# f1tenth/f1tenth_planning

Hardware: AMD Instinct MI355X
Metric: candidate-trajectory-steps/sec per GPU; p50 plan() latency @4096 egos (higher is better)
Workload: dtype f32 filter + f64 decision

## Files before the change

f1tenth_planning_amd/csrc/f1p_device.h:

```cpp
#pragma once
#include <hip/hip_runtime.h>
#include <stdint.h>

#include "../../include/f1p.h"

#define F1P_WAVE 64
#define F1P_PI 3.14159265358979323846
#define F1P_LA_NONE INT32_MIN
#ifndef F1P_NEAREST_PRUNE
#define F1P_NEAREST_PRUNE 1
#endif

namespace f1p {

__device__ __forceinline__ double shfl_d(double v, int src) {
    int lo = __double2loint(v), hi = __double2hiint(v);
    lo = __shfl(lo, src, F1P_WAVE);
    hi = __shfl(hi, src, F1P_WAVE);
    return __hiloint2double(hi, lo);
}
__device__ __forceinline__ double shfl_xor_d(double v, int mask) {
    int lo = __double2loint(v), hi = __double2hiint(v);
    lo = __shfl_xor(lo, mask, F1P_WAVE);
    hi = __shfl_xor(hi, mask, F1P_WAVE);
// ... 177 lines not shown
    best_d = __builtin_huge_val();
    best_i = 0x7fffffff;
    double bt = 0.0;
    const int lane = tid & 63, wave = tid >> 6, nw = nthreads >> 6;
    const int nseg = n - 1;
    const int nchunk = (nseg + 63) >> 6;
    const int stride = (n + 63) >> 6;
    int j = lane * stride;
    if (j > n - 1) j = n - 1;
    double b0x = 0.0, b0X = 0.0, b0y = 0.0, b0Y = 0.0, sx_ = 0.0, sy_ = 0.0;
    if (pre) { b0x = pre[0]; b0X = pre[1]; b0y = pre[2]; b0Y = pre[3]; sx_ = pre[4]; sy_ = pre[5]; }
    else {
        if (lane < nchunk) { b0x = box[4 * lane]; b0X = box[4 * lane + 1]; b0y = box[4 * lane + 2]; b0Y = box[4 * lane + 3]; }
        sx_ = wx[j]; sy_ = wy[j];
    }
    const double ex = px - sx_, ey = py - sy_;
    const double ub2_own = ex * ex + ey * ey;
    const float ub2_up = (float)ub2_own * (1.0f + 2.4e-7f);
    const double ub2 = (double)f32_from_order_key(wave_min_key(f32_order_key(ub2_up == ub2_up ? ub2_up : __builtin_nanf(""))));
    const double thr = ub2 * (1.0 + 1e-6) + 1e-9;
    int turn = 0;
    for (int cb = 0; cb < nchunk; cb += 64) {
        const int c = cb + lane;
        bool keep = false;
        if (c < nchunk) {
            double xmin = b0x, xmax = b0X, ymin = b0y, ymax = b0Y;
            if (cb > 0) { xmin = box[4 * c]; xmax = box[4 * c + 1]; ymin = box[4 * c + 2]; ymax = box[4 * c + 3]; }
            const double dx = __builtin_fmax(__builtin_fmax(xmin - px, px - xmax), 0.0);
            const double dy = __builtin_fmax(__builtin_fmax(ymin - py, py - ymax), 0.0);
            keep = !(dx * dx + dy * dy > thr);
        }
        unsigned long long m = __ballot(keep);
        while (m) {
            const int b = __ffsll((long long)m) - 1;
            m &= m - 1;
            if (turn == wave) {
                const int i = ((cb + b) << 6) + lane;
                if (i < nseg) {
                    const SegProj s = seg_project(px, py, wx[i], wy[i], wx[i + 1], wy[i + 1]);
                    if (argmin_better(s.d, i, best_d, best_i)) { best_d = s.d; best_i = i; bt = s.t; }
                }
            }
            if (++turn == nw) turn = 0;
        }
    }
    if (best_t) *best_t = bt;
}

struct SegHit { bool hit; double t, x, y; };

__device__ __forceinline__ SegHit seg_hit(double px, double py, double radius, double sx, double sy, double ex, double ey,
                                          bool is_start_seg, double start_t) {
    SegHit h;
    h.hit = false; h.t = 0.0; h.x = 0.0; h.y = 0.0;
    ex = ex + 1e-6;
    ey = ey + 1e-6;
    const double vx = ex - sx, vy = ey - sy;
    const double a = dot2(vx, vy, vx, vy);
    const double b = 2.0 * dot2(vx, vy, sx - px, sy - py);
    const double c = dot2(sx, sy, sx, sy) + dot2(px, py, px, py) - 2.0 * dot2(sx, sy, px, py) - radius * radius;
    double disc = b * b - 4 * a * c;
    if (disc < 0) return h;
    disc = __builtin_sqrt(disc);
    const double t1 = (-b - disc) / (2.0 * a);
    const double t2 = (-b + disc) / (2.0 * a);
    const bool ok1 = (t1 >= 0.0) & (t1 <= 1.0) & (!is_start_seg | (t1 >= start_t));
    const bool ok2 = (t2 >= 0.0) & (t2 <= 1.0) & (!is_start_seg | (t2 >= start_t));
    if (ok1) { h.hit = true; h.t = t1; }
    else if (ok2) { h.hit = true; h.t = t2; }
    if (h.hit) { h.x = sx + h.t * vx; h.y = sy + h.t * vy; }
    return h;
}

struct Intersect { bool found; int i; double t, x, y; };

__device__ __forceinline__ Intersect wave_intersect(double px, double py, double radius, const double* wx, const double* wy,
                                                    int n, double tstart, bool wrap) {
    const int lane = threadIdx.x & 63;
    const int start_i = (int)tstart;
    const double start_t = tstart - __builtin_trunc(tstart);
    Intersect r;
    r.found = false; r.i = 0; r.t = 0.0; r.x = 0.0; r.y = 0.0;
    for (int base = start_i; base < n - 1; base += 64) {
        const int i = base + lane;
        SegHit h;
        h.hit = false; h.t = 0; h.x = 0; h.y = 0;
        if (i < n - 1) h = seg_hit(px, py, radius, wx[i], wy[i], wx[i + 1], wy[i + 1], i == start_i, start_t);
        const unsigned long long m = __ballot(h.hit);
        if (m) {
            const int first = __ffsll((long long)m) - 1;
            r.found = true; r.i = base + first;
            r.t = shfl_d(h.t, first); r.x = shfl_d(h.x, first); r.y = shfl_d(h.y, first);
            return r;
        }
    }
    if (wrap) {
        for (int base = -1; base < start_i; base += 64) {
            const int i = base + lane;
            SegHit h;
            h.hit = false; h.t = 0; h.x = 0; h.y = 0;
            if (i < start_i) {
                const int i0 = i < 0 ? i + n : i;
                int i1 = i + 1; if (i1 >= n) i1 -= n;
                h = seg_hit(px, py, radius, wx[i0], wy[i0], wx[i1], wy[i1], false, 0.0);
            }
            const unsigned long long m = __ballot(h.hit);
            if (m) {
                const int first = __ffsll((long long)m) - 1;
                r.found = true; r.i = base + first;
                r.t = shfl_d(h.t, first); r.x = shfl_d(h.x, first); r.y = shfl_d(h.y, first);
                return r;
            }
        }
    }
    return r;
}

__device__ __forceinline__ void get_actuation(double pose_theta, double lx, double ly, double lspeed, double px, double py,
                                              double lookahead, double wheelbase, double& speed, double& steer) {
    const double sn = pose_theta == 0.0 ? -pose_theta : sin(-pose_theta);
    const double cs = pose_theta == 0.0 ? 1.0 : cos(-pose_theta);
    const double wy = dot2(sn, cs, lx - px, ly - py);
    speed = lspeed;
    if (fabs(wy) < 1e-6) { steer = 0.0; return; }
    const double radius = 1 / (2.0 * wy / (lookahead * lookahead));
    steer = atan(wheelbase / radius);
}

struct Track { double steer, speed; int la_idx, status; };

__device__ __forceinline__ Track wave_pursuit(double px, double py, double theta, double lookahead, double wheelbase,
                                              double max_reacquire, const double* wx, const double* wy, const double* wv,
                                              double v_const, int n, int near_i, double near_t, double near_d) {
    Track o;
    o.steer = 0.0; o.speed = 0.0; o.la_idx = F1P_LA_NONE; o.status = F1P_ST_NO_LOOKAHEAD;
    double cx, cy, cv;
    if (near_d < lookahead) {
        const Intersect it = wave_intersect(px, py, lookahead, wx, wy, n, (double)near_i + near_t, true);
        if (!it.found) return o;
        o.la_idx = it.i;
        const int r = it.i < 0 ? it.i + n : it.i;
        cx = wx[r]; cy = wy[r]; cv = wv ? wv[near_i] : v_const;
        o.status = F1P_ST_INTERSECT;
    } else if (near_d < max_reacquire) {
        cx = wx[near_i]; cy = wy[near_i]; cv = wv ? wv[near_i] : v_const;
        o.status = F1P_ST_REACQUIRE;
    } else {
        return o;
    }
    get_actuation(theta, cx, cy, cv, px, py, lookahead, wheelbase, o.speed, o.steer);
    return o;
}

struct GridDev {
    const uint32_t* bits;
    int32_t w, h, wwords;
    double inv_res, ox, oy;
};

__device__ __forceinline__ bool cell_of(const GridDev& g, double x, double y, int& gx, int& gy) {
    const double fx = __builtin_floor((x - g.ox) * g.inv_res);
    const double fy = __builtin_floor((y - g.oy) * g.inv_res);
    const bool inside = (fx >= 0.0) & (fy >= 0.0) & (fx < (double)g.w) & (fy < (double)g.h);
    gx = inside ? (int)fx : -1;
    gy = inside ? (int)fy : -1;
    return inside;
}

struct KmpcStep { double x, y, v, yaw; };

template <bool FAST>
__device__ __forceinline__ void kmpc_step(KmpcStep& s, double a, double delta, const f1p_kmpc_cfg& c) {
    if (delta >= c.max_steer) delta = c.max_steer;
    else if (delta <= -c.max_steer) delta = -c.max_steer;
    double sn, cs, tn;
    if (FAST) {
        double sd, cd;
        sincos_core(s.yaw, &sn, &cs);
        sincos_core(delta, &sd, &cd);
        tn = sd / cd;
    } else {
        sincos(s.yaw, &sn, &cs);
        tn = tan(delta);
    }
    const double x = s.x + s.v * cs * c.dt;
    const double y = s.y + s.v * sn * c.dt;
    const double yaw = s.yaw + (s.v / c.wheelbase) * tn * c.dt;
    double v = s.v + a * c.dt;
    if (v > c.max_speed) v = c.max_speed;
    else if (v < c.min_speed) v = c.min_speed;
    s.x = x; s.y = y; s.yaw = yaw; s.v = v;
}


struct DynState { double x, y, delta, v, yaw, yr, beta; };
struct DynConst { double K, gl_r, gl_f, h, F, R, M, N, lf2cf, lr2cr, l_r, l_f; };

__device__ __forceinline__ DynConst dyn_const(const f1p_stmpc_cfg& c) {
    const double* p = c.params;
    const double mass = p[0], l_f = p[1], l_r = p[2], h_cog = p[3], c_f = p[4], c_r = p[5], iz = p[6], mu = p[7];
    const double g = 9.81;
    DynConst k;
    k.K = (mu * mass) / ((l_f + l_r) * iz);
    k.gl_r = g * l_r; k.gl_f = g * l_f; k.h = h_cog;
    k.F = l_f * c_f; k.R = l_r * c_r;
    k.M = (mu * c_f) / (l_f + l_r);
    k.N = (mu * c_r) / (l_f + l_r);
    k.lf2cf = l_f * l_f * c_f; k.lr2cr = l_r * l_r * c_r;
    k.l_r = l_r; k.l_f = l_f;
    return k;
}

template <bool FAST>
__device__ __forceinline__ void dyn_step(DynState& s, double a, double delta_v, const f1p_stmpc_cfg& c, const DynConst& k) {
    if (delta_v >= c.max_steer_v) delta_v = c.max_steer_v;
    else if (delta_v <= -c.max_steer_v) delta_v = -c.max_steer_v;
    if (a >= c.max_accel) a = c.max_accel;
    else if (a <= -c.max_accel) a = -c.max_accel;
    const double T = k.gl_r - (a * k.h);
    const double V = k.gl_f + (a * k.h);
    const double A1 = k.K * k.F * T;
    const double A2 = k.K * (k.R * V - k.F * T);
    const double A3 = k.K * (k.lf2cf * T + k.lr2cr * V);
    const double A4 = k.M * T;
    const double A5 = k.N * V + k.M * T;
    const double A6 = k.N * V * k.l_r - k.M * T * k.l_f;
    double sn, cs, tn;
    if (FAST) {
        double sd, cd;
        sincos_fast(s.yaw + s.beta, &sn, &cs);
        sincos_core(s.delta, &sd, &cd);
        tn = sd / cd;
    } else {
        sincos(s.yaw + s.beta, &sn, &cs);
        tn = tan(s.delta);
    }
    const double x_new = s.x + s.v * cs * c.dt;
    const double y_new = s.y + s.v * sn * c.dt;
    double delta_new = s.delta + delta_v * c.dt;
    double v_new = s.v + a * c.dt;
    const double yaw_new = s.yaw + s.v / c.wheelbase * tn * c.dt;
    const double yr_new = s.yr + (A1 * s.delta + A2 * s.beta - A3 * (s.yr / s.v)) * c.dt;
    const double beta_new = s.beta + (A4 * (s.delta / s.v) - A5 * (s.beta / s.v) + A6 * (s.yr / (s.v * s.v)) - s.yr) * c.dt;
    if (v_new > c.max_speed) v_new = c.max_speed;
    else if (v_new < c.min_speed) v_new = c.min_speed;
    if (delta_new >= c.max_steer) delta_new = c.max_steer;
    else if (delta_new <= -c.max_steer) delta_new = -c.max_steer;
    s.x = x_new; s.y = y_new; s.delta = delta_new; s.v = v_new; s.yaw = yaw_new; s.yr = yr_new; s.beta = beta_new;
}

}
```

f1tenth_planning_amd/csrc/f1p_internal.h:

```cpp
#pragma once
#include <vector>
#include <hip/hip_runtime.h>
#include <stdint.h>

#include <string>

#include "../../include/f1p.h"
#include "f1p_device.h"

#define F1P_KMPC_CFG_SLOTS 8

struct WarmBuf {
    void* d = nullptr;
    size_t bytes = 0;
    int key[3] = {0, 0, 0};
    bool is(int a, int b, int c = 0) const { return d && key[0] == a && key[1] == b && key[2] == c; }
    template <typename T> T* as() const { return (T*)d; }
};

struct f1p_ctx {
    int device = -1;
    hipStream_t stream = nullptr;
    hipEvent_t ev0 = nullptr, ev1 = nullptr;
    hipStream_t copy_stream = nullptr;
    hipEvent_t ev_chunk[8] = {};
    std::string err;
    hipDeviceProp_t prop;

    int n_wp = 0;
    bool has_psi = false;
    double *d_wx = nullptr, *d_wy = nullptr, *d_wv = nullptr, *d_wpsi = nullptr, *d_wkappa = nullptr;
    bool has_kappa = false;
    double* d_wbox = nullptr;

    int trk_K = 0;
    int trk_rows = 0, trk_chunks = 0;
    bool trk_has_psi = false, trk_has_kappa = false;
    double *d_tx = nullptr, *d_ty = nullptr, *d_tv = nullptr, *d_tpsi = nullptr, *d_tkappa = nullptr, *d_tbox = nullptr;
    int32_t* d_ttab = nullptr;

    bool has_grid = false;
    uint32_t* d_bits = nullptr;
    uint32_t* d_bits0 = nullptr;
    double inflate_radius = 0.0;
    double user_inflate = 0.0;
    double disc_radius = 0.0;
    uint32_t* d_bits_clear = nullptr;
    double clear_dist = 0.0;
    int lattice_clear_r = 2;
    int n_disc = 0;
    double disc_off[4] = {0, 0, 0, 0};
    int gw = 0, gh = 0, gwwords = 0;
    double res = 0, inv_res = 0, ox = 0, oy = 0;

    char* d_arena = nullptr;
    size_t arena_bytes = 0, arena_used = 0;
    char* h_bounce = nullptr;

    bool kmpc_mixed = true;
    float* d_dbg_cost32 = nullptr;
    int32_t* d_dbg_nref = nullptr;

    bool stmpc_mixed = true;
    float* d_dbg_st_cost32 = nullptr;
    int32_t* d_dbg_st_nref = nullptr;
    char* d_st_scratch = nullptr;
    size_t st_scratch_bytes = 0;
    bool st_q_dirty = true;

    f1p_kmpc_cfg* d_kmpc_cfg = nullptr;
    f1p_kmpc_cfg* h_kmpc_cfg = nullptr;
    f1p_kmpc_cfg* d_kmpc_cfg_cur = nullptr;
    int kmpc_cfg_used = 0;
    WarmBuf kmpc_warm;
    bool kmpc_warm_valid = false;
    char* d_kmpc_scratch = nullptr;
    int kmpc_cap_E = 0, kmpc_cap_R = 0;
    int kmpc_yaw_fixup = 1;
    int kmpc_groups = 0;
    WarmBuf kmpc_qp_warm;
    bool kmpc_qp_warm_valid = false;
    int kmpc_qp_pack = 0;
    WarmBuf stmpc_qp_warm;
    std::vector<int32_t> stmpc_qp_len;
    WarmBuf stmpc_warm;
    std::vector<int32_t> stmpc_warm_tag;

    char* d_bb_scratch = nullptr;
    size_t bb_scratch_bytes = 0;

    int lattice_mixed = 1;
    int pursuit_form = 0;
    char* d_mix_scratch = nullptr;
    size_t mix_scratch_bytes = 0;
    int mix_last_E = 0;
    size_t mix_ego_n_off = 0;
    char* d_rec_scratch = nullptr;
    size_t rec_scratch_bytes = 0;
    float dbg_margin_rel = 0.f, dbg_margin_abs = 0.f; bool dbg_margins = false;
    int audit_every = 0, audit_egos = 0;
    bool auditing = false;
    unsigned long long audit_plans = 0;
    unsigned long long* d_audit = nullptr;
    char* d_audit_buf = nullptr;
    size_t audit_buf_bytes = 0;
    int lattice_chunks = 0;
    hipStream_t pipe_stream[2] = {};
    hipEvent_t ev_pipe[4] = {};
    char* d_order = nullptr;
    size_t order_bytes = 0;
    int order_E = 0;
    bool order_valid = false;
    int lattice_order = 1;
    bool step_chain = false;
    bool mix_q_dirty_prev = false;
    bool mix_q_dirty = false;
    bool lattice_profile = false, lattice_profile_valid = false;
    hipEvent_t ev_prof[5] = {};
    float* d_dbg_lat_bound = nullptr;
    float* d_dbg_lat_cost32 = nullptr;
    int32_t* d_dbg_lat_state = nullptr;
    int32_t* d_dbg_lat_pass = nullptr;

    bool lattice_closed_loop = false;
    double* d_cl_theta[2] = {nullptr, nullptr};
    size_t cl_bytes = 0;
    int cl_cur = 0;
    bool cl_valid = false;
    int cl_E = 0, cl_S = 0;

    bool traj_dst_host = false;
    char* h_step = nullptr; size_t step_host_bytes = 0;
    char* h_step_dev = nullptr;
    char* d_step = nullptr; size_t step_dev_bytes = 0;
    struct HostBlock { char* base; size_t bytes; char* dev; };
    std::vector<HostBlock> host_blocks;
    int step_traj_E = 0, step_traj_S = 0;

    char* d_split_scratch = nullptr;
    int split_cap_E = 0;
    int lattice_split = 0;

    void* rccl_lib = nullptr;
    void* comm = nullptr;
    int comm_rank = 0, comm_nranks = 0;
    uint64_t* d_comm_key = nullptr;
    int32_t* d_comm_idx = nullptr;
    int comm_cap = 0;
    int comm_exchange = 0;
    uint64_t* d_comm_rec = nullptr;
    int comm_rec_cap = 0, comm_rec_ranks = 0;
};

namespace f1p {

int set_error(f1p_ctx* ctx, int code, const std::string& msg);
int check_hip(f1p_ctx* ctx, hipError_t e, const char* what);

#define F1P_HIP(ctx, call)                                   \
    do {                                                     \
        hipError_t _e = (call);                              \
        if (_e != hipSuccess) return f1p::check_hip((ctx), _e, #call); \
    } while (0)

int arena_reset(f1p_ctx* ctx, size_t need_bytes);
void* arena_take(f1p_ctx* ctx, size_t bytes);

GridDev grid_dev(const f1p_ctx* ctx);

int warm_ensure(f1p_ctx* ctx, WarmBuf* w, size_t bytes, int a, int b, int c, bool zero, bool* fresh);
int warm_upload(f1p_ctx* ctx, WarmBuf* w, const void* host, size_t bytes);
int warm_download(f1p_ctx* ctx, const WarmBuf* w, void* host, size_t bytes);

int launch_nearest(f1p_ctx* ctx, const double* d_pts, int E, double* d_proj, double* d_dist, double* d_t, int32_t* d_idx);
int launch_intersect(f1p_ctx* ctx, const double* d_pts, const double* d_start_t, int E, double radius, int wrap,
                     double* d_p, int32_t* d_i, double* d_t, int32_t* d_found);
int launch_pure_pursuit(f1p_ctx* ctx, const double* d_poses, int E, double lookahead, double wheelbase,
                        double max_reacquire, double* d_steer, double* d_speed, int32_t* d_near, int32_t* d_la,
                        int32_t* d_status);
int launch_pack_grid(f1p_ctx* ctx, const uint8_t* d_img, int w, int h, int occupied_below);
int launch_grid_edt(f1p_ctx* ctx, int cap, uint32_t thr2, float* d_dist_img, uint32_t* d_d2, uint32_t* d_bits_out, const uint32_t* src = nullptr);
int ensure_clear_map(f1p_ctx* ctx, double dist_cells);

enum LatticeMode { LATTICE_FULL = 0, LATTICE_EVAL = 1, LATTICE_EMIT = 2 };
int launch_lattice(f1p_ctx* ctx, int mode, const double* d_poses, const double* d_goals, const double* d_prev_theta,
                   int E, const f1p_lattice_cfg* cfg, const int32_t* d_emit_idx, const double* d_emit_cost,
                   double* d_steer, double* d_speed, int32_t* d_best_idx, double* d_best_cost, int32_t* d_status,
                   int32_t* d_near_idx, double* d_best_traj, double* d_all_cost, double* d_all_traj, float* d_best_traj32 = nullptr,
                   double* d_theta_out = nullptr,
                   double* d_pose_copy = nullptr,
                   const int32_t* d_track_id = nullptr);
int launch_clothoid_sample(f1p_ctx* ctx, const double* d_params, int n, int S, double* d_rows);
int launch_clothoid_g1(f1p_ctx* ctx, const double* d_goals, int n, double* d_k0, double* d_dk, double* d_len, int32_t* d_ok);

int launch_kmpc_shoot(f1p_ctx* ctx, const double* d_x0, const double* d_ref, const float* d_controls, int E,
                      const f1p_kmpc_cfg* cfg, double* d_steer, double* d_speed, int32_t* d_best_idx,
                      double* d_best_cost, double* d_best_seq);
int launch_kmpc_plan_gen(f1p_ctx* ctx, const double* d_x0, const double* d_ref, int E, const f1p_kmpc_cfg* cfg,
                         const f1p_kmpc_sampler* smp, const float* d_warm_in, float* d_warm_out, double* d_steer, double* d_speed,
                         int32_t* d_best_idx, double* d_best_cost, double* d_best_seq,
                         const int32_t* d_ids = nullptr, int wstride = 0, uint32_t ego_off = 0u);
int launch_kmpc_gen_controls(f1p_ctx* ctx, float* d_controls, int E, const f1p_kmpc_cfg* cfg, const f1p_kmpc_sampler* smp, const float* d_warm);
int kmpc_plan_groups(const f1p_ctx* ctx, int E, int R);
int launch_kmpc_qp(f1p_ctx* ctx, const double* d_x0, const double* d_ref, const double* d_pa, const double* d_pd, int pstride, int E,
                   const f1p_kmpc_cfg* cfg, int max_iter, double tol, double* d_steer, double* d_speed, int32_t* d_status, double* d_u,
                   double* d_xk, double* d_obj, double* d_duals, int32_t* d_iters, double* d_warm_out);
int kmpc_qp_pack(const f1p_ctx* ctx, int T);
int launch_stmpc_qp(f1p_ctx* ctx, const double* d_x0, const double* d_ref, const double* d_pa, const double* d_pd, int pstride, int E,
                    const f1p_stmpc_cfg* cfg, int max_iter, double tol, double* d_steer, double* d_speed, int32_t* d_status, double* d_u,
                    double* d_x, double* d_obj, double* d_duals, int32_t* d_iters, double* d_warm_out);
size_t stmpc_qp_lds_bytes(int T);
int launch_stmpc_qp_warm_in(f1p_ctx* ctx, const double* d_warm, const int32_t* d_idx, const int32_t* d_use, int nb, int Tb, int W, double* d_out);
int launch_stmpc_qp_warm_out(f1p_ctx* ctx, const double* d_in, const int32_t* d_idx, int nb, int Tb, int W, double* d_warm);
int launch_stmpc_qp_kref(f1p_ctx* ctx, const double* d_ref7, int nb, int T, double* d_ref4);
int launch_kmpc_predict(f1p_ctx* ctx, const double* d_x0, const double* d_oa, const double* d_od, int E,
                        const f1p_kmpc_cfg* cfg, double* d_path);
int launch_kmpc_ref(f1p_ctx* ctx, const double* d_states, int E, int horizon, double dt, double dl, double* d_ref);
int launch_kmpc_sample(f1p_ctx* ctx, float* d_controls, int E, const f1p_kmpc_cfg* cfg, uint64_t seed, double sigma_a,
                       double sigma_d);
int launch_stanley(f1p_ctx* ctx, const double* d_states, int E, double wheelbase, double k_path, double* d_steer,
                   double* d_speed, int32_t* d_near);
int launch_lqr(f1p_ctx* ctx, const double* d_states, double* d_err, int E, double wheelbase, double ts, const double* q,
               double r, int max_iter, double eps, double* d_steer, double* d_speed, int32_t* d_near);
int launch_stmpc_predict(f1p_ctx* ctx, const double* d_x0, const double* d_oa, const double* d_od, int E, const f1p_stmpc_cfg* cfg, double* d_path);
int launch_stmpc_shoot(f1p_ctx* ctx, const double* d_x0, const double* d_ref, const float* d_controls, int E, const f1p_stmpc_cfg* cfg,
                       double* d_steer, double* d_speed, int32_t* d_best_idx, double* d_best_cost, double* d_best_seq);
int launch_stmpc_ref(f1p_ctx* ctx, const double* d_states, int E, int horizon, double dt, double dl, double* d_ref);
int launch_stmpc_plan_gen(f1p_ctx* ctx, const double* d_x0, const double* d_ref, int E, const f1p_stmpc_cfg* cfg, const f1p_stmpc_sampler* smp,
                          float* d_warm, int wstride, const int32_t* d_ids, double* d_steer, double* d_speed, int32_t* d_best_idx,
                          double* d_best_cost, double* d_best_seq);
int launch_stmpc_gen_controls(f1p_ctx* ctx, float* d_controls, int E, const f1p_stmpc_cfg* cfg, const f1p_stmpc_sampler* smp, float* d_warm, int wstride);
int launch_stmpc_warm_zero(f1p_ctx* ctx, float* d_warm, const int32_t* d_rows, int n, int wstride);
struct TrackSetDev {
    const double *x, *y, *v, *psi, *kappa, *box;
    const int4* tab;
    int K;
};
TrackSetDev track_set_dev(const f1p_ctx* ctx);
int launch_nearest_tracks(f1p_ctx* ctx, const double* d_pts, const int32_t* d_tid, int E, double* d_proj, double* d_dist, double* d_t,
                          int32_t* d_idx);
int launch_pure_pursuit_tracks(f1p_ctx* ctx, const double* d_poses, const int32_t* d_tid, int E, double lookahead, double wheelbase,
                               double max_reacquire, double* d_steer, double* d_speed, int32_t* d_near, int32_t* d_la, int32_t* d_status);
int launch_stanley_tracks(f1p_ctx* ctx, const double* d_states, const int32_t* d_tid, int E, double wheelbase, double k_path,
                          double* d_steer, double* d_speed, int32_t* d_near);
int launch_lqr_tracks(f1p_ctx* ctx, const double* d_states, const int32_t* d_tid, double* d_err, int E, double wheelbase, double ts,
                      const double* q, double r, int max_iter, double eps, double* d_steer, double* d_speed, int32_t* d_near);
int launch_kmpc_ref_tracks(f1p_ctx* ctx, const double* d_states, const int32_t* d_tid, int E, int horizon, double dt, double dl, double* d_ref);
int launch_stmpc_ref_tracks(f1p_ctx* ctx, const double* d_states, const int32_t* d_tid, int E, int horizon, double dt, double dl, double* d_ref);
int launch_argmin_key(f1p_ctx* ctx, const double* d_cost, uint64_t* d_key, int E);
int launch_argmin_mask(f1p_ctx* ctx, const uint64_t* d_own, const uint64_t* d_min, const int32_t* d_idx, int32_t* d_masked,
                       double* d_cost_out, int E);
int launch_argmin_pack(f1p_ctx* ctx, const double* d_cost, const int32_t* d_idx, uint64_t* d_rec, int E);
int launch_argmin_reduce(f1p_ctx* ctx, const uint64_t* d_recs, int N, int E, int32_t* d_idx_out, double* d_cost_out);

}
```

f1tenth_planning_amd/csrc/f1p_lattice.hip:

```cpp
#include "f1p_host.h"

using namespace f1p;

#ifndef F1P_TRAJ_ZEROCOPY
#define F1P_TRAJ_ZEROCOPY 1
#endif
#ifndef F1P_IO_ZEROCOPY
#define F1P_IO_ZEROCOPY 1
#endif
#define F1P_PLAN_CHUNK_MIN_EGOS 2048
#ifndef F1P_ZEROCOPY_MIN_EGOS
#define F1P_ZEROCOPY_MIN_EGOS 32
#endif
#define F1P_PLAN_CHUNKS_MAX 8

static int ensure_copy_stream(f1p_ctx* ctx) {
    if (ctx->copy_stream) return F1P_OK;
    F1P_HIP(ctx, hipStreamCreateWithFlags(&ctx->copy_stream, hipStreamNonBlocking));
    for (auto& ev : ctx->ev_chunk) F1P_HIP(ctx, hipEventCreateWithFlags(&ev, hipEventDisableTiming));
    return F1P_OK;
}

static int validate_lattice(f1p_ctx* ctx, const f1p_lattice_cfg* cfg, int E, bool device_goals, bool need_outputs_ok, bool tracks = false) {
    if (!cfg) return set_error(ctx, F1P_EINVAL, "cfg is NULL");
// ... 238 lines not shown
    const int K = (pinned && E >= 8192) ? (E / 4096 < F1P_PLAN_CHUNKS_MAX ? E / 4096 : F1P_PLAN_CHUNKS_MAX) : 1;
    if (K > 1 && (rc = ensure_copy_stream(ctx))) return rc;
    if (K == 1) {
        if ((rc = plan(0, e))) return rc;
        cl_commit(ctx, cl, E, (int)S);
        return s.finish();
    }
    for (int k = 0; k < K; ++k) {
        const size_t e0 = e * k / K, e1 = e * (k + 1) / K, n = e1 - e0;
        if ((rc = plan(e0, n))) return rc;
        F1P_HIP(ctx, hipEventRecord(ctx->ev_chunk[k], ctx->stream));
        F1P_HIP(ctx, hipStreamWaitEvent(ctx->copy_stream, ctx->ev_chunk[k], 0));
        F1P_HIP(ctx, hipMemcpyAsync(best_traj + e0 * S * 4, d_bt + e0 * S * 4, n * S * 4 * sizeof(TRAJ), hipMemcpyDeviceToHost, ctx->copy_stream));
    }
    cl_commit(ctx, cl, E, (int)S);
    rc = s.gather(best_traj);
    F1P_HIP(ctx, hipStreamSynchronize(ctx->copy_stream));
    return rc;
}

int f1p_lattice_plan_batch(f1p_ctx* ctx, const double* poses, const double* goals, const double* prev_theta,
                           int32_t E, const f1p_lattice_cfg* cfg, double* steer, double* speed, int32_t* best_idx,
                           double* best_cost, int32_t* status, int32_t* near_idx, double* best_traj,
                           double* all_cost, double* all_traj) {
    F1P_ENTER(ctx);
    return lattice_plan_batch_impl<double>(ctx, poses, goals, prev_theta, E, cfg, steer, speed, best_idx, best_cost, status, near_idx, best_traj, all_cost, all_traj);
}

int f1p_lattice_plan_batch_f32(f1p_ctx* ctx, const double* poses, const double* goals, const double* prev_theta,
                               int32_t E, const f1p_lattice_cfg* cfg, double* steer, double* speed, int32_t* best_idx,
                               double* best_cost, int32_t* status, int32_t* near_idx, float* best_traj32) {
    F1P_ENTER(ctx);
    return lattice_plan_batch_impl<float>(ctx, poses, goals, prev_theta, E, cfg, steer, speed, best_idx, best_cost, status, near_idx, best_traj32, nullptr, nullptr);
}

int f1p_lattice_plan_tracks_batch(f1p_ctx* ctx, const double* poses, const double* goals, const double* prev_theta, const int32_t* track_id,
                                  int32_t E, const f1p_lattice_cfg* cfg, double* steer, double* speed, int32_t* best_idx,
                                  double* best_cost, int32_t* status, int32_t* near_idx, double* best_traj,
                                  double* all_cost, double* all_traj) {
    F1P_ENTER(ctx);
    return lattice_plan_batch_impl<double>(ctx, poses, goals, prev_theta, E, cfg, steer, speed, best_idx, best_cost, status, near_idx, best_traj, all_cost, all_traj,
                                           track_id, true);
}

int f1p_lattice_plan_tracks_batch_f32(f1p_ctx* ctx, const double* poses, const double* goals, const double* prev_theta, const int32_t* track_id,
                                      int32_t E, const f1p_lattice_cfg* cfg, double* steer, double* speed, int32_t* best_idx,
                                      double* best_cost, int32_t* status, int32_t* near_idx, float* best_traj32) {
    F1P_ENTER(ctx);
    return lattice_plan_batch_impl<float>(ctx, poses, goals, prev_theta, E, cfg, steer, speed, best_idx, best_cost, status, near_idx, best_traj32, nullptr, nullptr,
                                          track_id, true);
}

static int ensure_step(f1p_ctx* ctx, int E, int S, bool keep_traj) {
    const size_t hb = al256(32 * (size_t)E) + 2 * al256(8 * (size_t)E) + al256(4 * (size_t)E);
    if (hb > ctx->step_host_bytes) {
        F1P_HIP(ctx, hipStreamSynchronize(ctx->stream));
        if (ctx->h_step) (void)hipHostFree(ctx->h_step);
        ctx->h_step = nullptr; ctx->step_host_bytes = 0; ctx->h_step_dev = nullptr;
        F1P_HIP(ctx, hipHostMalloc((void**)&ctx->h_step, hb, hipHostMallocDefault));
        ctx->step_host_bytes = hb;
        void* dev = nullptr;
        ctx->h_step_dev = (hipHostGetDevicePointer(&dev, ctx->h_step, 0) == hipSuccess) ? (char*)dev : nullptr;
        if (!ctx->h_step_dev) (void)hipGetLastError();
    }
    const size_t db = al256(32 * (size_t)E) + 2 * al256(4 * (size_t)E) + (keep_traj ? al256(32 * (size_t)E * S) : 0);
    if (db > ctx->step_dev_bytes) {
        F1P_HIP(ctx, hipStreamSynchronize(ctx->stream));
        if (ctx->d_step) (void)hipFree(ctx->d_step);
        ctx->d_step = nullptr; ctx->step_dev_bytes = 0; ctx->step_traj_E = 0;
        F1P_HIP(ctx, hipMalloc((void**)&ctx->d_step, db));
        ctx->step_dev_bytes = db;
    }
    return F1P_OK;
}

static int lattice_step_impl(f1p_ctx* ctx, const double* poses, int32_t E, const f1p_lattice_cfg* cfg, double* steer, double* speed,
                             int32_t* status, int32_t keep_traj, const int32_t* track_id, bool tracks) {
    int rc = validate_lattice(ctx, cfg, E, true, E == 0 || (poses && steer && speed), tracks);
    if (rc) return rc;
    if (cfg->cand_count > 0) return set_error(ctx, F1P_EINVAL, "f1p_lattice_step_batch plans whole egos: cfg.cand_count must be 0");
    if (tracks && E > 0 && !track_id) return set_error(ctx, F1P_EINVAL, "track_id is NULL");
    if (E == 0) return F1P_OK;
    const int S = cfg->n_stations;
    const size_t e = (size_t)E;
    if ((rc = ensure_step(ctx, E, S, keep_traj != 0))) return rc;
    char* hb = ctx->h_step;
    double* h_poses = (double*)hb; double* h_steer = (double*)(hb + al256(32 * e)); double* h_speed = (double*)((char*)h_steer + al256(8 * e));
    int32_t* h_status = (int32_t*)((char*)h_speed + al256(8 * e));
    char* db = ctx->d_step;
    double* d_pose_copy = (double*)db; int32_t* d_idx = (int32_t*)(db + al256(32 * e)); int32_t* d_near = (int32_t*)((char*)d_idx + al256(4 * e));
    double* d_traj = keep_traj ? (double*)((char*)d_near + al256(4 * e)) : nullptr;
    const double* k_poses = (const double*)pinned_device_ptr(ctx, poses, 32 * e);
    if (!k_poses) { memcpy(h_poses, poses, 32 * e); k_poses = (const double*)pinned_device_ptr(ctx, h_poses, 32 * e); }
    double* k_steer = (double*)pinned_device_ptr(ctx, steer, 8 * e); double* k_speed = (double*)pinned_device_ptr(ctx, speed, 8 * e);
    int32_t* k_status = status ? (int32_t*)pinned_device_ptr(ctx, status, 4 * e) : nullptr;
    const bool own_steer = !k_steer, own_speed = !k_speed, own_status = status && !k_status;
    if (own_steer) k_steer = (double*)pinned_device_ptr(ctx, h_steer, 8 * e);
    if (own_speed) k_speed = (double*)pinned_device_ptr(ctx, h_speed, 8 * e);
    if (own_status) k_status = (int32_t*)pinned_device_ptr(ctx, h_status, 4 * e);
    if (!k_poses || !k_steer || !k_speed || (status && !k_status)) return set_error(ctx, F1P_ESTATE, "page-locked step block is not device-visible");
    const int32_t* k_tid = tracks ? (const int32_t*)pinned_device_ptr(ctx, track_id, 4 * e) : nullptr;
    if (tracks && !k_tid) {
        if ((rc = arena_reset(ctx, al256(4 * e)))) return rc;
        int32_t* d = (int32_t*)arena_take(ctx, 4 * e);
        F1P_HIP(ctx, hipMemcpyAsync(d, track_id, 4 * e, hipMemcpyHostToDevice, ctx->stream));
        k_tid = d;
    }
    const bool was_armed = ctx->lattice_closed_loop;
    if (!was_armed && !ctx->step_chain) ctx->cl_valid = false;
    ctx->lattice_closed_loop = true;
    ClosedLoop cl;
    rc = cl_begin(ctx, nullptr, E, S, true, &cl);
    if (rc == F1P_OK)
        rc = launch_lattice(ctx, LATTICE_FULL, k_poses, nullptr, cl.prev, E, cfg, nullptr, nullptr, k_steer, k_speed, d_idx, nullptr, k_status, d_near,
                            d_traj, nullptr, nullptr, nullptr, cl.out, d_pose_copy, k_tid);
    ctx->lattice_closed_loop = was_armed;
    if (rc) return rc;
    cl_commit(ctx, cl, E, S);
    ctx->step_chain = !was_armed;
    ctx->step_traj_E = keep_traj ? E : 0; ctx->step_traj_S = S;
    F1P_HIP(ctx, hipStreamSynchronize(ctx->stream));
    if (own_steer) memcpy(steer, h_steer, 8 * e);
    if (own_speed) memcpy(speed, h_speed, 8 * e);
    if (own_status) memcpy(status, h_status, 4 * e);
    return F1P_OK;
}

int f1p_lattice_step_batch(f1p_ctx* ctx, const double* poses, int32_t E, const f1p_lattice_cfg* cfg, double* steer, double* speed,
                           int32_t* status, int32_t keep_traj) {
    F1P_ENTER(ctx);
    return lattice_step_impl(ctx, poses, E, cfg, steer, speed, status, keep_traj, nullptr, false);
}

int f1p_lattice_step_tracks_batch(f1p_ctx* ctx, const double* poses, const int32_t* track_id, int32_t E, const f1p_lattice_cfg* cfg, double* steer,
                                  double* speed, int32_t* status, int32_t keep_traj) {
    F1P_ENTER(ctx);
    return lattice_step_impl(ctx, poses, E, cfg, steer, speed, status, keep_traj, track_id, true);
}

int f1p_lattice_fetch_traj(f1p_ctx* ctx, double* best_traj, int32_t E, int32_t S) {
    F1P_ENTER(ctx);
    if (!best_traj) return set_error(ctx, F1P_EINVAL, "best_traj is NULL");
    if (ctx->step_traj_E <= 0 || !ctx->d_step) return set_error(ctx, F1P_ESTATE, "no trajectories kept: call f1p_lattice_step_batch with keep_traj = 1 first");
    if (E != ctx->step_traj_E || S != ctx->step_traj_S) return set_error(ctx, F1P_EINVAL, "E / S differ from the last f1p_lattice_step_batch");
    const size_t e = (size_t)E;
    const char* d_traj = ctx->d_step + al256(32 * e) + 2 * al256(4 * e);
    F1P_HIP(ctx, hipMemcpyAsync(best_traj, d_traj, 32 * e * S, hipMemcpyDeviceToHost, ctx->stream));
    F1P_HIP(ctx, hipStreamSynchronize(ctx->stream));
    return F1P_OK;
}

int f1p_lattice_set_mode(f1p_ctx* ctx, int32_t mixed, float* d_cost32, int32_t* d_state) {
    if (!ctx) return F1P_EINVAL;
    if (mixed < 0 || mixed > 3) return set_error(ctx, F1P_EINVAL, "mixed must be 0 (all fp64), 1 (f32 filter, the default), 2 (f32 filter at any batch size) or 3 (as 2, one ego per wave in the per-ego kernels)");
    ctx->lattice_mixed = mixed;
    ctx->d_dbg_lat_cost32 = d_cost32;
    ctx->d_dbg_lat_state = d_state;
    return F1P_OK;
}

int f1p_lattice_set_split(f1p_ctx* ctx, int32_t groups) {
    if (!ctx) return F1P_EINVAL;
    if (groups < 0 || groups > 16) return set_error(ctx, F1P_EINVAL, "groups must be in [0, 16]");
    ctx->lattice_split = groups;
    return F1P_OK;
}

int f1p_lattice_set_clearance(f1p_ctx* ctx, int32_t stations_each_side) {
    if (!ctx) return F1P_EINVAL;
    if (stations_each_side < 0 || stations_each_side > 2) return set_error(ctx, F1P_EINVAL, "stations_each_side must be 0, 1 or 2");
    ctx->lattice_clear_r = stations_each_side;
    return F1P_OK;
}

int f1p_lattice_debug_queue(f1p_ctx* ctx, int32_t* entries_per_ego, int32_t E) {
    F1P_ENTER(ctx);
    if (!entries_per_ego || E < 1) return set_error(ctx, F1P_EINVAL, "entries_per_ego is NULL or E < 1");
    if (!ctx->d_mix_scratch || ctx->mix_last_E != E) return set_error(ctx, F1P_ESTATE, "no mixed-schedule plan of this batch size has run");
    F1P_HIP(ctx, hipStreamSynchronize(ctx->stream));
    F1P_HIP(ctx, hipMemcpy(entries_per_ego, ctx->d_mix_scratch + ctx->mix_ego_n_off, sizeof(int32_t) * (size_t)E, hipMemcpyDeviceToHost));
    return F1P_OK;
}

int f1p_lattice_debug_bound(f1p_ctx* ctx, float* d_bound) {
    if (!ctx) return F1P_EINVAL;
    ctx->d_dbg_lat_bound = d_bound;
    return F1P_OK;
}

int f1p_lattice_set_order(f1p_ctx* ctx, int32_t heavy_first) {
    if (!ctx) return F1P_EINVAL;
    if (heavy_first < 0 || heavy_first > 1) return set_error(ctx, F1P_EINVAL, "heavy_first must be 0 or 1");
    ctx->lattice_order = heavy_first;
    return F1P_OK;
}

int f1p_lattice_debug_pass(f1p_ctx* ctx, int32_t* d_pass) {
    if (!ctx) return F1P_EINVAL;
    ctx->d_dbg_lat_pass = d_pass;
    return F1P_OK;
}

int f1p_lattice_debug_margins(f1p_ctx* ctx, int32_t enable, float margin_rel, float margin_abs) {
    if (!ctx) return F1P_EINVAL;
    ctx->dbg_margins = enable != 0; ctx->dbg_margin_rel = margin_rel; ctx->dbg_margin_abs = margin_abs;
    return F1P_OK;
}

int f1p_lattice_set_audit(f1p_ctx* ctx, int32_t every_n, int32_t n_egos) {
    if (!ctx) return F1P_EINVAL;
    if (every_n < 0 || n_egos < 0 || (every_n > 0 && n_egos < 1)) return set_error(ctx, F1P_EINVAL, "every_n >= 0 and, when auditing, n_egos >= 1");
    ctx->audit_every = every_n; ctx->audit_egos = n_egos;
    return F1P_OK;
}

int f1p_lattice_audit_read(f1p_ctx* ctx, uint64_t out[3], int32_t reset) {
    F1P_ENTER(ctx);
    if (!out) return set_error(ctx, F1P_EINVAL, "out is NULL");
    out[0] = out[1] = out[2] = 0;
    if (!ctx->d_audit) return F1P_OK;
    F1P_HIP(ctx, hipStreamSynchronize(ctx->stream));
    unsigned long long h[3];
    F1P_HIP(ctx, hipMemcpy(h, ctx->d_audit, sizeof(h), hipMemcpyDeviceToHost));
    out[0] = h[0]; out[1] = h[1]; out[2] = h[2];
    if (reset) F1P_HIP(ctx, hipMemset(ctx->d_audit, 0, sizeof(h)));
    return F1P_OK;
}

int f1p_lattice_set_pipeline(f1p_ctx* ctx, int32_t chunks) {
    if (!ctx) return F1P_EINVAL;
    if (chunks < 0 || chunks > 8) return set_error(ctx, F1P_EINVAL, "chunks must be in [0, 8]");
    ctx->lattice_chunks = chunks;
    return F1P_OK;
}

int f1p_lattice_profile(f1p_ctx* ctx, int32_t enable, float kernel_ms[4]) {
    F1P_ENTER(ctx);
    if (kernel_ms) {
        if (!ctx->lattice_profile || !ctx->lattice_profile_valid) return set_error(ctx, F1P_ESTATE, "no profiled mixed-schedule plan has run");
        F1P_HIP(ctx, hipEventSynchronize(ctx->ev_prof[4]));
        for (int k = 0; k < 4; ++k) F1P_HIP(ctx, hipEventElapsedTime(&kernel_ms[k], ctx->ev_prof[k], ctx->ev_prof[k + 1]));
    }
    if (enable && !ctx->ev_prof[0])
        for (auto& ev : ctx->ev_prof) F1P_HIP(ctx, hipEventCreate(&ev));
    ctx->lattice_profile = enable != 0;
    if (!enable) ctx->lattice_profile_valid = false;
    return F1P_OK;
}

int f1p_clothoid_sample_batch(f1p_ctx* ctx, const double* params, int32_t n, int32_t npts, double* rows) {
    F1P_ENTER(ctx);
    if (n < 0 || (n > 0 && (!params || !rows))) return set_error(ctx, F1P_EINVAL, "bad params / rows / n");
    if (npts < 1 || npts > 65536) return set_error(ctx, F1P_EINVAL, "npts must be in [1, 65536]");
    Stage s(ctx);
    s.need(8 * 3 * (size_t)n); s.need(8 * 4 * (size_t)n * npts);
    int rc = s.begin(); if (rc) return rc;
    const double* d_p;
    if ((rc = s.in(params, (size_t)3 * n, &d_p))) return rc;
    double* d_rows = s.out(rows, (size_t)4 * n * npts);
    if ((rc = launch_clothoid_sample(ctx, d_p, n, npts, d_rows))) return rc;
    return s.finish();
}

int f1p_clothoid_g1_batch(f1p_ctx* ctx, const double* goals, int32_t n, double* kappa0, double* dkappa, double* length, int32_t* ok) {
    F1P_ENTER(ctx);
    if (n < 0 || (n > 0 && !goals)) return set_error(ctx, F1P_EINVAL, "bad goals / n");
    Stage s(ctx);
    s.need(8 * 3 * (size_t)n); s.need(8 * (size_t)n, kappa0); s.need(8 * (size_t)n, dkappa); s.need(8 * (size_t)n, length); s.need(4 * (size_t)n, ok);
    int rc = s.begin(); if (rc) return rc;
    const double* d_g;
    if ((rc = s.in(goals, (size_t)3 * n, &d_g))) return rc;
    double* d_k0 = s.out(kappa0, n); double* d_dk = s.out(dkappa, n); double* d_L = s.out(length, n); int32_t* d_ok = s.out(ok, n);
    if ((rc = launch_clothoid_g1(ctx, d_g, n, d_k0, d_dk, d_L, d_ok))) return rc;
    return s.finish();
}
```

f1tenth_planning_amd/csrc/k_lattice_filter3.hip:

```cpp
#include "lattice_mixed.h"

namespace f1p {

__constant__ float c_gl16_xf[16] = {5.299532504e-03f, 2.771248846e-02f, 6.718439881e-02f, 1.222977958e-01f, 1.910618778e-01f, 2.709916112e-01f, 3.591982246e-01f, 4.524937451e-01f, 5.475062549e-01f, 6.408017754e-01f, 7.290083888e-01f, 8.089381222e-01f, 8.777022042e-01f, 9.328156012e-01f, 9.722875115e-01f, 9.947004675e-01f};
__constant__ float c_gl16_wuf[16][6] = {
    {1.357622971e-02f, -7.156638159e-05f, 3.772584204e-07f, -1.988697942e-09f, 1.048331671e-11f, -5.526225325e-14f},
    {3.112676197e-02f, -8.386952385e-04f, 2.259822926e-05f, -6.088981340e-07f, 1.640645970e-08f, -4.420639591e-10f},
    {4.757925584e-02f, -2.981823145e-03f, 1.868728107e-04f, -1.171144152e-05f, 7.339637150e-07f, -4.599798703e-08f},
    {6.231448563e-02f, -6.688902003e-03f, 7.179937307e-04f, -7.707019733e-05f, 8.272795516e-06f, -8.880105154e-07f},
    {7.479799441e-02f, -1.156057132e-02f, 1.786769958e-03f, -2.761582272e-04f, 4.268225247e-05f, -6.596850996e-06f},
    {8.457825970e-02f, -1.670887144e-02f, 3.300923736e-03f, -6.521145096e-04f, 1.288285849e-04f, -2.545075142e-05f},
    {9.130170752e-02f, -2.101535775e-02f, 4.837207029e-03f, -1.113403451e-03f, 2.562774835e-04f, -5.898863390e-05f},
    {9.472530523e-02f, -2.346754605e-02f, 5.813923915e-03f, -1.440359858e-03f, 3.568392966e-04f, -8.840449344e-05f},
    {9.472530523e-02f, -2.346754605e-02f, 5.813923915e-03f, -1.440359858e-03f, 3.568392966e-04f, -8.840449344e-05f},
    {9.130170752e-02f, -2.101535775e-02f, 4.837207029e-03f, -1.113403451e-03f, 2.562774835e-04f, -5.898863390e-05f},
    {8.457825970e-02f, -1.670887144e-02f, 3.300923736e-03f, -6.521145096e-04f, 1.288285849e-04f, -2.545075142e-05f},
    {7.479799441e-02f, -1.156057132e-02f, 1.786769958e-03f, -2.761582272e-04f, 4.268225247e-05f, -6.596850996e-06f},
    {6.231448563e-02f, -6.688902003e-03f, 7.179937307e-04f, -7.707019733e-05f, 8.272795516e-06f, -8.880105154e-07f},
    {4.757925584e-02f, -2.981823145e-03f, 1.868728107e-04f, -1.171144152e-05f, 7.339637150e-07f, -4.599798703e-08f},
    {3.112676197e-02f, -8.386952385e-04f, 2.259822926e-05f, -6.088981340e-07f, 1.640645970e-08f, -4.420639591e-10f},
    {1.357622971e-02f, -7.156638159e-05f, 3.772584204e-07f, -1.988697942e-09f, 1.048331671e-11f, -5.526225325e-14f}};

__constant__ float c_gl8_p[8] = {4.947285525e-01f, 4.730554936e-01f, 4.373293446e-01f, 3.926589550e-01f, 3.454427633e-01f, 3.024448422e-01f, 2.698251400e-01f, 2.522568443e-01f};
__constant__ float c_gl8_q[8] = {-4.947004675e-01f, -4.722875115e-01f, -4.328156012e-01f, -3.777022042e-01f, -3.089381222e-01f, -2.290083888e-01f, -1.408017754e-01f, -4.750625492e-02f};
// ... 840 lines not shown
    const int S_u = __builtin_amdgcn_readfirstlane(ep->S);
    const PassPlan plan = pass_plan<CR>(S_u, exact_all_wg);
    const PassPlan plan_x = pass_plan<CR>(S_u, true);
    const F1P_LDS(unsigned char)* tile_b = (const F1P_LDS(unsigned char)*)lds_raw;
    const unsigned pitch_b = (unsigned)pitch * 8u;
    float thr = my_hi_p;
    bool thr_is_T = false;
    F1P_FPH();
    wg_min1(0, thr);
    F1P_FPH();
#if defined(F1P_F3_ABLATE) && F1P_F3_ABLATE == 3
    if (tid == 0) { mx.ego_base[e] = 0; mx.ego_n[e] = 0; }
    return;
#endif
    int rounds_run = 0;
    for (int round = 0; round < F1P_MIX_ROUNDS; ++round) {
        rounds_run = round + 1;
        float my_lo_p = INF;
        for (int cb = c0; cb < c1; cb += blockDim.x) {
            const int c = cand_of(cb);
            const int st = c < c1 ? (int)c_st[c - c0] : F1P_ST_BAD;
            const float lo = c < c1 ? c_lo[c - c0] : INF;
            const int st7 = st & 0x7f;
            const bool pend = (st7 == F1P_ST_PENDING) | (st7 == F1P_ST_PENDING2);
            const bool sel = pend && (all_states || !(lo > thr));
            const bool sel1 = sel && st7 == F1P_ST_PENDING;
            const unsigned long long m1 = __ballot(sel1);
            unsigned long long m2 = __ballot(sel && st7 == F1P_ST_PENDING2);
            int ns = st7;
            if (m1 | m2) {
                float k0 = 0.f, dk = 0.f, L = 0.f, ek0 = 0.f, edk = 0.f, eL = 0.f;
                if (sel) {
                    if (one_pass) { const float* q = c_fit + (c - c0); k0 = q[0]; dk = q[nc]; L = q[2 * nc]; ek0 = q[3 * nc]; edk = q[4 * nc]; eL = q[5 * nc]; }
                    else {
                        float lo2, hi2, gx, gy; Brk32 o; int dbg_code;
                        (void)bracket_of(c, k0, dk, L, ek0, edk, eL, lo2, hi2, gx, gy, o, dbg_code);
                    }
                }
                [[maybe_unused]] float xe = 0.f, ye = 0.f;
                bool bound_known = false;
#pragma nounroll
                for (int look = 0; look < 2; ++look) {
                    const unsigned long long m = look == 0 ? m1 : m2;
                    if (!m) continue;
                    const bool ex = look == 0 ? exact_all_wg : true;
                    const bool mine = ((m >> lane) & 1ull) != 0ull;
                    float edge = 2.0f;
                    bool nfree = look == 0 && (st & 0x80) != 0;
                    if (mine) { edge = GEN == F1P_GEN_CUBIC ? edge_cubic(edk, ep, ft.omax) : edge_f2<CR>(k0, dk, L, ek0, edk, eL, ep, ex, nullptr, ft.omax); nfree |= !(edge < 0.8f); }
                    const int nt = ex ? plan_x.nt : plan.nt;
                    bool coop = false;
#ifndef F1P_MIX_DEBUG_END
                    coop = F1P_MIX_MACRO && nt <= 64 && (__builtin_popcountll(m) <= ((look == 1 && !(thr_is_T | bound_known)) ? 2 * F1P_MIX_COOP_MAX : F1P_MIX_COOP_MAX) || (all_states && (e & 1)));
#endif
                    PassPlan pl;
                    pl.nt = nt; pl.nm = ex ? plan_x.nm : plan.nm; pl.first_m = ex ? plan_x.first_m : plan.first_m;
                    pl.tail_m = ex ? plan_x.tail_m : plan.tail_m; pl.tail_pos = ex ? plan_x.tail_pos : plan.tail_pos;
                    if (coop) {
                        for (unsigned long long mm = m; mm; mm &= mm - 1) {
                            const int sl = __ffsll((long long)mm) - 1;
                            const float uk0 = __int_as_float(__builtin_amdgcn_readlane(__float_as_int(k0), sl)), udk = __int_as_float(__builtin_amdgcn_readlane(__float_as_int(dk), sl));
                            const float uL = __int_as_float(__builtin_amdgcn_readlane(__float_as_int(L), sl)), uedge = __int_as_float(__builtin_amdgcn_readlane(__float_as_int(edge), sl));
                            const bool unf = __builtin_amdgcn_readlane(nfree ? 1 : 0, sl) != 0;
                            int r;
                            if constexpr (GEN == F1P_GEN_CUBIC) {
                                const float ucy = __int_as_float(__builtin_amdgcn_readlane(__float_as_int(ek0), sl)), um_ = __int_as_float(__builtin_amdgcn_readlane(__float_as_int(edk), sl));
                                r = station_pass_wave_cubic<CR, FOOT>(uk0, udk, uL, ucy, um_, uedge, unf, ep, (const F1P_LDS(CubicTab)*)ctab, tile_b, pitch_b, lane, pl, ex, ft);
                            } else r = station_pass_wave<CR, FOOT>(uk0, udk, uL, uedge, unf, ep, tile_b, pitch_b, lane, pl, ex, ft);
                            if (lane == sl) ns = r;
                        }
                    } else if (mine) {
                        if constexpr (GEN == F1P_GEN_CUBIC) ns = station_pass_cubic<CR, FOOT>(k0, dk, L, ek0, edk, edge, nfree, ep, (const F1P_LDS(CubicTab)*)ctab, tile_b, pitch_b, pl, ex, ft);
                        else ns = station_pass_f2<CR, FOOT>(k0, dk, L, edge, nfree, ep, tile_b, pitch_b, xe, ye, ex, ft);
                        if (DBG && mx.dbg_pass) atomicAdd(&mx.dbg_pass[4 * (size_t)e + 1], 1);
                    }
                    if (DBG && mx.dbg_pass && mine) atomicAdd(&mx.dbg_pass[4 * (size_t)e + (look == 0 ? 0 : 3)], 1);
                    if (look == 0) {
                        const bool again = mine && ns == F1P_ST_UNSURE && !ex;
                        if (again) ns = F1P_ST_PENDING2;
                        if (coop | thr_is_T) m2 |= __ballot(again);
                        else {
                            const float t_w = f32_from_order_key(wave_min_key(f32_order_key((mine && ns == F1P_ST_FREE) ? c_hi[c - c0] : INF)));
                            if (t_w < INF) { m2 |= __ballot(again && !(lo > t_w)); bound_known = true; }
                        }
                        const int n2 = __builtin_popcountll(m2);
                        if (n2 > F1P_MIX_COOP_MAX && n2 <= F1P_MIX_COOP_MAX_X && (thr_is_T | bound_known) && !all_states) {
                            unsigned long long pick = 0ull, rem = m2;
#pragma unroll
                            for (int i = 0; i < F1P_MIX_COOP_MAX; ++i) {
                                const bool in = ((rem >> lane) & 1ull) != 0ull;
                                const int key = f32_order_key(in ? lo : INF);
                                const int kmin = wave_min_key(key);
                                const unsigned long long eq = __ballot(in && key == kmin);
                                const unsigned long long one = eq & (0ull - eq);
                                pick |= one; rem &= ~one;
                            }
                            m2 = pick;
                        }
                    }
                }
                if (ns != st7) {
                    c_st[c - c0] = (unsigned char)ns;
                    if (ns == F1P_ST_FREE) t_free = fminf(t_free, c_hi[c - c0]);
                    if (DBG && mx.dbg_state) mx.dbg_state[(size_t)e * C + c] = ns;
#ifdef F1P_MIX_DEBUG_END
                    if (DBG && mx.dbg_cost32) {
                        const int l = (int)(((float)c + 0.5f) * ep->inv_nw), k = c - l * cfg.n_width;
                        const F1P_LDS(GoalFrame32)* gf = (const F1P_LDS(GoalFrame32)*)gfr + l;
                        const double w = ((const F1P_LDS(double)*)wtab)[k];
                        const float gx = (float)__builtin_fma(w, gf->nx, gf->cx), gy = (float)__builtin_fma(w, gf->ny, gf->cy);
                        mx.dbg_cost32[(size_t)e * C + c] = __builtin_sqrtf((gx - xe) * (gx - xe) + (gy - ye) * (gy - ye));
                    }
#endif
                }
            }
            if ((ns == F1P_ST_PENDING) | (ns == F1P_ST_PENDING2)) my_lo_p = fminf(my_lo_p, lo);
        }
        float t = t_free;
        wg_min2(1 + (round & 1), t, my_lo_p);
#ifdef F1P_F3_PHASES
        ++n_rounds;
#endif
        if (DBG && mx.dbg_pass && tid == 0) atomicAdd(&mx.dbg_pass[4 * (size_t)e + 2], 1);
        thr_is_T = t < INF;
        thr = t;
        t_free = t;
        if (!(my_lo_p <= thr) && !(all_states && my_lo_p < INF)) break;
    }
    F1P_FPH();
#if defined(F1P_F3_ABLATE) && F1P_F3_ABLATE == 2
    if (tid == 0) { mx.ego_base[e] = 0; mx.ego_n[e] = 0; }
    return;
#endif
    const float t_min = t_free;

    const bool none_free = !(t_min < INF);
    int mine = 0;
    for (int cb = c0; cb < c1; cb += blockDim.x) {
        const int c = cand_of(cb);
        if (c >= c1) continue;
        const int st = c_st[c - c0] & 0x7f;
        const bool need = ((st == F1P_ST_FREE) | (st == F1P_ST_UNSURE) | (st == F1P_ST_PENDING2)) & !(c_lo[c - c0] > t_min);
        mine += (need | (none_free & (c == c0))) ? 1 : 0;
    }
    int pos = 0;
    if (mine) pos = atomicAdd(&cnt[0], mine);
    __syncthreads();
    if (tid == 0) {
        const int n = cnt[0];
        const unsigned int sh = (unsigned int)e % F1P_MIX_QSHARDS;
        const unsigned int base = sh * mx.q_shard_cap + atomicAdd(&mx.qcount[sh * 32u], (unsigned int)n);
        cnt[1] = (int)base;
        mx.ego_base[e] = (int)base; mx.ego_n[e] = n;
        if (mx.heavy) { const int h = mx.heavy[e]; mx.heavy[e] = (unsigned char)(rounds_run >= 2 ? F1P_MIX_HEAVY_MEMORY : (h > 0 ? h - 1 : 0)); }
    }
    double g1x = 0.0, g1y = 0.0, g1th = 0.0;
    int ok1 = 0;
    bool need1 = false;
    if (one_pass && cand_of(c0) < c1) {
        const int c = cand_of(c0);
        need1 = mine != 0;
        if (need1) {
            const int st = c_st[c - c0] & 0x7f;
            const bool gok = HG ? candidate_goal_host(a.goals, e, C, c, g1x, g1y, g1th) : candidate_goal_rec(cfg, c, hdr, cen, nl, gfr, g1x, g1y, g1th);
            ok1 = gok ? (st == F1P_ST_FREE ? -2 : -1) : 0;
        }
    }
    __syncthreads();
    const int base = cnt[1];
    if (one_pass) {
        if (need1) {
            RefEntry r;
            r.e = e; r.c = cand_of(c0); r.gx = g1x; r.gy = g1y; r.gth = g1th;
            r.cost = __builtin_huge_val(); r.k0 = 0.0; r.dk = 0.0; r.L = 0.0; r.ok = ok1; r.pad = 0;
            mx.q[base + pos] = r;
        }
    } else
    for (int cb = c0; cb < c1; cb += blockDim.x) {
        const int c = cand_of(cb);
        if (c >= c1) continue;
        const int st = c_st[c - c0] & 0x7f;
        const bool need = ((st == F1P_ST_FREE) | (st == F1P_ST_UNSURE) | (st == F1P_ST_PENDING2)) & !(c_lo[c - c0] > t_min);
        if (need | (none_free & (c == c0))) {
            double gx = 0.0, gy = 0.0, gth = 0.0;
            const bool gok = HG ? candidate_goal_host(a.goals, e, C, c, gx, gy, gth) : candidate_goal_rec(cfg, c, hdr, cen, nl, gfr, gx, gy, gth);
            RefEntry r;
            r.e = e; r.c = c; r.gx = gx; r.gy = gy; r.gth = gth;
            r.cost = __builtin_huge_val(); r.k0 = 0.0; r.dk = 0.0; r.L = 0.0; r.ok = gok ? (st == F1P_ST_FREE ? -2 : -1) : 0; r.pad = 0;
            mx.q[base + pos] = r;
            ++pos;
        }
    }
#ifdef F1P_F3_PHASES
    F1P_FPH();
    if (DBG && mx.dbg_cost32 && !mx.dbg_state && lane == 0) {
        float* d = mx.dbg_cost32 + (size_t)e * C + 16 * wave;
        for (int k = 1; k < nfp; ++k) d[k] = (float)(fph[k] - fph[0]);
        d[0] = (float)nfp; d[14] = (float)n_rounds; d[15] = (float)(fph[0] & 0xffffff);
    }
#endif
#if F1P_MIX_F3_EGOS_PER_WG > 1
    __syncthreads();
#endif
    }
}



template <int CR>
static bool filter3_fits(f1p_ctx* ctx, bool foot, bool cubic, size_t lds) {
    bool ok = lds_fits(ctx, k_lattice_filter3<CR>, lds) && lds_fits(ctx, (k_lattice_filter3<CR, true>), lds) && lds_fits(ctx, (k_lattice_filter3<CR, true, true>), lds) &&
              lds_fits(ctx, (k_lattice_filter3<CR, false, true>), lds);
    if (foot)
        ok = ok && lds_fits(ctx, (k_lattice_filter3<CR, true, false, F1P_GEN_CLOTHOID, true>), lds) && lds_fits(ctx, (k_lattice_filter3<CR, true, true, F1P_GEN_CLOTHOID, true>), lds) &&
             lds_fits(ctx, (k_lattice_filter3<CR, false, false, F1P_GEN_CLOTHOID, true>), lds);
    if (cubic)
        ok = ok && lds_fits(ctx, (k_lattice_filter3<CR, true, false, F1P_GEN_CUBIC, true>), lds) && lds_fits(ctx, (k_lattice_filter3<CR, true, true, F1P_GEN_CUBIC, true>), lds) &&
             lds_fits(ctx, (k_lattice_filter3<CR, false, false, F1P_GEN_CUBIC>), lds) && lds_fits(ctx, (k_lattice_filter3<CR, true, false, F1P_GEN_CUBIC>), lds) &&
             lds_fits(ctx, (k_lattice_filter3<CR, true, true, F1P_GEN_CUBIC>), lds);
    return ok;
}

bool mixed_filter3_fits(f1p_ctx* ctx, int cr, bool foot, bool cubic, size_t lds) {
    return cr == 1 ? filter3_fits<1>(ctx, foot, cubic, lds) : filter3_fits<2>(ctx, foot, cubic, lds);
}

template <int CR>
static void filter3_launch(bool hooks, bool host_goals, bool cubic, bool foot, unsigned grid, size_t lds, hipStream_t st, const LatticeArgs& a,
                           const f1p_lattice_cfg& cfg, const MixArgs& mx, const unsigned char* recs) {
    const dim3 g(grid), fb(F1P_MIX_FILTER_BLOCK);
    if (cubic && foot && host_goals) hipLaunchKernelGGL((k_lattice_filter3<CR, true, true, F1P_GEN_CUBIC, true>), g, fb, lds, st, a, cfg, mx, recs);
    else if (cubic && foot) hipLaunchKernelGGL((k_lattice_filter3<CR, true, false, F1P_GEN_CUBIC, true>), g, fb, lds, st, a, cfg, mx, recs);
    else if (cubic && host_goals) hipLaunchKernelGGL((k_lattice_filter3<CR, true, true, F1P_GEN_CUBIC>), g, fb, lds, st, a, cfg, mx, recs);
    else if (cubic) {
        if (hooks) hipLaunchKernelGGL((k_lattice_filter3<CR, true, false, F1P_GEN_CUBIC>), g, fb, lds, st, a, cfg, mx, recs);
        else hipLaunchKernelGGL((k_lattice_filter3<CR, false, false, F1P_GEN_CUBIC>), g, fb, lds, st, a, cfg, mx, recs);
    } else if (foot) {
        if (host_goals) hipLaunchKernelGGL((k_lattice_filter3<CR, true, true, F1P_GEN_CLOTHOID, true>), g, fb, lds, st, a, cfg, mx, recs);
        else if (hooks) hipLaunchKernelGGL((k_lattice_filter3<CR, true, false, F1P_GEN_CLOTHOID, true>), g, fb, lds, st, a, cfg, mx, recs);
        else hipLaunchKernelGGL((k_lattice_filter3<CR, false, false, F1P_GEN_CLOTHOID, true>), g, fb, lds, st, a, cfg, mx, recs);
    } else if (host_goals) {
        if (hooks) hipLaunchKernelGGL((k_lattice_filter3<CR, true, true>), g, fb, lds, st, a, cfg, mx, recs);
        else hipLaunchKernelGGL((k_lattice_filter3<CR, false, true>), g, fb, lds, st, a, cfg, mx, recs);
    } else {
        if (hooks) hipLaunchKernelGGL((k_lattice_filter3<CR, true>), g, fb, lds, st, a, cfg, mx, recs);
        else hipLaunchKernelGGL(k_lattice_filter3<CR>, g, fb, lds, st, a, cfg, mx, recs);
    }
}

void mixed_launch_filter3(int cr, bool hooks, bool host_goals, bool cubic, bool foot, unsigned grid, size_t lds, hipStream_t st, const LatticeArgs& a,
                          const f1p_lattice_cfg& cfg, const MixArgs& mx, const unsigned char* recs) {
    if (cr == 1) filter3_launch<1>(hooks, host_goals, cubic, foot, grid, lds, st, a, cfg, mx, recs);
    else filter3_launch<2>(hooks, host_goals, cubic, foot, grid, lds, st, a, cfg, mx, recs);
}

}
```

f1tenth_planning_amd/csrc/k_lattice_mixed.hip:

```cpp
#include "lattice_mixed.h"

namespace f1p {

__global__ void k_lattice_audit_compare(int n, int S, const double* steer, const double* speed, const int32_t* idx, const double* cost,
                                        const int32_t* status, const int32_t* near_idx, const double* traj, const float* traj32,
                                        const double* r_steer, const double* r_speed, const int32_t* r_idx, const double* r_cost,
                                        const int32_t* r_status, const int32_t* r_near, const double* r_traj, unsigned long long* counters) {
    const int i = blockIdx.x * blockDim.x + threadIdx.x;
    bool bad = false;
    if (i < n) {
        auto same = [](double a, double b) { return __double_as_longlong(a) == __double_as_longlong(b) || (a != a && b != b); };
        if (steer) bad |= !same(steer[i], r_steer[i]);
        if (speed) bad |= !same(speed[i], r_speed[i]);
        bad |= idx[i] != r_idx[i];
        if (cost) bad |= !same(cost[i], r_cost[i]);
        if (status) bad |= status[i] != r_status[i];
        if (near_idx) bad |= near_idx[i] != r_near[i];
        if (traj) for (int k = 0; k < 4 * S; ++k) bad |= !same(traj[(size_t)i * 4 * S + k], r_traj[(size_t)i * 4 * S + k]);
        if (traj32) for (int k = 0; k < 4 * S; ++k) { const float a = traj32[(size_t)i * 4 * S + k], b = (float)r_traj[(size_t)i * 4 * S + k]; bad |= !(a == b || (a != a && b != b)); }
    }
    const unsigned long long m = __ballot(bad);
    if ((threadIdx.x & 63) == 0 && m) atomicAdd(&counters[2], (unsigned long long)__builtin_popcountll(m));
    if (i == 0) { atomicAdd(&counters[0], 1ull); atomicAdd(&counters[1], (unsigned long long)n); }
}

static int lattice_audit(f1p_ctx* ctx, const double* d_poses, const double* d_prev_theta, const int32_t* d_track_id, int E, const f1p_lattice_cfg* cfg,
                         double* d_steer, double* d_speed, int32_t* d_best_idx, double* d_best_cost, int32_t* d_status,
                         int32_t* d_near_idx, double* d_best_traj, float* d_best_traj32) {
    const int n = ctx->audit_egos < E ? ctx->audit_egos : E;
    const int S = cfg->n_stations;
    const unsigned long long h = (ctx->audit_plans * 0x9E3779B97F4A7C15ull) >> 20;
    const int w0 = E > n ? (int)(h % (unsigned long long)(E - n + 1)) : 0;
    const size_t need = 256 * 8 + (size_t)n * (8 + 8 + 4 + 8 + 4 + 4) + (size_t)n * S * 32;
    if (!ctx->d_audit) {
        F1P_HIP(ctx, hipMalloc((void**)&ctx->d_audit, 3 * sizeof(unsigned long long)));
        F1P_HIP(ctx, hipMemsetAsync(ctx->d_audit, 0, 3 * sizeof(unsigned long long), ctx->stream));
    }
    if (need > ctx->audit_buf_bytes) {
        F1P_HIP(ctx, hipStreamSynchronize(ctx->stream));
        if (ctx->d_audit_buf) (void)hipFree(ctx->d_audit_buf);
        ctx->d_audit_buf = nullptr; ctx->audit_buf_bytes = 0;
        F1P_HIP(ctx, hipMalloc((void**)&ctx->d_audit_buf, need));
        ctx->audit_buf_bytes = need;
    }
    char* b = ctx->d_audit_buf;
    auto take = [&](size_t bytes) { char* p = b; b += (bytes + 255) & ~(size_t)255; return p; };
    double* r_steer = (double*)take(8 * (size_t)n); double* r_speed = (double*)take(8 * (size_t)n);
    int32_t* r_idx = (int32_t*)take(4 * (size_t)n); double* r_cost = (double*)take(8 * (size_t)n);
    int32_t* r_status = (int32_t*)take(4 * (size_t)n); int32_t* r_near = (int32_t*)take(4 * (size_t)n);
    double* r_traj = (double*)take((size_t)n * S * 32);
    f1p_lattice_cfg ref_cfg = *cfg;
    ref_cfg.prune = 0;
    const int mixed = ctx->lattice_mixed;
    ctx->lattice_mixed = 0; ctx->auditing = true;
    const int rc = launch_lattice(ctx, LATTICE_FULL, d_poses + 4 * (size_t)w0, nullptr, d_prev_theta ? d_prev_theta + (size_t)w0 * S : nullptr, n, &ref_cfg,
                                  nullptr, nullptr, r_steer, r_speed, r_idx, r_cost, r_status, r_near, r_traj, nullptr, nullptr, nullptr, nullptr, nullptr,
                                  d_track_id ? d_track_id + w0 : nullptr);
    ctx->lattice_mixed = mixed; ctx->auditing = false;
    if (rc) return rc;
    hipLaunchKernelGGL(k_lattice_audit_compare, dim3((n + 255) / 256), dim3(256), 0, ctx->stream, n, S,
                       d_steer ? d_steer + w0 : nullptr, d_speed ? d_speed + w0 : nullptr, d_best_idx + w0, d_best_cost ? d_best_cost + w0 : nullptr,
                       d_status ? d_status + w0 : nullptr, d_near_idx ? d_near_idx + w0 : nullptr,
                       d_best_traj ? d_best_traj + (size_t)w0 * S * 4 : nullptr, d_best_traj32 ? d_best_traj32 + (size_t)w0 * S * 4 : nullptr,
                       r_steer, r_speed, r_idx, r_cost, r_status, r_near, r_traj, ctx->d_audit);
    return check_hip(ctx, hipGetLastError(), "k_lattice_audit_compare launch");
}

int launch_lattice_mixed(f1p_ctx* ctx, LatticeArgs& a, const f1p_lattice_cfg* cfg, int mode, int E, bool foot, bool cubic,
                         double* d_pose_copy, bool* handled) {
    *handled = false;
    const int S = cfg->n_stations;
    const int n_cand = cfg->cand_count > 0 ? cfg->cand_count : cfg->n_lookahead * cfg->n_width;
    const double *d_poses = a.poses, *d_prev_theta = a.prev_theta;
    double *d_all_traj = a.all_traj, *d_all_cost = a.all_cost;
    double *d_steer = a.steer, *d_speed = a.speed, *d_best_cost = a.best_cost, *d_best_traj = a.best_traj;
    int32_t *d_best_idx = a.best_idx, *d_status = a.status, *d_near_idx = a.near_idx;
    float* d_best_traj32 = a.best_traj32;
    auto fin = [](double v) { return v == v && v < HUGE_VAL && v > -HUGE_VAL; };
    const bool weights_finite = fin(cfg->w_length) && fin(cfg->w_max_kappa) && fin(cfg->w_mean_kappa) && fin(cfg->w_similarity);
    double clear_ds_cap = 0.0, clear_dist = 0.0;
    bool clear_ok = false;
    int clear_r_eff = 0;
    const bool collide = a.has_grid && cfg->check_collision;
    if (collide && ctx->lattice_clear_r > 0 && ctx->lattice_clear_r <= 2) {
        double la = 0.0, wd = 0.0;
        for (int l = 0; l < cfg->n_lookahead; ++l) la = fmax(la, fabs(cfg->lookahead[l]));
        for (int k = 0; k < cfg->n_width; ++k) wd = fmax(wd, fabs(cfg->width[k]));
        const int den = S - 1 > 1 ? S - 1 : 1;
        clear_ds_cap = 1.2 * hypot(la, wd) / (double)den;
        if (a.goals) clear_ds_cap = 1.2 * 4.0 / (double)den;
        if (foot) {
            double mo = 0.0;
            for (int d = 0; d < ctx->n_disc; ++d) mo = fmax(mo, fabs(ctx->disc_off[d]));
            clear_ds_cap *= 1.0 + mo * 1.0;
        }
        for (clear_r_eff = ctx->lattice_clear_r; clear_r_eff >= 1 && !clear_ok; --clear_r_eff) {
            clear_dist = (double)clear_r_eff * clear_ds_cap * 1.001 * ctx->inv_res + 1.41422 + 1.0;
            clear_ok = clear_dist == clear_dist && clear_dist <= 0.25 * (double)a.tile_rows;
            if (clear_ok) break;
        }
    }
    const bool tile_ok = a.tile_words + 1 <= 32;
    const bool cubic_ok = !cubic || S <= 256;
    if (ctx->lattice_mixed && tile_ok && cubic_ok && !d_all_traj && !d_all_cost && mode != LATTICE_EMIT && weights_finite && n_cand <= 4096 &&
        (E >= F1P_MIX_MIN_EGOS_V3 || ctx->lattice_mixed > 1)) {
        const size_t lds_r16 = sizeof(double) * 16 * (64 + 4 * (size_t)S), lds_r64 = sizeof(double) * 4 * (64 + 4 * (size_t)S);
        const size_t lds_r_static = 1024;
        const size_t lds_s = sizeof(double) * 16 * (size_t)S;
        const bool groups16 = mixed_refine_fits(ctx, 16, foot, lds_r16 + lds_r_static);
        const bool refine_fits = groups16 || mixed_refine_fits(ctx, 64, foot, lds_r64 + lds_r_static);
        const bool tracks = a.track_id != nullptr;
        if (refine_fits && mixed_select_fits(ctx, false, lds_s, tracks)) {
            MixArgs mx;
            mx.margin_rel = F1P_MIX_MARGIN_REL; mx.margin_abs = F1P_MIX_MARGIN_ABS; mx.edge0 = F1P_MIX_EDGE0; mx.edge1 = F1P_MIX_EDGE1;
            if (ctx->dbg_margins) { mx.margin_rel = ctx->dbg_margin_rel; mx.margin_abs = ctx->dbg_margin_abs; }
            mx.dbg_cost32 = ctx->d_dbg_lat_cost32; mx.dbg_state = ctx->d_dbg_lat_state; mx.dbg_bound = ctx->d_dbg_lat_bound; mx.dbg_pass = ctx->d_dbg_lat_pass;
            {
                double s2 = 0.0, s3 = 0.0, s4 = 0.0;
                for (int j = 0; j < S - cfg->n_shift - cfg->n_cull; ++j) { const double fj = (double)j; s2 += fj * fj; s3 += fj * fj * fj; s4 += (fj * fj) * (fj * fj); }
                mx.sim_s2 = s2; mx.sim_s3 = s3; mx.sim_s4 = s4;
            }
            mx.clear_bits = nullptr; mx.clear_r = 0; mx.clear_ds_cap = 0.f;
            mx.n_disc = 0;
            for (int d = 0; d < 4; ++d) { mx.disc_off[d] = 0.0; mx.disc_off_f[d] = 0.f; }
            mx.disc_omax_f = 0.f;
            if (clear_ok && ensure_clear_map(ctx, clear_dist) == F1P_OK) {
                mx.clear_bits = ctx->d_bits_clear; mx.clear_r = clear_r_eff; mx.clear_ds_cap = (float)clear_ds_cap;
            }
            if (foot) {
                mx.n_disc = ctx->n_disc;
                for (int d = 0; d < 4; ++d) { mx.disc_off[d] = ctx->disc_off[d]; mx.disc_off_f[d] = (float)ctx->disc_off[d]; if (d < mx.n_disc) mx.disc_omax_f = fmaxf(mx.disc_omax_f, fabsf(mx.disc_off_f[d]) * 1.000001f); }
            }
            const bool prof = ctx->lattice_profile && ctx->ev_prof[0];
            const size_t rec_stride = ego_rec_stride(cfg->n_lookahead);
            const size_t tile2_bytes = sizeof(uint32_t) * (size_t)(a.tile_rows + 1) * (a.tile_words + 1);
            size_t lds_f3 = 2 * tile2_bytes + 16 + rec_stride + sizeof(double) * F1P_MAX_WIDTHS + sizeof(float) * 24 + sizeof(int) * 4 + (size_t)n_cand * 9 + (n_cand <= F1P_MIX_FILTER_BLOCK ? (size_t)n_cand * 24 : 0) + 16;
            if (cubic) lds_f3 += 16 + (size_t)S * (sizeof(CubicTab) + sizeof(float));
            lds_f3 = (lds_f3 + 15) & ~(size_t)15;
            const size_t lds_rc = sizeof(double) * 16 * 5 * (size_t)S;
            const int cr = mx.clear_r == 2 ? 2 : 1;
            bool v3 = mixed_filter3_fits(ctx, cr, mx.n_disc > 0, cubic, lds_f3);
            if (cubic) v3 = v3 && S <= 256 && mixed_refine_cubic_fits(ctx, lds_rc) && mixed_select_fits(ctx, true, lds_s, tracks);
            if (!v3) return F1P_OK;
            int nch = 1;
            if (!prof) nch = ctx->lattice_chunks > 0 ? ctx->lattice_chunks : (E >= F1P_PIPE_MIN_EGOS ? F1P_PIPE_CHUNKS : 1);
            if (nch > 8) nch = 8;
            int ce = ((E + nch - 1) / nch + 3) & ~3;
            if (ce < 4) ce = 4;
            nch = (E + ce - 1) / ce;
            const size_t shard_cap = (size_t)((ce + F1P_MIX_QSHARDS - 1) / F1P_MIX_QSHARDS + 1) * n_cand;
            const size_t region = shard_cap * F1P_MIX_QSHARDS;
            const size_t qc_chunk = sizeof(unsigned int) * 32 * F1P_MIX_QSHARDS;
            const size_t qc_bytes = qc_chunk * 8;
            size_t inc_cap = (size_t)((ce + F1P_MIX_QSHARDS - 1) / F1P_MIX_QSHARDS + 1) * F1P_MIX_INC_PER_EGO;
            if (inc_cap > shard_cap) inc_cap = shard_cap;
            const size_t inc_block = 2 * (size_t)(S > 0 ? S : 1) * sizeof(double);
            const size_t inc_bytes = F1P_MIX_INC_PER_EGO > 0 ? inc_cap * F1P_MIX_QSHARDS * inc_block : 0;
            const size_t need = qc_bytes + sizeof(int32_t) * 3 * (size_t)E + 256 + sizeof(EgoXform) * (size_t)E + 256 + sizeof(RefEntry) * region * nch + 256 + inc_bytes * nch;
            bool fresh = false;
            if (need > ctx->mix_scratch_bytes) {
                fresh = true;
                F1P_HIP(ctx, hipStreamSynchronize(ctx->stream));
                if (ctx->d_mix_scratch) (void)hipFree(ctx->d_mix_scratch);
                ctx->d_mix_scratch = nullptr; ctx->mix_scratch_bytes = 0;
                F1P_HIP(ctx, hipMalloc((void**)&ctx->d_mix_scratch, need));
                ctx->mix_scratch_bytes = need;
            }
            ctx->mix_last_E = E; ctx->mix_ego_n_off = qc_bytes + sizeof(int32_t) * (size_t)E;
            mx.qcount = reinterpret_cast<unsigned int*>(ctx->d_mix_scratch);
            mx.q_shard_cap = (unsigned int)shard_cap;
            mx.ego_base = reinterpret_cast<int32_t*>(ctx->d_mix_scratch + qc_bytes);
            mx.ego_n = mx.ego_base + E; mx.ego_ni = mx.ego_n + E;
            const size_t xf_off = (qc_bytes + sizeof(int32_t) * 3 * (size_t)E + 255) & ~(size_t)255;
            mx.xf = reinterpret_cast<EgoXform*>(ctx->d_mix_scratch + xf_off);
            mx.q = reinterpret_cast<RefEntry*>(ctx->d_mix_scratch + ((xf_off + sizeof(EgoXform) * (size_t)E + 255) & ~(size_t)255));
            {
                const size_t q_off = (xf_off + sizeof(EgoXform) * (size_t)E + 255) & ~(size_t)255;
                const size_t inc_off = (q_off + sizeof(RefEntry) * region * nch + 255) & ~(size_t)255;
                mx.inc = inc_bytes ? reinterpret_cast<double*>(ctx->d_mix_scratch + inc_off) : nullptr;
                mx.inc_cap = (unsigned int)inc_cap;
            }
            if (fresh || ctx->mix_q_dirty) F1P_HIP(ctx, hipMemsetAsync(mx.qcount, 0, qc_bytes, ctx->stream));
            ctx->mix_q_dirty_prev = ctx->mix_q_dirty;
            ctx->mix_q_dirty = true;
            {
                const size_t need_rec = rec_stride * (size_t)E;
                if (need_rec > ctx->rec_scratch_bytes) {
                    F1P_HIP(ctx, hipStreamSynchronize(ctx->stream));
                    if (ctx->d_rec_scratch) (void)hipFree(ctx->d_rec_scratch);
                    ctx->d_rec_scratch = nullptr; ctx->rec_scratch_bytes = 0;
                    F1P_HIP(ctx, hipMalloc((void**)&ctx->d_rec_scratch, need_rec));
                    ctx->rec_scratch_bytes = need_rec;
                }
            }
            mx.perm = nullptr; mx.perm_fill = nullptr; mx.ocnt = nullptr; mx.heavy = nullptr; mx.perm_rs = 0;
            if (nch == 1 && E >= F1P_MIX_ORDER_MIN_EGOS && F1P_MIX_F3_EGOS_PER_WG == 1 && ctx->lattice_order) {
                const int rs = (E + F1P_MIX_OREG - 1) / F1P_MIX_OREG;
                const size_t perm_bytes = (sizeof(int32_t) * (size_t)F1P_MIX_OREG * rs + 255) & ~(size_t)255, ocnt_bytes = sizeof(unsigned int) * 64 * F1P_MIX_OREG;
                const size_t need_o = perm_bytes + ocnt_bytes + (size_t)E;
                if (need_o > ctx->order_bytes || ctx->order_E != E) {
                    if (need_o > ctx->order_bytes) {
                        F1P_HIP(ctx, hipStreamSynchronize(ctx->stream));
                        if (ctx->d_order) (void)hipFree(ctx->d_order);
                        ctx->d_order = nullptr; ctx->order_bytes = 0;
                        F1P_HIP(ctx, hipMalloc((void**)&ctx->d_order, need_o));
                        ctx->order_bytes = need_o;
                    }
                    F1P_HIP(ctx, hipMemsetAsync(ctx->d_order, 0, need_o, ctx->stream));
                    ctx->order_E = E; ctx->order_valid = false;
                } else if (fresh || ctx->mix_q_dirty_prev) ctx->order_valid = false;
                mx.perm = ctx->order_valid ? reinterpret_cast<int32_t*>(ctx->d_order) : nullptr;
                mx.perm_fill = reinterpret_cast<int32_t*>(ctx->d_order);
                mx.ocnt = reinterpret_cast<unsigned int*>(ctx->d_order + perm_bytes);
                mx.heavy = reinterpret_cast<unsigned char*>(ctx->d_order + perm_bytes + ocnt_bytes);
                mx.perm_rs = rs;
            }
            if (nch > 1) {
                if (!ctx->pipe_stream[0]) F1P_HIP(ctx, hipStreamCreateWithFlags(&ctx->pipe_stream[0], hipStreamNonBlocking));
                for (int j = 0; j < 2; ++j) if (!ctx->ev_pipe[j]) F1P_HIP(ctx, hipEventCreateWithFlags(&ctx->ev_pipe[j], hipEventDisableTiming));
            }
            if (prof) F1P_HIP(ctx, hipEventRecord(ctx->ev_prof[0], ctx->stream));
            const int cus = ctx->prop.multiProcessorCount > 0 ? ctx->prop.multiProcessorCount : 256;
            int rc = F1P_OK;
            for (int k = 0; k < nch && rc == F1P_OK; ++k) {
                hipStream_t st = (k & 1) ? ctx->pipe_stream[0] : ctx->stream;
                LatticeArgs ak = a;
                ak.e0 = k * ce; ak.E = ak.e0 + ce < E ? ak.e0 + ce : E;
                const int Ek = ak.E - ak.e0;
                MixArgs mk = mx;
                mk.qcount = mx.qcount + (size_t)k * 32 * F1P_MIX_QSHARDS;
                mk.q = mx.q + (size_t)k * region;
                if (mx.inc) mk.inc = mx.inc + (size_t)k * (inc_bytes / sizeof(double));
                {
                    ak.pose_copy = d_pose_copy;
#ifdef F1P_PRO_PHASES
                    const bool pro2 = false;
#else
                    const bool pro2 = F1P_PRO2 && ctx->lattice_mixed != 3 && cfg->n_lookahead <= 32 && ak.wbox != nullptr && (Ek >= F1P_PRO2_MIN_EGOS || ctx->lattice_mixed == 2);
#endif
                    mixed_launch_prologue(pro2, tracks, Ek, st, ak, *cfg, mk, (unsigned char*)ctx->d_rec_scratch);
                    if (d_pose_copy) { ak.poses = d_pose_copy; ak.pose_copy = nullptr; }
                    if (prof) F1P_HIP(ctx, hipEventRecord(ctx->ev_prof[1], st));
                    if (nch > 1 && k == 0) {
                        F1P_HIP(ctx, hipEventRecord(ctx->ev_pipe[0], st));
                        F1P_HIP(ctx, hipStreamWaitEvent(ctx->pipe_stream[0], ctx->ev_pipe[0], 0));
                    }
                    const unsigned f3_grid = mk.perm ? (unsigned)(F1P_MIX_OREG * mk.perm_rs) : (unsigned)((Ek + F1P_MIX_F3_EGOS_PER_WG - 1) / F1P_MIX_F3_EGOS_PER_WG);
                    const bool dbg = mk.dbg_cost32 || mk.dbg_state || mk.dbg_bound || mk.dbg_pass;
                    const unsigned char* recs = (const unsigned char*)ctx->d_rec_scratch;
                    mixed_launch_filter3(cr, dbg, ak.goals != nullptr, cubic, mk.n_disc > 0, f3_grid, lds_f3, st, ak, *cfg, mk, recs);
                }
                if ((rc = check_hip(ctx, hipGetLastError(), "k_lattice_filter3 launch"))) break;
                if (prof) F1P_HIP(ctx, hipEventRecord(ctx->ev_prof[2], st));
                size_t rb = (region + 3) / 4;
                rb = (rb + 15) & ~(size_t)15;
                const size_t rb_max = (size_t)cus * (groups16 ? F1P_MIX_REFINE_WG_PER_CU : 8) / (nch > 1 ? 2 : 1);
                if (rb > rb_max) rb = rb_max;
                rb = rb & ~(size_t)15;
                if (rb < 16) rb = 16;
                mixed_launch_refine(cubic, groups16 ? 16 : 64, mk.n_disc > 0, (unsigned)rb, cubic ? lds_rc : (groups16 ? lds_r16 : lds_r64), st, ak, *cfg, mk);
                if ((rc = check_hip(ctx, hipGetLastError(), "k_lattice_refine launch"))) break;
                if (prof) F1P_HIP(ctx, hipEventRecord(ctx->ev_prof[3], st));
                mixed_launch_select(cubic, tracks, (unsigned)((Ek + 3) / 4 + (mk.perm_fill ? (Ek + 255) / 256 : 0)), lds_s, st, ak, *cfg, mk);
                rc = check_hip(ctx, hipGetLastError(), "k_lattice_select launch");
                if (mk.perm_fill) ctx->order_valid = rc == F1P_OK;
            }
            if (nch > 1) {
                F1P_HIP(ctx, hipEventRecord(ctx->ev_pipe[1], ctx->pipe_stream[0]));
                F1P_HIP(ctx, hipStreamWaitEvent(ctx->stream, ctx->ev_pipe[1], 0));
            }
            if (rc == F1P_OK) ctx->mix_q_dirty = false;
            if (prof && rc == F1P_OK) { F1P_HIP(ctx, hipEventRecord(ctx->ev_prof[4], ctx->stream)); ctx->lattice_profile_valid = true; }
            if (rc == F1P_OK && ctx->audit_every > 0 && !ctx->auditing && mode == LATTICE_FULL && !a.goals && cfg->cand_count == 0) {
                if (ctx->audit_plans++ % (unsigned long long)ctx->audit_every == 0)
                    rc = lattice_audit(ctx, d_poses, d_prev_theta, a.track_id, E, cfg, d_steer, d_speed, d_best_idx, d_best_cost, d_status, d_near_idx, d_best_traj,
                                       d_best_traj32);
            }
            *handled = true;
            return rc;
        }
    }
    return F1P_OK;
}

}
```

f1tenth_planning_amd/csrc/k_lattice_prologue.hip:

```cpp
#include "lattice_mixed.h"

namespace f1p {

__device__ __forceinline__ int wave_scan_add_i32(int v) {
    v += __builtin_amdgcn_update_dpp(0, v, 0x111, 0xf, 0xf, false);
    v += __builtin_amdgcn_update_dpp(0, v, 0x112, 0xf, 0xf, false);
    v += __builtin_amdgcn_update_dpp(0, v, 0x114, 0xf, 0xf, false);
    v += __builtin_amdgcn_update_dpp(0, v, 0x118, 0xf, 0xf, false);
    v += __builtin_amdgcn_update_dpp(0, v, 0x142, 0xa, 0xf, false);
    v += __builtin_amdgcn_update_dpp(0, v, 0x143, 0xc, 0xf, false);
    return v;
}

__device__ __forceinline__ Intersect wave_intersect_boxed(double px, double py, double radius, const double* __restrict__ wx, const double* __restrict__ wy,
                                                          const double* __restrict__ box, int n, double tstart) {
    const int lane = threadIdx.x & 63;
    const int start_i = (int)tstart;
    const double start_t = tstart - __builtin_trunc(tstart);
    Intersect r;
    r.found = false; r.i = 0; r.t = 0.0; r.x = 0.0; r.y = 0.0;
    const int nseg = n - 1, nchunk = (nseg + 63) >> 6;
    if (!box || nchunk > 64 || start_i < 0 || start_i > nseg) return wave_intersect(px, py, radius, wx, wy, n, tstart, true);
    bool keep = false;
    if (lane < nchunk) {
// ... 94 lines not shown
                const float r = __int_as_float(__builtin_amdgcn_readlane(__float_as_int(my_r32), slot));
                const uint32_t sg = (uint32_t)__float_as_int(r - lo_s) | (uint32_t)__float_as_int(hi_s - r);
                m32 |= ((~sg) >> 31) << slot;
            }
            if (nan_seg) m32 = nslots >= 32 ? 0xffffffffu : ((1u << nslots) - 1u);
            mine = (unsigned long long)m32;
        } else {
            int slot = 0;
            for (int l = wave; l < nl; l += nwaves, ++slot) {
                const float r = __int_as_float(__builtin_amdgcn_readlane(__float_as_int(my_r32), slot));
                const bool flag = (!(r < lo_s) & !(r > hi_s)) | nan_seg;
                mine |= flag ? (1ull << slot) : 0ull;
            }
        }
        const int my_n = __builtin_popcountll(mine);
        const int incl = wave_scan_add_i32(my_n);
        total = __builtin_amdgcn_readlane(incl, 63);
        if (total > 64) fast = false;
        else {
            int idx = incl - my_n;
            for (unsigned long long m = mine; m; m &= m - 1) lds_pairs[idx++] = (lane << 8) | (__ffsll((long long)m) - 1);
        }
    }
    F1P_LAT(2);
    if (fast) {
        __builtin_amdgcn_s_waitcnt(0xc07f);
        __builtin_amdgcn_wave_barrier();
        const int code = lane < total ? lds_pairs[lane] : 0;
        const int off = code >> 8, slot = code & 0xff;
        const double hx0 = shfl_d(seg_sx, off), hy0 = shfl_d(seg_sy, off), hx1 = shfl_d(seg_ex, off), hy1 = shfl_d(seg_ey, off);
        const double pair_r = shfl_d(my_r, slot);
        if (lane < total) {
            const SegHit h = seg_hit(px, py, pair_r, hx0, hy0, hx1, hy1, off == 0, start_t);
            if (h.hit) atomicMin(&lds_first[slot], off);
        }
        __builtin_amdgcn_s_waitcnt(0xc07f);
        __builtin_amdgcn_wave_barrier();
    }
    F1P_LAT(3);
    const int my_first = (fast && lane < nslots) ? lds_first[lane] : 0x7fffffff;
    bool my_found = my_first != 0x7fffffff;
    int my_idx = my_first < nreg ? start_i + my_first : my_first - nreg - 1;
    double dmin = near_d;
    {
        const float ax = (float)(px - wrap_ax), ay = (float)(py - wrap_ay);
        const float vx = (float)(wrap_bx - wrap_ax), vy = (float)(wrap_by - wrap_ay), l2 = vx * vx + vy * vy;
        float t = l2 > 0.0f ? (ax * vx + ay * vy) * __builtin_amdgcn_rcpf(l2) : 0.0f;
        t = fminf(fmaxf(t, 0.0f), 1.0f);
        const float qx = ax - t * vx, qy = ay - t * vy;
        const double dw = (double)__builtin_amdgcn_sqrtf(qx * qx + qy * qy) * (1.0 - 1e-5);
        if (!(dw >= dmin)) dmin = dw;
    }
    const bool surely_none = my_r < dmin - (1e-4 + 4e-6 * dmin);
    unsigned long long rest = __ballot(lane < nslots && !my_found && !surely_none);
    if (stat) { stat[0] = __builtin_popcountll(rest); stat[1] = fast ? 1 : 0; stat[2] = total; stat[3] = __builtin_popcountll(__ballot(lane < nslots && surely_none)); }
    while (rest) {
        const int s = __ffsll((long long)rest) - 1;
        rest &= rest - 1;
        const Intersect it = wave_intersect_boxed(px, py, cfg.lookahead[wave + s * nwaves], wx, wy, wbox, n, tstart);
        if (lane == s) { my_found = it.found; my_idx = it.i; }
    }
    const bool from_scan = my_found && my_first == 0x7fffffff;
    const int src = my_found && !from_scan ? my_first : 0;
    double c_x = shfl_d(seg_sx, src), c_y = shfl_d(seg_sy, src), c_psi = shfl_d(seg_psi, src);
    if (lane < nslots) {
        const int l = wave + lane * nwaves;
        cen_ok[l] = my_found ? 1 : 0;
        if (from_scan) {
            const int r = my_idx < 0 ? my_idx + n : my_idx;
            c_x = wx[r]; c_y = wy[r]; c_psi = wpsi[r];
        }
        if (my_found) { cen_x[l] = c_x; cen_y[l] = c_y; cen_psi[l] = c_psi; }
    }
    F1P_LAT(4);
#undef F1P_LAT
}

struct EgoWindow { int tile_gx0, tile_gy0; double txo, tyo; uint32_t own_word; int own_bit; };

__device__ __forceinline__ EgoWindow ego_window(const LatticeArgs& a, const MixArgs& mx, bool collide_on, double px, double py, bool first) {
    EgoWindow w;
    w.tile_gx0 = 0; w.tile_gy0 = 0; w.own_word = 0xffffffffu; w.own_bit = -1;
    const double cxd = (px - a.grid.ox) * a.grid.inv_res, cyd = (py - a.grid.oy) * a.grid.inv_res;
    if (collide_on) {
        const double fx = __builtin_floor(cxd), fy = __builtin_floor(cyd);
        const int egx = (int)fmin(fmax(fx, -1.0e6), 1.0e6), egy = (int)fmin(fmax(fy, -1.0e6), 1.0e6);
        const int half = a.tile_rows / 2;
        w.tile_gx0 = ((egx - half) >> 5) << 5;
        w.tile_gy0 = egy - half;
    }
    w.txo = cxd - (double)w.tile_gx0; w.tyo = cyd - (double)w.tile_gy0;
    if (first && mx.clear_bits) {
        const int lx0 = cvt_flr_i32_f32((float)w.txo), ly0 = cvt_flr_i32_f32((float)w.tyo);
        if (((unsigned)lx0 < (unsigned)(a.tile_words * 32)) & ((unsigned)ly0 < (unsigned)a.tile_rows)) {
            w.own_bit = lx0 & 31;
            const int gw = (w.tile_gx0 >> 5) + (lx0 >> 5), gy = w.tile_gy0 + ly0;
            if (gw >= 0 && gw < a.grid.wwords && gy >= 0 && gy < a.grid.h) w.own_word = mx.clear_bits[(size_t)gy * a.grid.wwords + gw];
        }
    }
    return w;
}

__device__ __forceinline__ bool ego_disc_not_clear(const LatticeArgs& a, const MixArgs& mx, const EgoWindow& w, double cs_t, double sn_t, int idx) {
    bool ncl = false;
    if (idx < mx.n_disc) {
        const double o = (idx == 0 ? mx.disc_off[0] : idx == 1 ? mx.disc_off[1] : idx == 2 ? mx.disc_off[2] : mx.disc_off[3]) * a.grid.inv_res;
        const int lx0 = cvt_flr_i32_f32((float)__builtin_fma(cs_t, o, w.txo)), ly0 = cvt_flr_i32_f32((float)__builtin_fma(sn_t, o, w.tyo));
        ncl = true;
        if (((unsigned)lx0 < (unsigned)(a.tile_words * 32)) & ((unsigned)ly0 < (unsigned)a.tile_rows)) {
            const int gw = (w.tile_gx0 >> 5) + (lx0 >> 5), gy = w.tile_gy0 + ly0;
            if (gw >= 0 && gw < a.grid.wwords && gy >= 0 && gy < a.grid.h) ncl = ((mx.clear_bits[(size_t)gy * a.grid.wwords + gw] >> (lx0 & 31)) & 1u) != 0u;
        }
    }
    return ncl;
}

__device__ __forceinline__ void ego_record_write(const LatticeArgs& a, const f1p_lattice_cfg& cfg, const MixArgs& mx, unsigned char* rec, int e, int S, int sim_m,
                                                 double px, double py, double theta, double cs_t, double sn_t, const EgoWindow& w, double pm0, double pm1, double pm2,
                                                 bool disc_not_clear, int ni) {
    EgoXform xf;
    xf.txx = cs_t * a.grid.inv_res; xf.txy = -sn_t * a.grid.inv_res; xf.tx0 = w.txo;
    xf.tyx = sn_t * a.grid.inv_res; xf.tyy = cs_t * a.grid.inv_res; xf.ty0 = w.tyo;
    xf.tile_gx0 = w.tile_gx0; xf.tile_gy0 = w.tile_gy0;
    mx.xf[e] = xf;
    mx.ego_ni[e] = ni;
    EgoRecHdr h;
    h.px = px; h.py = py; h.theta = theta; h.ct = cs_t; h.st = sn_t;
    const int den = S - 1 > 1 ? S - 1 : 1;
    EgoParamsF2& p = h.p;
    p.txx = (float)xf.txx; p.txy = (float)xf.txy; p.tx0 = (float)xf.tx0; p.tyx = (float)xf.tyx; p.tyy = (float)xf.tyy; p.ty0 = (float)xf.ty0;
    p.w_len = (float)cfg.w_length; p.w_maxk = (float)cfg.w_max_kappa; p.w_meank = (float)cfg.w_mean_kappa; p.w_sim = (float)cfg.w_similarity;
    p.margin_rel = mx.margin_rel; p.margin_abs = mx.margin_abs;
    p.edge0 = mx.edge0; p.edge1 = mx.edge1 * (float)a.grid.inv_res;
    p.clear_ds_cap = mx.clear_ds_cap;
    p.inv_den = __builtin_amdgcn_rcpf((float)den);
    p.inv_S = __builtin_amdgcn_rcpf((float)S); p.fS = (float)S;
    p.inv_nw = 1.0f / (float)cfg.n_width; p.pad0 = 0.f;
    { const float n2 = p.txx * p.txx + p.txy * p.txy; p.cells_per_m = n2 > 0.f ? __builtin_sqrtf(n2) : 0.f; p.sqrt_S = __builtin_sqrtf((float)S); }
    p.prev = a.prev_theta ? a.prev_theta + (size_t)e * S : nullptr;
    p.M0 = pm0; p.M1 = pm1; p.M2 = pm2;
    p.tile_w = a.tile_words * 32; p.tile_h = a.tile_rows; p.tile_gx0 = w.tile_gx0; p.tile_gy0 = w.tile_gy0;
    p.S = S; p.sim_m = sim_m; p.n_shift = cfg.n_shift;
    p.exact_all = (w.own_bit < 0 || disc_not_clear) ? 1 : (int)((w.own_word >> w.own_bit) & 1u);
    *reinterpret_cast<EgoRecHdr*>(rec) = h;
}

template <bool TRK = false>
__global__ __launch_bounds__(256) void k_lattice_prologue(LatticeArgs a, f1p_lattice_cfg cfg, MixArgs mx, unsigned char* __restrict__ recs) {
    __shared__ double s_cen[4][3 * F1P_MAX_LOOKAHEADS];
    __shared__ int s_ok[4][F1P_MAX_LOOKAHEADS];
    __shared__ int s_first[4][F1P_MAX_LOOKAHEADS];
    __shared__ int s_pairs[4][64];
    warm_kernargs<sizeof(LatticeArgs) + sizeof(f1p_lattice_cfg) + sizeof(MixArgs) + 8>();
    const int lane = threadIdx.x & 63, wave = threadIdx.x >> 6;
    const int e = a.e0 + blockIdx.x * 4 + wave;
    if (e >= a.E) return;
    bool bad = false;
    if constexpr (TRK) bad = !lattice_bind_track(a, e);
    const int nl = cfg.n_lookahead, S = cfg.n_stations;
    double* cen_x = s_cen[wave]; double* cen_y = cen_x + F1P_MAX_LOOKAHEADS; double* cen_psi = cen_y + F1P_MAX_LOOKAHEADS;
    int* cen_ok = s_ok[wave];
#ifdef F1P_PRO_PHASES
    long long pph[10]; int npp = 0;
#define F1P_PPH() do { __builtin_amdgcn_s_waitcnt(0); pph[npp++] = clock64(); } while (0)
#else
#define F1P_PPH() do {} while (0)
#endif
    F1P_PPH();
    double scan_pre[6];
    if (!bad) nearest_scan_preload(a.wx, a.wy, a.wbox, a.n, lane, scan_pre);
    const double px = a.poses[4 * e], py = a.poses[4 * e + 1], theta = a.poses[4 * e + 2];
    if (a.pose_copy && lane < 4) a.pose_copy[4 * e + lane] = a.poses[4 * e + lane];
    const int sim_m = S - cfg.n_shift - cfg.n_cull;
    double pm0 = 0.0, pm1 = 0.0, pm2 = 0.0;
    if (a.prev_theta) {
        const double* pv = a.prev_theta + (size_t)e * S + cfg.n_shift;
        for (int j = lane; j < sim_m; j += 64) {
            const double p = pv[j], fj = (double)j;
            pm0 = __builtin_fma(p, p, pm0); pm1 = __builtin_fma(fj, p, pm1); pm2 = __builtin_fma(fj * fj, p, pm2);
        }
    }
    const bool collide_on = cfg.check_collision && a.has_grid;
    const EgoWindow win = ego_window(a, mx, collide_on, px, py, lane == 0);
    double sn_t = 0.0, cs_t = 1.0;
    if (lane == 0) sincos(theta, &sn_t, &cs_t);
    F1P_PPH();
    double nd; int ni;
    double my_t = 0.0;
    if (!bad) nearest_scan_boxed(px, py, a.wx, a.wy, a.wbox, a.n, lane, 64, nd, ni, &my_t, a.wbox ? scan_pre : nullptr);
    else { nd = 0.0; ni = 0; }
    F1P_PPH();
    SegProj ns;
    {
        const int my_i = ni;
        wave_argmin_2step(nd, ni);
        const unsigned long long own = __ballot(my_i == ni);
        ns.t = shfl_d(my_t, own ? __ffsll((long long)own) - 1 : 0); ns.d = nd; ns.qx = 0.0; ns.qy = 0.0;
    }
    F1P_PPH();
#ifdef F1P_PRO_PHASES
    int lstat[4] = {0, 0, 0, 0};
    long long lat[5] = {0, 0, 0, 0, 0};
    if (!bad) wave_lookahead_centres(px, py, cfg, a.wx, a.wy, a.wpsi, a.n, (double)ni + ns.t, 0, 1, cen_x, cen_y, cen_psi, cen_ok, s_first[wave], s_pairs[wave], nd, lstat, a.wbox, F1P_MAX_LOOKAHEADS, lat);
    if (lane == 0 && mx.dbg_cost32) for (int k = 0; k < 4; ++k) mx.dbg_cost32[(size_t)e * nl * cfg.n_width + 40 + k] = (float)lstat[k];
    if (lane == 0 && mx.dbg_cost32) for (int k = 0; k < 4; ++k) mx.dbg_cost32[(size_t)e * nl * cfg.n_width + 48 + k] = (float)(lat[k + 1] - lat[k]);
#else
    if (!a.goals && !bad) wave_lookahead_centres(px, py, cfg, a.wx, a.wy, a.wpsi, a.n, (double)ni + ns.t, 0, 1, cen_x, cen_y, cen_psi, cen_ok, s_first[wave], s_pairs[wave], nd, nullptr, a.wbox, F1P_MAX_LOOKAHEADS);
#endif
    if (bad && lane < nl) cen_ok[lane] = 0;
    __builtin_amdgcn_s_waitcnt(0xc07f);
    __builtin_amdgcn_wave_barrier();
    F1P_PPH();
    sn_t = shfl_d(sn_t, 0); cs_t = shfl_d(cs_t, 0);
    bool disc_not_clear = false;
    if (mx.n_disc > 0 && mx.clear_bits) {
        const bool ncl = ego_disc_not_clear(a, mx, win, cs_t, sn_t, lane);
        disc_not_clear = __ballot(ncl) != 0ull;
    }
    if (a.prev_theta) {
#pragma unroll
        for (int m = 32; m >= 1; m >>= 1) { pm0 += shfl_xor_d(pm0, m); pm1 += shfl_xor_d(pm1, m); pm2 += shfl_xor_d(pm2, m); }
    }
    unsigned char* rec = recs + (size_t)e * ego_rec_stride(nl);
    double* r_cen = reinterpret_cast<double*>(rec + sizeof(EgoRecHdr));
    GoalFrame32* r_gf = reinterpret_cast<GoalFrame32*>(r_cen + 5 * (size_t)nl);
    if (lane < nl && !a.goals) {
        const int l = lane;
        GoalFrame32 g;
        g.cx = 0.0; g.cy = 0.0; g.nx = 0.0; g.ny = 0.0; g.gth = 0.f; g.ok = cen_ok[l];
        double cxv = 0.0, cyv = 0.0, sp = 0.0, cp = 1.0, gth64 = 0.0;
        if (g.ok) {
            cxv = cen_x[l]; cyv = cen_y[l];
            const double cpv = cen_psi[l];
            sincos_core(cpv, &sp, &cp);
            const double dx = cxv - px, dy = cyv - py;
            g.cx = cs_t * dx + sn_t * dy; g.cy = -sn_t * dx + cs_t * dy;
            g.nx = cs_t * (-sp) + sn_t * cp; g.ny = sn_t * sp + cs_t * cp;
            gth64 = remainder_2pi(cpv - theta);
            g.gth = (float)gth64;
        }
        __builtin_nontemporal_store(cxv, r_cen + l); __builtin_nontemporal_store(cyv, r_cen + nl + l); __builtin_nontemporal_store(sp, r_cen + 2 * nl + l);
        __builtin_nontemporal_store(cp, r_cen + 3 * nl + l); __builtin_nontemporal_store(gth64, r_cen + 4 * nl + l);
        {
            typedef double f1p_d2 __attribute__((ext_vector_type(2)));
            typedef int f1p_i2 __attribute__((ext_vector_type(2)));
            double* gd = reinterpret_cast<double*>(r_gf + l);
            __builtin_nontemporal_store((f1p_d2){g.cx, g.cy}, reinterpret_cast<f1p_d2*>(gd));
            __builtin_nontemporal_store((f1p_d2){g.nx, g.ny}, reinterpret_cast<f1p_d2*>(gd + 2));
            __builtin_nontemporal_store((f1p_i2){__float_as_int(g.gth), g.ok}, reinterpret_cast<f1p_i2*>(gd + 4));
        }
    }
    F1P_PPH();
    if (lane == 0) ego_record_write(a, cfg, mx, rec, e, S, sim_m, px, py, theta, cs_t, sn_t, win, pm0, pm1, pm2, disc_not_clear, ni);
    F1P_PPH();
#ifdef F1P_PRO_PHASES
    if (lane == 0 && mx.dbg_cost32) { for (int k = 0; k + 1 < npp; ++k) mx.dbg_cost32[(size_t)e * nl * cfg.n_width + 32 + k] = (float)(pph[k + 1] - pph[k]); mx.dbg_cost32[(size_t)e * nl * cfg.n_width + 31] = (float)(pph[0] & 0xffffff); }
#endif
}
#undef F1P_PPH


__device__ __forceinline__ int half_last_i32(int v, bool hi_half) {
    const int lo = __builtin_amdgcn_readlane(v, 31), hi = __builtin_amdgcn_readlane(v, 63);
    return hi_half ? hi : lo;
}
__device__ __forceinline__ int half_min_key(int v, bool hi_half) {
    v = min(v, __builtin_amdgcn_update_dpp(0x7fffffff, v, 0x111, 0xf, 0xf, false));
    v = min(v, __builtin_amdgcn_update_dpp(0x7fffffff, v, 0x112, 0xf, 0xf, false));
    v = min(v, __builtin_amdgcn_update_dpp(0x7fffffff, v, 0x114, 0xf, 0xf, false));
    v = min(v, __builtin_amdgcn_update_dpp(0x7fffffff, v, 0x118, 0xf, 0xf, false));
    v = min(v, __builtin_amdgcn_update_dpp(0x7fffffff, v, 0x142, 0xa, 0xf, false));
    return half_last_i32(v, hi_half);
}
__device__ __forceinline__ int half_scan_add_i32(int v) {
    v += __builtin_amdgcn_update_dpp(0, v, 0x111, 0xf, 0xf, false);
    v += __builtin_amdgcn_update_dpp(0, v, 0x112, 0xf, 0xf, false);
    v += __builtin_amdgcn_update_dpp(0, v, 0x114, 0xf, 0xf, false);
    v += __builtin_amdgcn_update_dpp(0, v, 0x118, 0xf, 0xf, false);
    v += __builtin_amdgcn_update_dpp(0, v, 0x142, 0xa, 0xf, false);
    return v;
}
__device__ __forceinline__ double readlane_d(double v, int src) {
    const long long b = __double_as_longlong(v);
    const int lo = __builtin_amdgcn_readlane((int)(b & 0xffffffffll), src), hi = __builtin_amdgcn_readlane((int)(b >> 32), src);
    return __longlong_as_double(((long long)hi << 32) | (long long)(unsigned int)lo);
}
__device__ __forceinline__ void half_argmin_dpp(double& d, int& i, bool hi_half) {
#define F1P_HALF_ARGMIN_STEP(CTRL, ROWS)                                                                                        \
    {                                                                                                                           \
        const long long b = __double_as_longlong(d);                                                                            \
        const int lo = (int)(b & 0xffffffffll), hi = (int)(b >> 32);                                                            \
        const int olo = __builtin_amdgcn_update_dpp(lo, lo, CTRL, ROWS, 0xf, false), ohi = __builtin_amdgcn_update_dpp(hi, hi, CTRL, ROWS, 0xf, false); \
        const int oi = __builtin_amdgcn_update_dpp(i, i, CTRL, ROWS, 0xf, false);                                               \
        const double od = __longlong_as_double(((long long)ohi << 32) | (long long)(unsigned int)olo);                          \
        if (argmin_better(od, oi, d, i)) { d = od; i = oi; }                                                                    \
    }
    F1P_HALF_ARGMIN_STEP(0x111, 0xf)
    F1P_HALF_ARGMIN_STEP(0x112, 0xf)
    F1P_HALF_ARGMIN_STEP(0x114, 0xf)
    F1P_HALF_ARGMIN_STEP(0x118, 0xf)
    F1P_HALF_ARGMIN_STEP(0x142, 0xa)
#undef F1P_HALF_ARGMIN_STEP
    const long long b = __double_as_longlong(d);
    const int lo = half_last_i32((int)(b & 0xffffffffll), hi_half), hi = half_last_i32((int)(b >> 32), hi_half);
    d = __longlong_as_double(((long long)hi << 32) | (long long)(unsigned int)lo);
    i = half_last_i32(i, hi_half);
}
__device__ __forceinline__ void half_argmin_2step(double& d, int& i, bool hi_half) {
    const int k = (d != d) ? (int)0x80000000 : f32_order_key((float)d);
    const int kmin = half_min_key(k, hi_half);
    const long long gap = (long long)k - (long long)kmin;
    const unsigned long long m = __ballot(gap <= 2ll);
    unsigned int m0 = (unsigned int)m, m1 = (unsigned int)(m >> 32);
    if (__builtin_popcount(m0) > 4 || __builtin_popcount(m1) > 4) { half_argmin_dpp(d, i, hi_half); return; }
    const long long b = __double_as_longlong(d);
    const int lo = (int)(b & 0xffffffffll), hi = (int)(b >> 32);
    double bd0 = __builtin_huge_val(), bd1 = __builtin_huge_val(); int bi0 = 0x7fffffff, bi1 = 0x7fffffff;
    while (m0) {
        const int src = __builtin_ctz(m0);
        m0 &= m0 - 1;
        const int olo = __builtin_amdgcn_readlane(lo, src), ohi = __builtin_amdgcn_readlane(hi, src), oi = __builtin_amdgcn_readlane(i, src);
        const double od = __longlong_as_double(((long long)ohi << 32) | (long long)(unsigned int)olo);
        if (argmin_better(od, oi, bd0, bi0)) { bd0 = od; bi0 = oi; }
    }
    while (m1) {
        const int src = 32 + __builtin_ctz(m1);
        m1 &= m1 - 1;
        const int olo = __builtin_amdgcn_readlane(lo, src), ohi = __builtin_amdgcn_readlane(hi, src), oi = __builtin_amdgcn_readlane(i, src);
        const double od = __longlong_as_double(((long long)ohi << 32) | (long long)(unsigned int)olo);
        if (argmin_better(od, oi, bd1, bi1)) { bd1 = od; bi1 = oi; }
    }
    d = hi_half ? bd1 : bd0; i = hi_half ? bi1 : bi0;
}

__global__ __launch_bounds__(256) void k_lattice_prologue2(LatticeArgs a, f1p_lattice_cfg cfg, MixArgs mx, unsigned char* __restrict__ recs) {
    __shared__ double s_seg[4][2][5][64];
    __shared__ int s_first[4][2][32];
    __shared__ int s_pairs[4][2][64];
    warm_kernargs<sizeof(LatticeArgs) + sizeof(f1p_lattice_cfg) + sizeof(MixArgs) + 8>();
    const int lane = threadIdx.x & 63, wave = threadIdx.x >> 6;
    const bool hh = lane >= 32;
    const int h = hh ? 1 : 0, hl = lane & 31, hbase = lane & 32;
    const int e_first = a.e0 + ((blockIdx.x * 4 + wave) << 1);
    if (e_first >= a.E) return;
    const bool valid = e_first + h < a.E;
    const int e = valid ? e_first + h : a.E - 1;
    const int nl = cfg.n_lookahead, S = cfg.n_stations, n = a.n;
    double (*seg)[64] = s_seg[wave][h];
    int* lds_first = s_first[wave][h];
    int* lds_pairs = s_pairs[wave][h];
    const double* __restrict__ wx = a.wx; const double* __restrict__ wy = a.wy;
#ifdef F1P_PRO2_PHASES
    long long pph[10], lat[5] = {0, 0, 0, 0, 0}; int npp = 0;
#define F1P_PPH() do { __builtin_amdgcn_s_waitcnt(0); pph[npp++] = clock64(); } while (0)
#define F1P_LAT(k) do { __builtin_amdgcn_s_waitcnt(0); lat[k] = clock64(); } while (0)
#else
#define F1P_PPH() do {} while (0)
#define F1P_LAT(k) do {} while (0)
#endif
    F1P_PPH();
    const int nseg = n - 1, nchunk = (nseg + 63) >> 6;
    double b0x = 0.0, b0X = 0.0, b0y = 0.0, b0Y = 0.0;
    if (hl < nchunk) { b0x = a.wbox[4 * hl]; b0X = a.wbox[4 * hl + 1]; b0y = a.wbox[4 * hl + 2]; b0Y = a.wbox[4 * hl + 3]; }
    int sj0 = hl * ((n + 63) >> 6), sj1 = (hl + 32) * ((n + 63) >> 6);
    if (sj0 > n - 1) sj0 = n - 1;
    if (sj1 > n - 1) sj1 = n - 1;
    const double smx0 = wx[sj0], smy0 = wy[sj0], smx1 = wx[sj1], smy1 = wy[sj1];
    const double px = a.poses[4 * e], py = a.poses[4 * e + 1], theta = a.poses[4 * e + 2];
    if (a.pose_copy && hl < 4 && valid) a.pose_copy[4 * e + hl] = a.poses[4 * e + hl];
    const int sim_m = S - cfg.n_shift - cfg.n_cull;
    double pm0 = 0.0, pm1 = 0.0, pm2 = 0.0;
    if (a.prev_theta) {
        const double* pv = a.prev_theta + (size_t)e * S + cfg.n_shift;
        for (int j = hl; j < sim_m; j += 32) {
            const double p = pv[j], fj = (double)j;
            pm0 = __builtin_fma(p, p, pm0); pm1 = __builtin_fma(fj, p, pm1); pm2 = __builtin_fma(fj * fj, p, pm2);
        }
    }
    const bool collide_on = cfg.check_collision && a.has_grid;
    const EgoWindow win = ego_window(a, mx, collide_on, px, py, hl == 0);
    double sn_t = 0.0, cs_t = 1.0;
    F1P_PPH();
    double nd = __builtin_huge_val(); int ni = 0x7fffffff; double my_t = 0.0;
    bool pm_done = false;
    {
        const double ex0 = px - smx0, ey0 = py - smy0, ex1 = px - smx1, ey1 = py - smy1;
        const double ub2_a = ex0 * ex0 + ey0 * ey0, ub2_b = ex1 * ex1 + ey1 * ey1;
        const double ub2_own = ub2_b < ub2_a ? ub2_b : ub2_a;
        const float ub2_up = (float)ub2_own * (1.0f + 2.4e-7f);
        const double ub2 = (double)f32_from_order_key(half_min_key(f32_order_key(ub2_up == ub2_up ? ub2_up : __builtin_nanf("")), hh));
        const double thr = ub2 * (1.0 + 1e-6) + 1e-9;
        for (int cb = 0; cb < nchunk; cb += 32) {
            const int c = cb + hl;
            bool keep = false;
            if (c < nchunk) {
                double xmin = b0x, xmax = b0X, ymin = b0y, ymax = b0Y;
                if (cb > 0) { xmin = a.wbox[4 * c]; xmax = a.wbox[4 * c + 1]; ymin = a.wbox[4 * c + 2]; ymax = a.wbox[4 * c + 3]; }
                const double dx = __builtin_fmax(__builtin_fmax(xmin - px, px - xmax), 0.0);
                const double dy = __builtin_fmax(__builtin_fmax(ymin - py, py - ymax), 0.0);
                keep = !(dx * dx + dy * dy > thr);
            }
            const unsigned long long m = __ballot(keep);
            unsigned int m0 = (unsigned int)m, m1 = (unsigned int)(m >> 32);
            bool first_trip = cb == 0;
            while (m0 | m1) {
                const int ca0 = m0 ? __builtin_ctz(m0) : -1, ca1 = m1 ? __builtin_ctz(m1) : -1;
                m0 &= m0 - 1; m1 &= m1 - 1;
                const int cc0 = m0 ? __builtin_ctz(m0) : -1, cc1 = m1 ? __builtin_ctz(m1) : -1;
                m0 &= m0 - 1; m1 &= m1 - 1;
                const int cmA = hh ? ca1 : ca0, cmB = hh ? cc1 : cc0;
                const bool anyB = (cc0 >= 0) | (cc1 >= 0);
                double sxv[4], syv[4], exv[4], eyv[4]; int iv[4]; bool onv[4];
#pragma unroll
                for (int u = 0; u < 4; ++u) {
                    const int cm = u < 2 ? cmA : cmB;
                    iv[u] = ((cb + cm) << 6) + (u & 1) * 32 + hl;
                    onv[u] = cm >= 0 && iv[u] < nseg;
                    sxv[u] = 0.0; syv[u] = 0.0; exv[u] = 0.0; eyv[u] = 0.0;
                }
#pragma unroll
                for (int u = 0; u < 2; ++u) if (onv[u]) { sxv[u] = wx[iv[u]]; syv[u] = wy[iv[u]]; exv[u] = wx[iv[u] + 1]; eyv[u] = wy[iv[u] + 1]; }
                if (anyB) {
#pragma unroll
                    for (int u = 2; u < 4; ++u) if (onv[u]) { sxv[u] = wx[iv[u]]; syv[u] = wy[iv[u]]; exv[u] = wx[iv[u] + 1]; eyv[u] = wy[iv[u] + 1]; }
                }
                if (first_trip && a.prev_theta) {
#pragma unroll
                    for (int mm = 16; mm >= 1; mm >>= 1) { pm0 += shfl_xor_d(pm0, mm); pm1 += shfl_xor_d(pm1, mm); pm2 += shfl_xor_d(pm2, mm); }
                    pm_done = true;
                }
                first_trip = false;
#pragma unroll
                for (int u = 0; u < 2; ++u) {
                    if (onv[u]) {
                        const SegProj sp_ = seg_project(px, py, sxv[u], syv[u], exv[u], eyv[u]);
                        if (argmin_better(sp_.d, iv[u], nd, ni)) { nd = sp_.d; ni = iv[u]; my_t = sp_.t; }
                    }
                }
                if (anyB) {
#pragma unroll
                    for (int u = 2; u < 4; ++u) {
                        if (onv[u]) {
                            const SegProj sp_ = seg_project(px, py, sxv[u], syv[u], exv[u], eyv[u]);
                            if (argmin_better(sp_.d, iv[u], nd, ni)) { nd = sp_.d; ni = iv[u]; my_t = sp_.t; }
                        }
                    }
                }
            }
        }
    }
    F1P_PPH();
    double ns_t;
    {
        const int my_i = ni;
        half_argmin_2step(nd, ni, hh);
        const unsigned long long ownm = __ballot(my_i == ni);
        const unsigned int own = hh ? (unsigned int)(ownm >> 32) : (unsigned int)ownm;
        ns_t = shfl_d(my_t, hbase + (own ? __builtin_ctz(own) : 0));
    }
    F1P_PPH();
    bool my_found = false;
    double c_x = 0.0, c_y = 0.0, c_psi = 0.0;
    if (!a.goals) {
        const double tstart = (double)ni + ns_t;
        const int start_i = (int)tstart;
        const double start_t = tstart - __builtin_trunc(tstart);
        bool fast = start_i >= 0 && start_i <= n - 2 && n > 130 && nl <= 32;
        const int nreg = n - 1 - start_i;
        F1P_LAT(0);
        const double my_r = hl < nl ? cfg.lookahead[hl] : 0.0;
        const float my_r32 = (float)my_r;
        const double wrap_ax = wx[n - 1], wrap_ay = wy[n - 1], wrap_bx = wx[0], wrap_by = wy[0];
        uint32_t mineA = 0u, mineB = 0u;
        {
            double rsx[2], rsy[2], rex[2], rey[2], rpsi[2];
#pragma unroll
            for (int u = 0; u < 2; ++u) {
                const int j = hl + 32 * u;
                const int vi = j < nreg ? start_i + j : j - nreg - 1;
                int i0 = vi < 0 ? vi + n : vi, i1 = vi + 1;
                i0 = i0 < 0 ? 0 : (i0 > n - 1 ? n - 1 : i0);
                i1 = i1 < 0 ? 0 : (i1 > n - 1 ? n - 1 : i1);
                rpsi[u] = a.wpsi[i0]; rsx[u] = wx[i0]; rsy[u] = wy[i0]; rex[u] = wx[i1]; rey[u] = wy[i1];
            }
            if (hl == 0) sincos(theta, &sn_t, &cs_t);
            typedef float f1p_v2 __attribute__((ext_vector_type(2)));
            f1p_v2 lo2, hi2; bool nan_seg[2];
#pragma unroll
            for (int u = 0; u < 2; ++u) {
                const int j = hl + 32 * u;
                const double sx = rsx[u], sy = rsy[u], ex = rex[u], ey = rey[u];
                seg[0][j] = sx; seg[1][j] = sy; seg[2][j] = ex; seg[3][j] = ey; seg[4][j] = rpsi[u];
// ... 159 lines not shown
```

f1tenth_planning_amd/csrc/k_lattice_refine.hip:

```cpp
#include "lattice_mixed.h"

namespace f1p {

template <int GS>
__device__ __forceinline__ double group_shr1(double v) {
    const long long b = __double_as_longlong(v);
    const int lo = (int)(b & 0xffffffffll), hi = (int)(b >> 32);
    constexpr int ctrl = GS == 16 ? 0x111 : 0x138;
    const int slo = __builtin_amdgcn_update_dpp(0, lo, ctrl, 0xf, 0xf, false), shi = __builtin_amdgcn_update_dpp(0, hi, ctrl, 0xf, 0xf, false);
    return __longlong_as_double(((long long)shi << 32) | (long long)(unsigned int)slo);
}

template <int GS, bool FOOT = false>
__global__ __launch_bounds__(256, 2) void k_lattice_refine(LatticeArgs a, f1p_lattice_cfg cfg, MixArgs mx) {
    extern __shared__ __align__(16) unsigned char lds_raw[];
    warm_kernargs<sizeof(LatticeArgs) + sizeof(f1p_lattice_cfg) + sizeof(MixArgs)>();
    constexpr int GPW = 64 / GS;
    const int tid = threadIdx.x, lane = tid & 63, wave = tid >> 6;
    const int gl = lane & (GS - 1), grp = lane / GS, gbase = lane & ~(GS - 1);
    const int S_arg = cfg.n_stations;
    if (mx.perm_fill) {
        const int np = F1P_MIX_OREG * mx.perm_rs;
        for (int i = (int)(blockIdx.x * blockDim.x) + tid; i < np; i += (int)(gridDim.x * blockDim.x)) mx.perm_fill[i] = 0;
        if (blockIdx.x == 0 && tid < 2 * F1P_MIX_OREG) mx.ocnt[tid * 32u] = 0u;
    }
    __shared__ double s_gl_wu[16][6];
    __shared__ double s_gl_x[16];
#ifdef F1P_MIX_PHASES
    long long rph[16]; int nrp = 0;
#define F1P_RPH() do { if (nrp < 15) rph[nrp++] = clock64(); } while (0)
#else
#define F1P_RPH() do {} while (0)
#endif
    F1P_RPH();
    const bool collide_on = cfg.check_collision && a.has_grid;
    const unsigned int ngroups_total = gridDim.x * (blockDim.x >> 6) * GPW;
    const unsigned int g0 = (blockIdx.x * (blockDim.x >> 6) + wave) * GPW + grp;
    const unsigned int sh = (g0 / GPW) % F1P_MIX_QSHARDS, lstride = ngroups_total / F1P_MIX_QSHARDS;
    const unsigned int li_first = (g0 / (GPW * F1P_MIX_QSHARDS)) * GPW + g0 % GPW;
    RefEntry r_first;
    r_first.ok = 0; r_first.e = 0; r_first.c = 0; r_first.gx = 0; r_first.gy = 0; r_first.gth = 0; r_first.cost = 0; r_first.k0 = 0; r_first.dk = 0; r_first.L = 0; r_first.pad = 0;
    unsigned int n = mx.qcount[sh * 32u];
    if (li_first < mx.q_shard_cap) r_first = mx.q[sh * mx.q_shard_cap + li_first];
    if (tid < 96) s_gl_wu[tid / 6][tid % 6] = c_gl_wu[tid / 6][tid % 6];
    else if (tid < 112) s_gl_x[tid - 96] = c_gl_x[tid - 96];
    __syncthreads();
    asm volatile("" : "+v"(n), "+v"(r_first.ok));
    for (unsigned int ib = 0, li = li_first; ; ib += ngroups_total, li += lstride) {
#ifdef F1P_MIX_REFINE_LICM
        const int S = S_arg;
#else
        int S = S_arg;
        asm volatile("" : "+s"(S));
#endif
        const int den = S - 1 > 1 ? S - 1 : 1;
        const int sim_m = S - cfg.n_shift - cfg.n_cull;
        double* ncs = reinterpret_cast<double*>(lds_raw) + (size_t)(wave * GPW + grp) * (64 + 4 * (size_t)S);
        double* nsn = ncs + 32;
        double* inc_x = nsn + 32;
        double* inc_y = inc_x + S;
        double* akv = inc_y + S;
        double* simv = akv + S;
        const unsigned int i = sh * mx.q_shard_cap + li;
        const bool live = li < n;
        if (!__any(live)) break;
        RefEntry r = r_first;
        if (ib != 0) {
            r.ok = 0; r.e = 0; r.c = 0; r.gx = 0; r.gy = 0; r.gth = 0; r.cost = 0; r.k0 = 0; r.dk = 0; r.L = 0; r.pad = 0;
            if (li < mx.q_shard_cap) r = mx.q[i];
        }
        if (!live) { r.ok = 0; r.e = a.e0; r.c = 0; }
        F1P_RPH();
        const bool work = live && r.ok != 0;
        const int e = r.e;
        const bool check_occ = collide_on && r.ok != -2;
        EgoXform xf = {};
        if (work && check_occ) xf = mx.xf[e];
        const double* prev = a.prev_theta ? a.prev_theta + (size_t)e * S : nullptr;
        double pv[4] = {0.0, 0.0, 0.0, 0.0};
        if (work && prev) {
#pragma unroll
            for (int k = 0; k < 4; ++k) { const int q = gl + k * GS; if (q < sim_m) pv[k] = prev[q + cfg.n_shift]; }
        }
        Clothoid cl;
        cl.ok = false; cl.k0 = 0; cl.dk = 0; cl.L = 0;
        G1State g;
        g.r = 0; g.phi0 = 0; g.delta = 0; g.A = 0;
        bool fitting = work && g1_begin(r.gx, r.gy, r.gth, g);
        F1P_RPH();
        double c0 = 0.0;
        bool ok = false;
        for (int it = 0; it < 20 && __any(fitting); ++it) {
            const double fa = g.A, fb = g.delta - g.A, fc = g.phi0;
            const double exc = fabs(fa) + fabs(fb);
            int off = 88, cnt = 32, panels = 1;
            if (exc <= 8.0) { off = 0; cnt = 16; }
            else if (exc <= 14.0) { off = 16; cnt = 20; }
            else if (exc <= 21.0) { off = 36; cnt = 24; }
            else if (exc <= 29.0) { off = 60; cnt = 28; }
            else if (!(exc <= 36.0)) {
                const double pn = __builtin_ceil(exc * (1.0 / 36.0));
                panels = pn <= 1024.0 ? (int)pn : 1024;
            }
            if (!fitting) { cnt = 0; panels = 1; }
            double acc = 0.0;
            const int k = gl < 6 ? gl : gl - 6;
            int max_panels = panels;
            if (__any(panels > 1)) {
#pragma unroll
                for (int m_ = 32; m_ >= 1; m_ >>= 1) { const int o = __shfl_xor(max_panels, m_, 64); max_panels = o > max_panels ? o : max_panels; }
            }
            if (max_panels == 1) {
                const bool rule16 = cnt == 16;
                for (int j = gl; j < cnt; j += GS) {
                    const double tau = rule16 ? s_gl_x[j] : c_gl_x[off + j];
                    const double ph = __builtin_fma(__builtin_fma(fa, tau, fb), tau, fc);
                    double sn, cs;
                    sincos_core(ph, &sn, &cs);
                    ncs[j] = cs; nsn[j] = sn;
                }
                __builtin_amdgcn_s_waitcnt(0xc07f);
                __builtin_amdgcn_wave_barrier();
#ifdef F1P_MIX_PHASES
                if (it == 0) F1P_RPH();
#endif
                if (gl < 12) {
                    const double* v = gl < 6 ? ncs : nsn;
                    if (rule16) {
                        double w[16], u[16];
#pragma unroll
                        for (int j = 0; j < 16; ++j) { w[j] = s_gl_wu[j][k]; u[j] = v[j]; }
#pragma unroll
                        for (int j = 0; j < 16; ++j) acc = __builtin_fma(w[j], u[j], acc);
                    } else {
                        for (int j0 = 0; j0 < cnt; j0 += 4) {
                            const double w0 = c_gl_wu[off + j0][k], w1 = c_gl_wu[off + j0 + 1][k], w2 = c_gl_wu[off + j0 + 2][k], w3 = c_gl_wu[off + j0 + 3][k];
                            const double u0 = v[j0], u1 = v[j0 + 1], u2 = v[j0 + 2], u3 = v[j0 + 3];
                            acc = __builtin_fma(w0, u0, acc); acc = __builtin_fma(w1, u1, acc); acc = __builtin_fma(w2, u2, acc); acc = __builtin_fma(w3, u3, acc);
                        }
                    }
                }
                __builtin_amdgcn_wave_barrier();
            } else {
                const double h = 1.0 / (double)panels;
                for (int p = 0; p < max_panels; ++p) {
                    const bool mine = fitting && p < panels;
                    if (mine && panels == 1) {
                        for (int j = gl; j < cnt; j += GS) {
                            const double tau = c_gl_x[off + j];
                            const double ph = __builtin_fma(__builtin_fma(fa, tau, fb), tau, fc);
                            double sn, cs;
                            sincos_core(ph, &sn, &cs);
                            ncs[j] = cs; nsn[j] = sn;
                        }
                    } else if (mine) {
                        const double t0 = (double)p * h;
                        for (int j = gl; j < cnt; j += GS) {
                            const double tau = __builtin_fma(h, c_gl_x[off + j], t0);
                            const double ph = __builtin_fma(__builtin_fma(fa, tau, fb), tau, fc);
                            double sn, cs;
                            sincos_core(ph, &sn, &cs);
                            const double w = h * c_gl_w[off + j];
                            ncs[j] = w * cs; nsn[j] = w * sn;
                            akv[j] = __builtin_fma(tau, tau, -tau);
                        }
                    }
                    __builtin_amdgcn_s_waitcnt(0xc07f);
                    __builtin_amdgcn_wave_barrier();
                    if (mine && gl < 12) {
                        const double* v = gl < 6 ? ncs : nsn;
                        if (panels == 1) {
                            for (int j = 0; j < cnt; ++j) acc = __builtin_fma(c_gl_wu[off + j][k], v[j], acc);
                        } else {
                            for (int j = 0; j < cnt; ++j) {
                                double t = v[j];
                                for (int q = 0; q < k; ++q) t *= akv[j];
                                acc += t;
                            }
                        }
                    }
                    __builtin_amdgcn_wave_barrier();
                }
            }
            FitMoments m;
#pragma unroll
            for (int q = 0; q < 6; ++q) { m.c[q] = shfl_d(acc, gbase + q); m.s[q] = shfl_d(acc, gbase + 6 + q); }
#ifdef F1P_MIX_PHASES
            if (it == 0) F1P_RPH();
#endif
            if (fitting) {
                const int st = g1_step(m, g, c0);
                if (st != 0) { fitting = false; ok = st > 0; }
            }
        }
        if (ok) cl = g1_finish(g, c0);
        F1P_RPH();
        double cost = __builtin_huge_val();
        const bool run = cl.ok;
        const double k0 = cl.k0, dk = cl.dk, L = run ? cl.L : 1.0;
        const double ds = L / (double)den;
        bool hit = false;
        const bool occ_pass = run && check_occ;
        const bool store_inc = run && mx.inc != nullptr && li < mx.inc_cap;
        const bool inc_pass = occ_pass || store_inc;
        double rix[4] = {0.0, 0.0, 0.0, 0.0}, riy[4] = {0.0, 0.0, 0.0, 0.0};
        if (__any(inc_pass)) {
            if (inc_pass) {
                const IntervalCoef ic = interval_setup(k0, dk, L, ds);
                const int per = (S - 1 + GS - 1) / GS, q0 = gl * per, q1 = q0 + per < S - 1 ? q0 + per : S - 1;
                if (!FOOT && per <= 4) {
#pragma unroll
                    for (int k = 0; k < 4; ++k) { rix[k] = 0.0; riy[k] = 0.0; }
                    if (q0 < q1) {
                        PieceState st = piece_state_at(k0, dk, ds, q0, ic);
#pragma unroll
                        for (int k = 0; k < 4; ++k) {
                            if (q0 + k < q1) interval_increment(k0, dk, (double)(q0 + k) * ds, (q0 + k) * ic.nsub, ic, st, rix[k], riy[k]);
                        }
                    }
                } else if (q0 < q1) {
                    PieceState st = piece_state_at(k0, dk, ds, q0, ic);
                    for (int q = q0; q < q1; ++q) {
                        double dx, dy;
                        interval_increment(k0, dk, (double)q * ds, q * ic.nsub, ic, st, dx, dy);
                        inc_x[q] = dx; inc_y[q] = dy;
                    }
                }
            }
            __builtin_amdgcn_s_waitcnt(0xc07f);
            __builtin_amdgcn_wave_barrier();
            F1P_RPH();
            double* gp = store_inc ? mx.inc + ((size_t)sh * mx.inc_cap + li) * 2 * (size_t)S : nullptr;
            double* pos_x = akv; double* pos_y = simv;
            if (inc_pass) {
                const int per = (S - 1 + GS - 1) / GS;
                if (gl == 0) { pos_x[0] = 0.0; pos_y[0] = 0.0; }
                if (!FOOT && per <= 4) {
                    const int nrounds = (S - 1 + per - 1) / per;
                    double xin = 0.0, yin = 0.0, xo = 0.0, yo = 0.0;
                    for (int t = 0; t < nrounds; ++t) {
                        xin = group_shr1<GS>(xo); yin = group_shr1<GS>(yo);
                        xo = xin; yo = yin;
#pragma unroll
                        for (int k = 0; k < 4; ++k) { xo += rix[k]; yo += riy[k]; }
                    }
                    double x = xin, y = yin;
                    const int q0 = gl * per;
#pragma unroll
                    for (int k = 0; k < 4; ++k) {
                        x += rix[k]; y += riy[k];
                        if (k < per && q0 + k < S - 1) { pos_x[q0 + k + 1] = x; pos_y[q0 + k + 1] = y; }
                    }
                } else {
                double x = 0.0, y = 0.0;
                int j0 = 0;
                for (; j0 + 8 <= S - 1; j0 += 8) {
                    double dx[8], dy[8], xs[8], ys[8];
#pragma unroll
                    for (int u = 0; u < 8; ++u) { dx[u] = inc_x[j0 + u]; dy[u] = inc_y[j0 + u]; }
#pragma unroll
                    for (int u = 0; u < 8; ++u) { x += dx[u]; y += dy[u]; xs[u] = x; ys[u] = y; }
                    if (gl == 0) {
#pragma unroll
                        for (int u = 0; u < 8; ++u) { pos_x[j0 + u + 1] = xs[u]; pos_y[j0 + u + 1] = ys[u]; }
                    }
                }
                for (; j0 < S - 1; ++j0) {
                    x += inc_x[j0]; y += inc_y[j0];
                    if (gl == 0) { pos_x[j0 + 1] = x; pos_y[j0 + 1] = y; }
                }
                }
            }
            __builtin_amdgcn_s_waitcnt(0xc07f);
            __builtin_amdgcn_wave_barrier();
            F1P_RPH();
            if (inc_pass) {
                constexpr int NSL = 4;
                for (int qb = 0; qb < S; qb += NSL * GS) {
                    double xs[NSL], ys[NSL];
#pragma unroll
                    for (int k = 0; k < NSL; ++k) { const int q = qb + k * GS + gl; xs[k] = q < S ? pos_x[q] : 0.0; ys[k] = q < S ? pos_y[q] : 0.0; }
                    auto cell = [&](double qx, double qy, uint32_t& word, int& bit) {
                        word = 0xffffffffu; bit = 0;
                        const double lxf = __builtin_floor(__builtin_fma(xf.txx, qx, __builtin_fma(xf.txy, qy, xf.tx0)));
                        const double lyf = __builtin_floor(__builtin_fma(xf.tyx, qx, __builtin_fma(xf.tyy, qy, xf.ty0)));
                        const double gxf = lxf + (double)xf.tile_gx0, gyf = lyf + (double)xf.tile_gy0;
                        if ((gxf >= 0.0) & (gxf < (double)a.grid.w) & (gyf >= 0.0) & (gyf < (double)a.grid.h)) {
                            const int cgx = (int)gxf, cgy = (int)gyf;
                            word = a.grid.bits[(size_t)cgy * a.grid.wwords + (cgx >> 5)];
                            bit = cgx & 31;
                        }
                    };
                    if (gp) {
#pragma unroll
                        for (int k = 0; k < NSL; ++k) { const int q = qb + k * GS + gl; if (q < S) { __builtin_nontemporal_store(xs[k], gp + q); __builtin_nontemporal_store(ys[k], gp + S + q); } }
                    }
                    if (!occ_pass) continue;
                    if (!FOOT || mx.n_disc == 0) {
                        uint32_t word[NSL]; int bit[NSL]; bool have[NSL];
#pragma unroll
                        for (int k = 0; k < NSL; ++k) {
                            have[k] = qb + k * GS + gl < S;
                            word[k] = 0u; bit[k] = 0;
                            if (have[k]) cell(xs[k], ys[k], word[k], bit[k]);
                        }
#pragma unroll
                        for (int k = 0; k < NSL; ++k) hit |= have[k] && ((word[k] >> bit[k]) & 1u);
                    } else {
#pragma unroll
                        for (int k = 0; k < NSL; ++k) {
                            const int q = qb + k * GS + gl;
                            if (q < S) {
                                const double sq = (double)q * ds;
                                const double th = sq * (k0 + 0.5 * sq * dk);
                                double sn_h, cs_h;
                                sincos_fast(th, &sn_h, &cs_h);
                                for (int d = 0; d < mx.n_disc; ++d) {
                                    const double o = mx.disc_off[d];
                                    uint32_t word; int bit;
                                    cell(xs[k] + o * cs_h, ys[k] + o * sn_h, word, bit);
                                    hit |= (word >> bit) & 1u;
                                }
                            }
                        }
                    }
                }
            }
            __builtin_amdgcn_s_waitcnt(0xc07f);
            __builtin_amdgcn_wave_barrier();
        }
        F1P_RPH();
        if (run) {
            for (int q = gl; q < S; q += GS) {
                const double s = (double)q * ds;
                akv[q] = fabs(k0 + dk * s);
                double sv = 0.0;
                if (prev && q < sim_m) {
                    const int kq = (q - gl) / GS;
                    const double pq = kq < 4 ? (kq == 0 ? pv[0] : (kq == 1 ? pv[1] : (kq == 2 ? pv[2] : pv[3]))) : prev[q + cfg.n_shift];
                    const double th = s * (k0 + 0.5 * s * dk); const double d = th - pq; sv = d * d;
                }
                simv[q] = sv;
            }
        }
        __builtin_amdgcn_s_waitcnt(0xc07f);
        __builtin_amdgcn_wave_barrier();
        F1P_RPH();
        const unsigned long long hm = __ballot(hit);
        const bool any_hit = ((hm >> gbase) & (GS == 64 ? ~0ull : (1ull << (GS & 63)) - 1ull)) != 0ull;
        if (run) {
            double sumk = 0.0, sim = 0.0;
            {
                int q = 0;
                for (; q + 8 <= S; q += 8) {
                    double v[8];
#pragma unroll
                    for (int u = 0; u < 8; ++u) v[u] = akv[q + u];
#pragma unroll
                    for (int u = 0; u < 8; ++u) sumk += v[u];
                }
                for (; q < S; ++q) sumk += akv[q];
            }
            if (prev) {
                int q = 0;
                for (; q + 8 <= sim_m; q += 8) {
                    double v[8];
#pragma unroll
                    for (int u = 0; u < 8; ++u) v[u] = simv[q + u];
#pragma unroll
                    for (int u = 0; u < 8; ++u) sim += v[u];
                }
                for (; q < sim_m; ++q) sim += simv[q];
            }
            const double maxk = __builtin_fmax(fabs(k0 + dk * (0.0 * ds)), fabs(k0 + dk * ((double)(S - 1) * ds)));
            cost = 0.0;
            cost += cfg.w_length * (1.0 / L);
            cost += cfg.w_max_kappa * maxk;
            cost += cfg.w_mean_kappa * (sumk / (double)S);
            cost += cfg.w_similarity * sim;
            if (any_hit) cost = __builtin_huge_val();
        }
        __builtin_amdgcn_wave_barrier();
        if (work && gl == 0) {
            RefEntry o = r;
            o.cost = cost; o.k0 = cl.k0; o.dk = cl.dk; o.L = cl.L; o.ok = cl.ok ? 1 : 0; o.pad = store_inc ? 1 : 0;
            mx.q[i] = o;
        }
#ifdef F1P_MIX_PHASES
        F1P_RPH();
        if (ib == 0 && live && gl == 0 && mx.dbg_state && (size_t)i * 16 + 16 <= (size_t)a.E * cfg.n_lookahead * cfg.n_width) {
            for (int k = 0; k + 1 < nrp; ++k) mx.dbg_state[(size_t)i * 16 + k] = (int)(rph[k + 1] - rph[k]);
            mx.dbg_state[(size_t)i * 16 + 15] = nrp;
        }
#endif
    }
}

template <int GS, bool FOOT = false>
__global__ __launch_bounds__(256, 2) void k_lattice_refine_cubic(LatticeArgs a, f1p_lattice_cfg cfg, MixArgs mx) {
    extern __shared__ __align__(16) unsigned char lds_raw[];
    warm_kernargs<sizeof(LatticeArgs) + sizeof(f1p_lattice_cfg) + sizeof(MixArgs)>();
    constexpr int GPW = 64 / GS;
    const int tid = threadIdx.x, lane = tid & 63, wave = tid >> 6;
    const int gl = lane & (GS - 1), grp = lane / GS, gbase = lane & ~(GS - 1);
    const int S = cfg.n_stations;
    if (mx.perm_fill) {
        const int np = F1P_MIX_OREG * mx.perm_rs;
        for (int i = (int)(blockIdx.x * blockDim.x) + tid; i < np; i += (int)(gridDim.x * blockDim.x)) mx.perm_fill[i] = 0;
        if (blockIdx.x == 0 && tid < 2 * F1P_MIX_OREG) mx.ocnt[tid * 32u] = 0u;
    }
    const bool collide_on = cfg.check_collision && a.has_grid;
    const unsigned int ngroups_total = gridDim.x * (blockDim.x >> 6) * GPW;
    const unsigned int g0 = (blockIdx.x * (blockDim.x >> 6) + wave) * GPW + grp;
    const unsigned int sh = (g0 / GPW) % F1P_MIX_QSHARDS, lstride = ngroups_total / F1P_MIX_QSHARDS;
    const unsigned int li_first = (g0 / (GPW * F1P_MIX_QSHARDS)) * GPW + g0 % GPW;
    const unsigned int n = mx.qcount[sh * 32u];
    const int den = S - 1 > 1 ? S - 1 : 1;
    const int sim_m = S - cfg.n_shift - cfg.n_cull;
    double* px = reinterpret_cast<double*>(lds_raw) + (size_t)(wave * GPW + grp) * 5 * (size_t)S;
    double* py = px + S;
    double* chv = py + S;
    double* akv = chv + S;
    double* simv = akv + S;
    for (unsigned int li = li_first; ; li += lstride) {
        const bool live = li < n;
        if (!__any(live)) break;
        const unsigned int i = sh * mx.q_shard_cap + li;
        RefEntry r;
        r.ok = 0; r.e = a.e0; r.c = 0; r.gx = 0; r.gy = 0; r.gth = 0; r.cost = 0; r.k0 = 0; r.dk = 0; r.L = 0; r.pad = 0;
        if (live) r = mx.q[i];
        const bool work = live && r.ok != 0;
        const int e = r.e;
        const bool check_occ = collide_on && r.ok != -2;
        EgoXform xf = {};
        if (work && check_occ) xf = mx.xf[e];
        const double* prev = a.prev_theta ? a.prev_theta + (size_t)e * S : nullptr;
        Cubic cq = cubic_setup(r.gx, r.gy, r.gth);
        const bool run = work && cq.ok;
        bool hit = false;
        double maxk = 0.0;
        for (int q = gl; q < S; q += GS) {
            double x = 0.0, y = 0.0, th = 0.0, ak = 0.0;
            if (run) cubic_row(cq, (double)q / (double)den, x, y, th, ak);
            px[q] = x; py[q] = y; akv[q] = ak;
            double sv = 0.0;
            if (run && prev && q < sim_m) { const double d = th - prev[q + cfg.n_shift]; sv = d * d; }
            simv[q] = sv;
            maxk = __builtin_fmax(maxk, ak);
            if (run && check_occ) {
                auto occupied = [&](double qx, double qy) -> bool {
                    uint32_t word = 0xffffffffu; int bit = 0;
                    const double lxf = __builtin_floor(__builtin_fma(xf.txx, qx, __builtin_fma(xf.txy, qy, xf.tx0)));
                    const double lyf = __builtin_floor(__builtin_fma(xf.tyx, qx, __builtin_fma(xf.tyy, qy, xf.ty0)));
                    const double gxf = lxf + (double)xf.tile_gx0, gyf = lyf + (double)xf.tile_gy0;
                    if ((gxf >= 0.0) & (gxf < (double)a.grid.w) & (gyf >= 0.0) & (gyf < (double)a.grid.h)) {
                        const int cgx = (int)gxf, cgy = (int)gyf;
                        word = a.grid.bits[(size_t)cgy * a.grid.wwords + (cgx >> 5)];
                        bit = cgx & 31;
                    }
                    return ((word >> bit) & 1u) != 0u;
                };
                if (!FOOT || mx.n_disc == 0) hit |= occupied(x, y);
                else {
                    double sn_h, cs_h;
                    sincos_fast(th, &sn_h, &cs_h);
                    for (int d = 0; d < mx.n_disc; ++d) {
                        const double o = mx.disc_off[d];
                        hit |= occupied(x + o * cs_h, y + o * sn_h);
                    }
                }
            }
        }
        __builtin_amdgcn_s_waitcnt(0xc07f);
        __builtin_amdgcn_wave_barrier();
        for (int q = gl; q < S; q += GS) {
            double ch = 0.0;
            if (q > 0) { const double ddx = px[q] - px[q - 1], ddy = py[q] - py[q - 1]; ch = __builtin_sqrt(ddx * ddx + ddy * ddy); }
            chv[q] = ch;
        }
        __builtin_amdgcn_s_waitcnt(0xc07f);
        __builtin_amdgcn_wave_barrier();
        double acc = 0.0;
        {
            const double* arr = gl == 0 ? chv : (gl == 1 ? akv : simv);
            const int cnt = gl == 2 ? (sim_m > 0 ? sim_m : 0) : S;
            int q = 0;
            for (; q + 8 <= S; q += 8) {
                double v[8];
#pragma unroll
                for (int u = 0; u < 8; ++u) v[u] = arr[q + u];
#pragma unroll
                for (int u = 0; u < 8; ++u) acc += (q + u < cnt) ? v[u] : 0.0;
            }
            for (; q < S; ++q) acc += q < cnt ? arr[q] : 0.0;
        }
#pragma unroll
        for (int m_ = GS / 2; m_ >= 1; m_ >>= 1) maxk = __builtin_fmax(maxk, shfl_xor_d(maxk, m_));
        const double len = shfl_d(acc, gbase), sumk = shfl_d(acc, gbase + 1), sim = shfl_d(acc, gbase + 2);
        const unsigned long long hm = __ballot(hit);
        const bool any_hit = ((hm >> gbase) & (GS == 64 ? ~0ull : (1ull << (GS & 63)) - 1ull)) != 0ull;
        double cost = __builtin_huge_val();
        if (run) {
            cost = 0.0;
            cost += cfg.w_length * (1.0 / len);
            cost += cfg.w_max_kappa * maxk;
            cost += cfg.w_mean_kappa * (sumk / (double)S);
            cost += cfg.w_similarity * (prev ? sim : 0.0);
            if (any_hit) cost = __builtin_huge_val();
        }
        __builtin_amdgcn_wave_barrier();
        if (work && gl == 0) {
            RefEntry o = r;
            o.cost = cost; o.k0 = r.gx; o.dk = r.gy; o.L = r.gth; o.ok = run ? 1 : 0; o.pad = 0;
            mx.q[i] = o;
        }
    }
}

bool mixed_refine_fits(f1p_ctx* ctx, int lanes, bool foot, size_t lds) {
    if (lanes == 16) return foot ? lds_fits(ctx, (k_lattice_refine<16, true>), lds) : lds_fits(ctx, k_lattice_refine<16>, lds);
    return foot ? lds_fits(ctx, (k_lattice_refine<64, true>), lds) : lds_fits(ctx, k_lattice_refine<64>, lds);
}

bool mixed_refine_cubic_fits(f1p_ctx* ctx, size_t lds) {
    return lds_fits(ctx, k_lattice_refine_cubic<16>, lds) && lds_fits(ctx, (k_lattice_refine_cubic<16, true>), lds);
}

void mixed_launch_refine(bool cubic, int lanes, bool foot, unsigned grid, size_t lds, hipStream_t st, const LatticeArgs& a, const f1p_lattice_cfg& cfg, const MixArgs& mx) {
    const dim3 g(grid), b(256);
    if (cubic && foot) hipLaunchKernelGGL((k_lattice_refine_cubic<16, true>), g, b, lds, st, a, cfg, mx);
    else if (cubic) hipLaunchKernelGGL(k_lattice_refine_cubic<16>, g, b, lds, st, a, cfg, mx);
    else if (lanes == 16) {
        if (foot) hipLaunchKernelGGL((k_lattice_refine<16, true>), g, b, lds, st, a, cfg, mx);
        else hipLaunchKernelGGL(k_lattice_refine<16>, g, b, lds, st, a, cfg, mx);
    } else {
        if (foot) hipLaunchKernelGGL((k_lattice_refine<64, true>), g, b, lds, st, a, cfg, mx);
        else hipLaunchKernelGGL(k_lattice_refine<64>, g, b, lds, st, a, cfg, mx);
    }
}

}
```

f1tenth_planning_amd/csrc/lattice_device.h:

```cpp
#pragma once
#include <type_traits>

#include "f1p_internal.h"
#include "tracker_device.h"

#ifndef F1P_K3_UNROLL
#define F1P_K3_UNROLL 2
#endif
#ifndef F1P_FIT_INLINE
#define F1P_FIT_INLINE __noinline__
#endif
#ifndef F1P_SETUP_INLINE
#define F1P_SETUP_INLINE __forceinline__
#endif
#ifndef F1P_STATION_INLINE
#define F1P_STATION_INLINE __forceinline__
#endif
#ifndef F1P_K3_WAVES_STAGE
#define F1P_K3_WAVES_STAGE 3
#endif
#ifndef F1P_K3_WAVES_STAGE2
#define F1P_K3_WAVES_STAGE2 2
#endif
#ifndef F1P_STAGE_T
// ... 669 lines not shown
    const int32_t* track_id;
    const int4* track_tab;
    int track_K;
};

__device__ __forceinline__ bool lattice_bind_track(LatticeArgs& a, int e) {
    TrackSetDev ts;
    ts.x = a.wx; ts.y = a.wy; ts.v = a.wv; ts.psi = a.wpsi; ts.kappa = nullptr; ts.box = a.wbox; ts.tab = a.track_tab; ts.K = a.track_K;
    TrackView tv;
    if (!track_of(ts, a.track_id, e, tv)) return false;
    a.wx = tv.x; a.wy = tv.y; a.wv = tv.v; a.wpsi = tv.psi; a.wbox = tv.box; a.n = tv.n;
    return true;
}

__device__ __forceinline__ void lattice_bad_track(const LatticeArgs& a, const f1p_lattice_cfg& cfg, int e, int i0, int step) {
    const int S = cfg.n_stations;
    if (i0 == 0) {
        a.steer[e] = __builtin_nan(""); a.speed[e] = __builtin_nan("");
        if (a.best_idx) a.best_idx[e] = -1;
        if (a.best_cost) a.best_cost[e] = __builtin_nan("");
        if (a.status) a.status[e] = F1P_ST_BAD_TRACK;
        if (a.near_idx) a.near_idx[e] = -1;
    }
    for (int i = i0; i < 4 * S; i += step) {
        if (a.best_traj) a.best_traj[(size_t)e * S * 4 + i] = 0.0;
        if (a.best_traj32) a.best_traj32[(size_t)e * S * 4 + i] = 0.f;
    }
    if (a.theta_out) for (int i = i0; i < S; i += step) a.theta_out[(size_t)e * S + i] = 0.0;
    const int C = cfg.n_lookahead * cfg.n_width;
    if (a.all_cost) for (int c = i0; c < C; c += step) a.all_cost[(size_t)e * C + c] = __builtin_nan("");
    if (a.all_traj) for (size_t i = i0; i < (size_t)C * S * 4; i += step) a.all_traj[(size_t)e * C * S * 4 + i] = 0.0;
}

__device__ __forceinline__ bool candidate_goal(const LatticeArgs& a, const f1p_lattice_cfg& cfg, int e, int c, int C,
                                               const volatile EgoParams* ep,
                                               const double* cen_x, const double* cen_y, const double* cen_psi,
                                               const int* cen_ok, double& gx, double& gy, double& gth) {
    if (a.goals) {
        const double* g = a.goals + ((size_t)e * C + c) * 3;
        gx = g[0]; gy = g[1]; gth = g[2];
        return isfinite(gx) && isfinite(gy) && isfinite(gth);
    }
    const int l = c / cfg.n_width, k = c - l * cfg.n_width;
    if (!cen_ok[l]) { gx = 0.0; gy = 0.0; gth = 0.0; return false; }
    const double psi = cen_psi[l];
    const double w = cfg.width[k];
    double sp, cp;
    sincos_core(psi, &sp, &cp);
    const double mx = cen_x[l] + w * (-sp);
    const double my = cen_y[l] + w * cp;
    const double dx = mx - ep->px, dy = my - ep->py;
    const double ct = ep->ct, st = ep->st;
    gx = ct * dx + st * dy;
    gy = -st * dx + ct * dy;
    gth = remainder_2pi(psi - ep->theta);
    return true;
}

template <int GEN, bool HAVE_INC = false>
__device__ __forceinline__ void emit_and_track(const LatticeArgs& a, const f1p_lattice_cfg& cfg, int e, int lane, int ni, int den,
                                               const Clothoid& cl, double bc, double* tr_x, double* tr_y, double* inc_x, double* inc_y,
                                               long long* stamps = nullptr, const double* v_near = nullptr) {
    const int S = cfg.n_stations;
    double* bt = a.best_traj ? a.best_traj + (size_t)e * S * 4 : nullptr;
    float4* bt32 = a.best_traj32 ? reinterpret_cast<float4*>(a.best_traj32) + (size_t)e * S : nullptr;
    double* tho = a.theta_out ? a.theta_out + (size_t)e * S : nullptr;
    if (GEN == F1P_GEN_CUBIC) {
        const Cubic cq = cubic_setup(cl.k0, cl.dk, cl.L);
        for (int i = lane; i < S; i += 64) {
            double x = 0.0, y = 0.0, th = 0.0, ak = 0.0;
            if (cl.ok) cubic_row(cq, (double)i / (double)den, x, y, th, ak);
            tr_x[i] = x; tr_y[i] = y;
            if (bt) {
                reinterpret_cast<double2*>(bt)[2 * i] = make_double2(x, y);
                reinterpret_cast<double2*>(bt)[2 * i + 1] = make_double2(th, ak);
            }
            if (bt32) bt32[i] = make_float4((float)x, (float)y, (float)th, (float)ak);
            if (tho) tho[i] = th;
        }
    } else {
        const double ds = cl.ok ? cl.L / (double)den : 0.0;
        if (!HAVE_INC || !cl.ok) {
            IntervalCoef ic;
            if (cl.ok) ic = interval_setup(cl.k0, cl.dk, cl.L, ds);
            for (int i = lane; i < S - 1; i += 64) {
                double dx = 0.0, dy = 0.0;
                if (cl.ok) {
                    PieceState st = piece_state_at(cl.k0, cl.dk, ds, i, ic);
                    interval_increment(cl.k0, cl.dk, (double)i * ds, i * ic.nsub, ic, st, dx, dy);
                }
                inc_x[i] = dx; inc_y[i] = dy;
            }
        }
        __builtin_amdgcn_s_waitcnt(0xc07f);
        __builtin_amdgcn_wave_barrier();
        if (stamps) stamps[0] = clock64();
        for (int i = lane; i < S; i += 64) {
            double x = 0.0, y = 0.0;
            if (HAVE_INC && cl.ok) { x = tr_x[i]; y = tr_y[i]; }
            else {
                for (int j = 0; j < i; ++j) { x += inc_x[j]; y += inc_y[j]; }
                tr_x[i] = x; tr_y[i] = y;
            }
            if (bt || bt32 || tho) {
                const double s = (double)i * ds;
                const double th = cl.ok ? s * (cl.k0 + 0.5 * s * cl.dk) : 0.0;
                const double ak = cl.ok ? fabs(cl.k0 + cl.dk * s) : 0.0;
                if (bt) {
                    typedef double f1p_d2 __attribute__((ext_vector_type(2)));
                    if (a.traj_in_hbm) {
                        __builtin_nontemporal_store((f1p_d2){x, y}, reinterpret_cast<f1p_d2*>(bt) + 2 * i);
                        __builtin_nontemporal_store((f1p_d2){th, ak}, reinterpret_cast<f1p_d2*>(bt) + 2 * i + 1);
                    } else {
                        reinterpret_cast<double2*>(bt)[2 * i] = make_double2(x, y);
                        reinterpret_cast<double2*>(bt)[2 * i + 1] = make_double2(th, ak);
                    }
                }
                if (bt32) bt32[i] = make_float4((float)x, (float)y, (float)th, (float)ak);
                if (tho) __builtin_nontemporal_store(th, tho + i);
            }
        }
    }
    __builtin_amdgcn_s_waitcnt(0xc07f);
    __builtin_amdgcn_wave_barrier();
    if (stamps) stamps[1] = clock64();

    Track o;
    o.steer = 0.0; o.speed = 0.0; o.la_idx = F1P_LA_NONE; o.status = F1P_ST_ALL_BLOCKED;
    if (cl.ok && bc < __builtin_huge_val()) {
        bool plain = true;
        for (int i = lane; i < S - 1; i += 64) {
            const double ax = tr_x[i], ay = tr_y[i], dx = tr_x[i + 1] - ax, dy = tr_y[i + 1] - ay;
            const double l2 = dx * dx + dy * dy;
            plain &= (l2 > 0.0) & (l2 < __builtin_huge_val()) & (fabs(ax) < __builtin_huge_val()) & (fabs(ay) < __builtin_huge_val());
        }
        plain = __all(plain) && tr_x[0] == 0.0 && tr_y[0] == 0.0 && S >= 2;
        double td = 0.0, tt = 0.0; int ti = 0;
        if (!plain) {
            nearest_scan(0.0, 0.0, tr_x, tr_y, S, lane, 64, td, ti);
            wave_argmin(td, ti);
            const SegProj ts = seg_project(0.0, 0.0, tr_x[ti], tr_y[ti], tr_x[ti + 1], tr_y[ti + 1]);
            tt = ts.t; td = ts.d;
        }
        o = wave_pursuit(0.0, 0.0, 0.0, cfg.track_lookahead, cfg.wheelbase, cfg.max_reacquire, tr_x, tr_y, nullptr,
                         v_near ? *v_near : a.wv[ni], S, ti, tt, td);
    }
    if (lane == 0) {
        a.steer[e] = o.steer;
        a.speed[e] = o.speed;
        if (a.status) a.status[e] = o.status;
    }
}

template <typename K>
static bool lds_fits(f1p_ctx* ctx, K kernel, size_t bytes) {
    if (bytes <= (size_t)ctx->prop.sharedMemPerBlock) return true;
    if (bytes > (size_t)ctx->prop.maxSharedMemoryPerMultiProcessor) return false;
    if (hipFuncSetAttribute(reinterpret_cast<const void*>(kernel), hipFuncAttributeMaxDynamicSharedMemorySize, (int)bytes) != hipSuccess) {
        (void)hipGetLastError();
        return false;
    }
    return true;
}

int launch_lattice_mixed(f1p_ctx* ctx, LatticeArgs& a, const f1p_lattice_cfg* cfg, int mode, int E, bool foot, bool cubic,
                         double* d_pose_copy, bool* handled);

}
```

f1tenth_planning_amd/csrc/lattice_mixed.h:

```cpp
#pragma once
#include "lattice_device.h"

namespace f1p {

#ifndef F1P_MIX_MIN_EGOS_V3
#define F1P_MIX_MIN_EGOS_V3 1
#endif
#ifndef F1P_MIX_MARGIN_REL
#define F1P_MIX_MARGIN_REL 3.0e-5f
#endif
#ifndef F1P_MIX_MARGIN_ABS
#define F1P_MIX_MARGIN_ABS 1.0e-6f
#endif
#ifndef F1P_MIX_MACRO
#define F1P_MIX_MACRO 1
#endif
#ifndef F1P_MIX_INC_PER_EGO
#define F1P_MIX_INC_PER_EGO 4
#endif
#ifndef F1P_MIX_EXC_MAX
#define F1P_MIX_EXC_MAX 20.0f
#endif
#ifndef F1P_MIX_LOOKAHEAD_PAIRS
#define F1P_MIX_LOOKAHEAD_PAIRS 1
#endif
#ifndef F1P_MIX_FILTER_BLOCK
#define F1P_MIX_FILTER_BLOCK 256
#endif
#ifndef F1P_MIX_FILTER_WAVES
#define F1P_MIX_FILTER_WAVES 8
#endif
#ifndef F1P_MIX_FIT_UNROLL
#define F1P_MIX_FIT_UNROLL 4
#endif
#ifndef F1P_MIX_COOP_MAX
#define F1P_MIX_COOP_MAX 4
#endif
#ifndef F1P_MIX_COOP_MAX_X
#define F1P_MIX_COOP_MAX_X 24
#endif
#ifndef F1P_MIX_OREG
#define F1P_MIX_OREG 64
#endif
#ifndef F1P_MIX_HEAVY_MEMORY
#define F1P_MIX_HEAVY_MEMORY 16
#endif
#ifndef F1P_MIX_ORDER_MIN_EGOS
#define F1P_MIX_ORDER_MIN_EGOS 1024
#endif
#ifndef F1P_MIX_ROUNDS
#define F1P_MIX_ROUNDS 10
#endif
#ifndef F1P_F3_CONTRACT
#define F1P_F3_CONTRACT 1
#endif
#if F1P_F3_CONTRACT
#define F1P_F32_CONTRACT _Pragma("clang fp contract(fast)")
#else
#define F1P_F32_CONTRACT
#endif
#ifndef F1P_F3_FIT_PAIRS
#define F1P_F3_FIT_PAIRS 1
#endif
#ifndef F1P_F3_RAW_SQRT
#define F1P_F3_RAW_SQRT 1
#endif
#ifndef F1P_F3_FAST_ATAN
#define F1P_F3_FAST_ATAN 1
#endif
#ifndef F1P_MIX_F3_EGOS_PER_WG
#define F1P_MIX_F3_EGOS_PER_WG 1
#endif
#ifndef F1P_PIPE_CHUNKS
#define F1P_PIPE_CHUNKS 1
#endif
#ifndef F1P_PIPE_MIN_EGOS
#define F1P_PIPE_MIN_EGOS 2048
#endif
#ifndef F1P_MIX_EDGE0
#define F1P_MIX_EDGE0 2.0e-4f
#endif
#ifndef F1P_MIX_EDGE1
#define F1P_MIX_EDGE1 8.0e-6f
#endif
#ifndef F1P_MIX_QSHARDS
#define F1P_MIX_QSHARDS 8
#endif
#ifndef F1P_MIX_REFINE_WG_PER_CU
#define F1P_MIX_REFINE_WG_PER_CU 4
#endif
#ifndef F1P_PRO2
#define F1P_PRO2 1
#endif
#ifndef F1P_PRO2_MIN_EGOS
#define F1P_PRO2_MIN_EGOS 3072
#endif
#define F1P_ST_FREE 0
#define F1P_ST_HIT 1
#define F1P_ST_UNSURE 2
#define F1P_ST_BAD 3
#define F1P_ST_PENDING 4
#define F1P_ST_PENDING2 5
#define F1P_INV_2PI_F 0.15915494309189535f

struct RefEntry {
    int32_t e, c;
    double gx, gy, gth;
    double cost, k0, dk, L;
    int32_t ok, pad;
};

struct EgoXform { double txx, txy, tx0, tyx, tyy, ty0; int tile_gx0, tile_gy0; };


struct MixArgs {
    unsigned int* qcount;
    unsigned int q_shard_cap;
    double* inc;
    unsigned int inc_cap;
    RefEntry* q;
    int32_t* ego_base;
    int32_t* ego_n;
    int32_t* ego_ni;
    struct EgoXform* xf;
    const uint32_t* clear_bits;
    int clear_r;
    float clear_ds_cap;
    int n_disc;
    double disc_off[4];
    float disc_off_f[4], disc_omax_f;
    double sim_s2, sim_s3, sim_s4;
    float margin_rel, margin_abs;
    float edge0, edge1;
    float* dbg_bound;
    float* dbg_cost32;
    int32_t* dbg_state;
    int32_t* perm;
    int32_t* perm_fill;
    unsigned int* ocnt;
    unsigned char* heavy;
    int perm_rs;
    int32_t* dbg_pass;
};

struct GoalFrame32 { double cx, cy, nx, ny; float gth; int ok; };

__device__ __forceinline__ int cvt_flr_i32_f32(float v) {
    int r;
    asm("v_cvt_flr_i32_f32 %0, %1" : "=v"(r) : "v"(v));
    return r;
}

struct EgoParamsF2 {
    float txx, txy, tx0, tyx, tyy, ty0;
    float w_len, w_maxk, w_meank, w_sim;
    float margin_rel, margin_abs, edge0, edge1;
    float clear_ds_cap, inv_den, inv_S, fS;
    float cells_per_m, sqrt_S;
    float inv_nw, pad0;
    const double* prev;
    double M0, M1, M2;
    int tile_w, tile_h;
    int tile_gx0, tile_gy0;
    int S, sim_m, n_shift;
    int exact_all;
};

struct CubicTab { float h10, h01, h11, pad0, d10, d01, d11, pad1, e10, e01, e11, pad2; };

struct EgoRecHdr {
    double px, py, theta, ct, st;
    EgoParamsF2 p;
};
static_assert(sizeof(EgoRecHdr) % 8 == 0, "record header must keep the fp64 arrays aligned");

__host__ __device__ inline size_t ego_rec_stride(int nl) { return (sizeof(EgoRecHdr) + (size_t)nl * (40 + sizeof(GoalFrame32)) + 15) & ~(size_t)15; }

void mixed_launch_prologue(bool two_per_wave, bool tracks, int egos, hipStream_t st, const LatticeArgs& a, const f1p_lattice_cfg& cfg, const MixArgs& mx, unsigned char* recs);
bool mixed_filter3_fits(f1p_ctx* ctx, int cr, bool foot, bool cubic, size_t lds);
void mixed_launch_filter3(int cr, bool hooks, bool host_goals, bool cubic, bool foot, unsigned grid, size_t lds, hipStream_t st, const LatticeArgs& a,
                          const f1p_lattice_cfg& cfg, const MixArgs& mx, const unsigned char* recs);
bool mixed_refine_fits(f1p_ctx* ctx, int lanes, bool foot, size_t lds);
bool mixed_refine_cubic_fits(f1p_ctx* ctx, size_t lds);
void mixed_launch_refine(bool cubic, int lanes, bool foot, unsigned grid, size_t lds, hipStream_t st, const LatticeArgs& a, const f1p_lattice_cfg& cfg, const MixArgs& mx);
bool mixed_select_fits(f1p_ctx* ctx, bool cubic, size_t lds, bool tracks = false);
void mixed_launch_select(bool cubic, bool tracks, unsigned grid, size_t lds, hipStream_t st, const LatticeArgs& a, const f1p_lattice_cfg& cfg, const MixArgs& mx);

}
```

Baseline: 750.5 billion.

## Fuse refine and select into one tail kernel with per-ego completion counters

```diff
diff --git a/f1tenth_planning_amd/csrc/f1p_device.h b/f1tenth_planning_amd/csrc/f1p_device.h
--- a/f1tenth_planning_amd/csrc/f1p_device.h
+++ b/f1tenth_planning_amd/csrc/f1p_device.h
@@ -353,6 +353,79 @@
     return o;
 }
 
+template <int GS>
+__device__ __forceinline__ unsigned long long group_ballot(bool p, int gbase) {
+    return (__ballot(p) >> gbase) & (GS == 64 ? ~0ull : (1ull << (GS & 63)) - 1ull);
+}
+
+template <int GS>
+__device__ __forceinline__ Intersect group_intersect(bool act, double px, double py, double radius, const double* wx, const double* wy,
+                                                     int n, double tstart, bool wrap) {
+    const int lane = threadIdx.x & 63, gl = lane & (GS - 1), gbase = lane & ~(GS - 1);
+    const int start_i = (int)tstart;
+    const double start_t = tstart - __builtin_trunc(tstart);
+    Intersect r;
+    r.found = false; r.i = 0; r.t = 0.0; r.x = 0.0; r.y = 0.0;
+    bool scanning = act;
+    for (int base = start_i; ; base += GS) {
+        const bool go = scanning && base < n - 1;
+        if (!__any(go)) break;
+        const int i = base + gl;
+        SegHit h;
+        h.hit = false; h.t = 0; h.x = 0; h.y = 0;
+        if (go && i < n - 1) h = seg_hit(px, py, radius, wx[i], wy[i], wx[i + 1], wy[i + 1], i == start_i, start_t);
+        const unsigned long long m = group_ballot<GS>(h.hit, gbase);
+        const int first = m ? __ffsll((long long)m) - 1 : 0;
+        const double ht = shfl_d(h.t, gbase + first), hx = shfl_d(h.x, gbase + first), hy = shfl_d(h.y, gbase + first);
+        if (go && m) { r.found = true; r.i = base + first; r.t = ht; r.x = hx; r.y = hy; scanning = false; }
+    }
+    scanning = act && wrap && !r.found;
+    for (int base = -1; ; base += GS) {
+        const bool go = scanning && base < start_i;
+        if (!__any(go)) break;
+        const int i = base + gl;
+        SegHit h;
+        h.hit = false; h.t = 0; h.x = 0; h.y = 0;
+        if (go && i < start_i) {
+            const int i0 = i < 0 ? i + n : i;
+            int i1 = i + 1; if (i1 >= n) i1 -= n;
+            h = seg_hit(px, py, radius, wx[i0], wy[i0], wx[i1], wy[i1], false, 0.0);
+        }
+        const unsigned long long m = group_ballot<GS>(h.hit, gbase);
+        const int first = m ? __ffsll((long long)m) - 1 : 0;
+        const double ht = shfl_d(h.t, gbase + first), hx = shfl_d(h.x, gbase + first), hy = shfl_d(h.y, gbase + first);
+        if (go && m) { r.found = true; r.i = base + first; r.t = ht; r.x = hx; r.y = hy; scanning = false; }
+    }
+    return r;
+}
+
+template <int GS>
+__device__ __forceinline__ Track group_pursuit(bool act, double px, double py, double theta, double lookahead, double wheelbase,
+                                               double max_reacquire, const double* wx, const double* wy, double v_const, int n,
+                                               int near_i, double near_t, double near_d) {
+    Track o;
+    o.steer = 0.0; o.speed = 0.0; o.la_idx = F1P_LA_NONE; o.status = F1P_ST_NO_LOOKAHEAD;
+    const bool inter = act && near_d < lookahead;
+    const Intersect it = group_intersect<GS>(inter, px, py, lookahead, wx, wy, n, (double)near_i + near_t, true);
+    double cx = 0.0, cy = 0.0;
+    bool steer_to = false;
+    if (inter) {
+        if (it.found) {
+            o.la_idx = it.i;
+            const int r = it.i < 0 ? it.i + n : it.i;
+            cx = wx[r]; cy = wy[r];
+            o.status = F1P_ST_INTERSECT;
+            steer_to = true;
+        }
+    } else if (act && near_d < max_reacquire) {
+        cx = wx[near_i]; cy = wy[near_i];
+        o.status = F1P_ST_REACQUIRE;
+        steer_to = true;
+    }
+    if (steer_to) get_actuation(theta, cx, cy, v_const, px, py, lookahead, wheelbase, o.speed, o.steer);
+    return o;
+}
+
 struct GridDev {
     const uint32_t* bits;
     int32_t w, h, wwords;
diff --git a/f1tenth_planning_amd/csrc/f1p_internal.h b/f1tenth_planning_amd/csrc/f1p_internal.h
--- a/f1tenth_planning_amd/csrc/f1p_internal.h
+++ b/f1tenth_planning_amd/csrc/f1p_internal.h
@@ -111,6 +111,7 @@
     size_t order_bytes = 0;
     int order_E = 0;
     bool order_valid = false;
+    int order_cur = 0;
     int lattice_order = 1;
     bool step_chain = false;
     bool mix_q_dirty_prev = false;
diff --git a/f1tenth_planning_amd/csrc/f1p_lattice.hip b/f1tenth_planning_amd/csrc/f1p_lattice.hip
--- a/f1tenth_planning_amd/csrc/f1p_lattice.hip
+++ b/f1tenth_planning_amd/csrc/f1p_lattice.hip
@@ -414,7 +414,7 @@
 
 int f1p_lattice_set_mode(f1p_ctx* ctx, int32_t mixed, float* d_cost32, int32_t* d_state) {
     if (!ctx) return F1P_EINVAL;
-    if (mixed < 0 || mixed > 3) return set_error(ctx, F1P_EINVAL, "mixed must be 0 (all fp64), 1 (f32 filter, the default), 2 (f32 filter at any batch size) or 3 (as 2, one ego per wave in the per-ego kernels)");
+    if (mixed < 0 || mixed > 3) return set_error(ctx, F1P_EINVAL, "mixed must be 0 (all fp64), 1 (f32 filter, the default), 2 (f32 filter at any batch size) or 3 (as 2, one ego per wave in the prologue and separate refinement / selection kernels)");
     ctx->lattice_mixed = mixed;
     ctx->d_dbg_lat_cost32 = d_cost32;
     ctx->d_dbg_lat_state = d_state;
diff --git a/f1tenth_planning_amd/csrc/k_lattice_filter3.hip b/f1tenth_planning_amd/csrc/k_lattice_filter3.hip
--- a/f1tenth_planning_amd/csrc/k_lattice_filter3.hip
+++ b/f1tenth_planning_amd/csrc/k_lattice_filter3.hip
@@ -1016,6 +1016,7 @@
         const unsigned int base = sh * mx.q_shard_cap + atomicAdd(&mx.qcount[sh * 32u], (unsigned int)n);
         cnt[1] = (int)base;
         mx.ego_base[e] = (int)base; mx.ego_n[e] = n;
+        mx.ego_done[e] = 0u;
         if (mx.heavy) { const int h = mx.heavy[e]; mx.heavy[e] = (unsigned char)(rounds_run >= 2 ? F1P_MIX_HEAVY_MEMORY : (h > 0 ? h - 1 : 0)); }
     }
     double g1x = 0.0, g1y = 0.0, g1th = 0.0;
diff --git a/f1tenth_planning_amd/csrc/k_lattice_mixed.hip b/f1tenth_planning_amd/csrc/k_lattice_mixed.hip
--- a/f1tenth_planning_amd/csrc/k_lattice_mixed.hip
+++ b/f1tenth_planning_amd/csrc/k_lattice_mixed.hip
@@ -110,6 +110,16 @@
         const bool groups16 = mixed_refine_fits(ctx, 16, foot, lds_r16 + lds_r_static);
         const bool refine_fits = groups16 || mixed_refine_fits(ctx, 64, foot, lds_r64 + lds_r_static);
         const bool tracks = a.track_id != nullptr;
+        const size_t lds_t16 = sizeof(double) * 16 * (64 + 6 * (size_t)S), lds_t64 = sizeof(double) * 4 * (64 + 6 * (size_t)S);
+        bool fused = F1P_MIX_FUSED_TAIL && !cubic && !tracks && ctx->lattice_mixed != 3;
+#ifdef F1P_MIX_PHASES
+        fused = false;
+#endif
+        bool tail16 = false;
+        if (fused) {
+            tail16 = mixed_tail_fits(ctx, 16, foot, lds_t16 + lds_r_static);
+            fused = tail16 || mixed_tail_fits(ctx, 64, foot, lds_t64 + lds_r_static);
+        }
         if (refine_fits && mixed_select_fits(ctx, false, lds_s, tracks)) {
             MixArgs mx;
             mx.margin_rel = F1P_MIX_MARGIN_REL; mx.margin_abs = F1P_MIX_MARGIN_ABS; mx.edge0 = F1P_MIX_EDGE0; mx.edge1 = F1P_MIX_EDGE1;
@@ -156,7 +166,7 @@
             if (inc_cap > shard_cap) inc_cap = shard_cap;
             const size_t inc_block = 2 * (size_t)(S > 0 ? S : 1) * sizeof(double);
             const size_t inc_bytes = F1P_MIX_INC_PER_EGO > 0 ? inc_cap * F1P_MIX_QSHARDS * inc_block : 0;
-            const size_t need = qc_bytes + sizeof(int32_t) * 3 * (size_t)E + 256 + sizeof(EgoXform) * (size_t)E + 256 + sizeof(RefEntry) * region * nch + 256 + inc_bytes * nch;
+            const size_t need = qc_bytes + sizeof(int32_t) * 4 * (size_t)E + 256 + sizeof(EgoXform) * (size_t)E + 256 + sizeof(RefEntry) * region * nch + 256 + inc_bytes * nch;
             bool fresh = false;
             if (need > ctx->mix_scratch_bytes) {
                 fresh = true;
@@ -171,7 +181,8 @@
             mx.q_shard_cap = (unsigned int)shard_cap;
             mx.ego_base = reinterpret_cast<int32_t*>(ctx->d_mix_scratch + qc_bytes);
             mx.ego_n = mx.ego_base + E; mx.ego_ni = mx.ego_n + E;
-            const size_t xf_off = (qc_bytes + sizeof(int32_t) * 3 * (size_t)E + 255) & ~(size_t)255;
+            mx.ego_done = reinterpret_cast<unsigned int*>(mx.ego_ni + E);
+            const size_t xf_off = (qc_bytes + sizeof(int32_t) * 4 * (size_t)E + 255) & ~(size_t)255;
             mx.xf = reinterpret_cast<EgoXform*>(ctx->d_mix_scratch + xf_off);
             mx.q = reinterpret_cast<RefEntry*>(ctx->d_mix_scratch + ((xf_off + sizeof(EgoXform) * (size_t)E + 255) & ~(size_t)255));
             {
@@ -197,7 +208,7 @@
             if (nch == 1 && E >= F1P_MIX_ORDER_MIN_EGOS && F1P_MIX_F3_EGOS_PER_WG == 1 && ctx->lattice_order) {
                 const int rs = (E + F1P_MIX_OREG - 1) / F1P_MIX_OREG;
                 const size_t perm_bytes = (sizeof(int32_t) * (size_t)F1P_MIX_OREG * rs + 255) & ~(size_t)255, ocnt_bytes = sizeof(unsigned int) * 64 * F1P_MIX_OREG;
-                const size_t need_o = perm_bytes + ocnt_bytes + (size_t)E;
+                const size_t need_o = 2 * (perm_bytes + ocnt_bytes) + (size_t)E;
                 if (need_o > ctx->order_bytes || ctx->order_E != E) {
                     if (need_o > ctx->order_bytes) {
                         F1P_HIP(ctx, hipStreamSynchronize(ctx->stream));
@@ -207,12 +218,14 @@
                         ctx->order_bytes = need_o;
                     }
                     F1P_HIP(ctx, hipMemsetAsync(ctx->d_order, 0, need_o, ctx->stream));
-                    ctx->order_E = E; ctx->order_valid = false;
+                    ctx->order_E = E; ctx->order_valid = false; ctx->order_cur = 0;
                 } else if (fresh || ctx->mix_q_dirty_prev) ctx->order_valid = false;
-                mx.perm = ctx->order_valid ? reinterpret_cast<int32_t*>(ctx->d_order) : nullptr;
-                mx.perm_fill = reinterpret_cast<int32_t*>(ctx->d_order);
-                mx.ocnt = reinterpret_cast<unsigned int*>(ctx->d_order + perm_bytes);
-                mx.heavy = reinterpret_cast<unsigned char*>(ctx->d_order + perm_bytes + ocnt_bytes);
+                char* const ob_cur = ctx->d_order + (size_t)ctx->order_cur * (perm_bytes + ocnt_bytes);
+                char* const ob_next = ctx->d_order + (size_t)(1 - ctx->order_cur) * (perm_bytes + ocnt_bytes);
+                mx.perm = ctx->order_valid ? reinterpret_cast<int32_t*>(ob_cur) : nullptr;
+                mx.perm_fill = reinterpret_cast<int32_t*>(ob_next);
+                mx.ocnt = reinterpret_cast<unsigned int*>(ob_next + perm_bytes);
+                mx.heavy = reinterpret_cast<unsigned char*>(ctx->d_order + 2 * (perm_bytes + ocnt_bytes));
                 mx.perm_rs = rs;
             }
             if (nch > 1) {
@@ -258,12 +271,24 @@
                 if (rb > rb_max) rb = rb_max;
                 rb = rb & ~(size_t)15;
                 if (rb < 16) rb = 16;
-                mixed_launch_refine(cubic, groups16 ? 16 : 64, mk.n_disc > 0, (unsigned)rb, cubic ? lds_rc : (groups16 ? lds_r16 : lds_r64), st, ak, *cfg, mk);
-                if ((rc = check_hip(ctx, hipGetLastError(), "k_lattice_refine launch"))) break;
-                if (prof) F1P_HIP(ctx, hipEventRecord(ctx->ev_prof[3], st));
-                mixed_launch_select(cubic, tracks, (unsigned)((Ek + 3) / 4 + (mk.perm_fill ? (Ek + 255) / 256 : 0)), lds_s, st, ak, *cfg, mk);
-                rc = check_hip(ctx, hipGetLastError(), "k_lattice_select launch");
-                if (mk.perm_fill) ctx->order_valid = rc == F1P_OK;
+                if (fused) {
+                    const size_t rbt_max = (size_t)cus * (tail16 ? F1P_MIX_REFINE_WG_PER_CU : 8) / (nch > 1 ? 2 : 1);
+                    size_t rbt = (region + 3) / 4;
+                    rbt = (rbt + 15) & ~(size_t)15;
+                    if (rbt > rbt_max) rbt = rbt_max;
+                    rbt = rbt & ~(size_t)15;
+                    if (rbt < 16) rbt = 16;
+                    mixed_launch_tail(tail16 ? 16 : 64, mk.n_disc > 0, (unsigned)rbt, mk.perm_fill ? (unsigned)((Ek + 255) / 256) : 0u, tail16 ? lds_t16 : lds_t64, st, ak, *cfg, mk);
+                    rc = check_hip(ctx, hipGetLastError(), "k_lattice_tail launch");
+                    if (prof && rc == F1P_OK) F1P_HIP(ctx, hipEventRecord(ctx->ev_prof[3], st));
+                } else {
+                    mixed_launch_refine(cubic, groups16 ? 16 : 64, mk.n_disc > 0, (unsigned)rb, cubic ? lds_rc : (groups16 ? lds_r16 : lds_r64), st, ak, *cfg, mk);
+                    if ((rc = check_hip(ctx, hipGetLastError(), "k_lattice_refine launch"))) break;
+                    if (prof) F1P_HIP(ctx, hipEventRecord(ctx->ev_prof[3], st));
+                    mixed_launch_select(cubic, tracks, (unsigned)((Ek + 3) / 4 + (mk.perm_fill ? (Ek + 255) / 256 : 0)), lds_s, st, ak, *cfg, mk);
+                    rc = check_hip(ctx, hipGetLastError(), "k_lattice_select launch");
+                }
+                if (mk.perm_fill) { ctx->order_valid = rc == F1P_OK; if (rc == F1P_OK) ctx->order_cur = 1 - ctx->order_cur; }
             }
             if (nch > 1) {
                 F1P_HIP(ctx, hipEventRecord(ctx->ev_pipe[1], ctx->pipe_stream[0]));
diff --git a/f1tenth_planning_amd/csrc/k_lattice_prologue.hip b/f1tenth_planning_amd/csrc/k_lattice_prologue.hip
--- a/f1tenth_planning_amd/csrc/k_lattice_prologue.hip
+++ b/f1tenth_planning_amd/csrc/k_lattice_prologue.hip
@@ -270,6 +270,7 @@
     __shared__ int s_first[4][F1P_MAX_LOOKAHEADS];
     __shared__ int s_pairs[4][64];
     warm_kernargs<sizeof(LatticeArgs) + sizeof(f1p_lattice_cfg) + sizeof(MixArgs) + 8>();
+    mixed_rearm(mx);
     const int lane = threadIdx.x & 63, wave = threadIdx.x >> 6;
     const int e = a.e0 + blockIdx.x * 4 + wave;
     if (e >= a.E) return;
@@ -456,6 +457,7 @@
     __shared__ int s_first[4][2][32];
     __shared__ int s_pairs[4][2][64];
     warm_kernargs<sizeof(LatticeArgs) + sizeof(f1p_lattice_cfg) + sizeof(MixArgs) + 8>();
+    mixed_rearm(mx);
     const int lane = threadIdx.x & 63, wave = threadIdx.x >> 6;
     const bool hh = lane >= 32;
     const int h = hh ? 1 : 0, hl = lane & 31, hbase = lane & 32;
diff --git a/f1tenth_planning_amd/csrc/k_lattice_refine.hip b/f1tenth_planning_amd/csrc/k_lattice_refine.hip
--- a/f1tenth_planning_amd/csrc/k_lattice_refine.hip
+++ b/f1tenth_planning_amd/csrc/k_lattice_refine.hip
@@ -11,15 +11,83 @@
     return __longlong_as_double(((long long)shi << 32) | (long long)(unsigned int)slo);
 }
 
-template <int GS, bool FOOT = false>
-__global__ __launch_bounds__(256, 2) void k_lattice_refine(LatticeArgs a, f1p_lattice_cfg cfg, MixArgs mx) {
-    extern __shared__ __align__(16) unsigned char lds_raw[];
-    warm_kernargs<sizeof(LatticeArgs) + sizeof(f1p_lattice_cfg) + sizeof(MixArgs)>();
+typedef __attribute__((address_space(1))) unsigned long long f1p_gu64;
+typedef __attribute__((address_space(1))) unsigned int f1p_gu32;
+__device__ __forceinline__ void tail_publish64(void* p, unsigned long long v) {
+    __hip_atomic_store((f1p_gu64*)(unsigned long long*)p, v, __ATOMIC_RELAXED, __HIP_MEMORY_SCOPE_AGENT);
+}
+__device__ __forceinline__ void tail_publish(double* p, double v) { tail_publish64(p, (unsigned long long)__double_as_longlong(v)); }
+__device__ __forceinline__ unsigned long long tail_ld64(const void* p) {
+    return __hip_atomic_load((f1p_gu64*)(unsigned long long*)const_cast<void*>(p), __ATOMIC_RELAXED, __HIP_MEMORY_SCOPE_AGENT);
+}
+__device__ __forceinline__ double tail_ld(const double* p) { return __longlong_as_double((long long)tail_ld64(p)); }
+static_assert(sizeof(RefEntry) == 72, "k_lattice_tail publishes a RefEntry as nine 8-byte words");
+
+__device__ __forceinline__ double readlane_d(double v, int src_lane) {
+    const long long b = __double_as_longlong(v);
+    const int lo = __builtin_amdgcn_readlane((int)(b & 0xffffffffll), src_lane), hi = __builtin_amdgcn_readlane((int)(b >> 32), src_lane);
+    return __longlong_as_double(((long long)hi << 32) | (long long)(unsigned int)lo);
+}
+
+__device__ __forceinline__ void tail_select_wave(const LatticeArgs& a, const f1p_lattice_cfg& cfg, const MixArgs& mx, int e, int lane, double* wl) {
+    const int S = cfg.n_stations;
+    double* tr_x = wl; double* tr_y = tr_x + S; double* inc_x = tr_y + S; double* inc_y = inc_x + S;
+    const int base = mx.ego_base[e], n = mx.ego_n[e], ni = mx.ego_ni[e];
+    const double v_near = a.wv[ni];
+    const int c0 = cfg.cand_begin;
+    double bc = __builtin_huge_val(); int bi = 0x7fffffff, bslot = -1;
+    for (int j = lane; j < n; j += 64) {
+        const RefEntry* q = mx.q + base + j;
+        const double cost = __longlong_as_double((long long)tail_ld64(&q->cost));
+        const int c = (int)(tail_ld64(q) >> 32);
+        if (argmin_better(cost, c, bc, bi)) { bc = cost; bi = c; bslot = base + j; }
+    }
+    {
+        double d = bc; int i = bi;
+        wave_argmin_2step(d, i);
+        const unsigned long long m = __ballot((bi == i) & (bslot >= 0));
+        bslot = __shfl(bslot, m ? __ffsll((long long)m) - 1 : 0, 64);
+        bc = d; bi = i;
+    }
+    if (!(bc < __builtin_huge_val()) && !(bc != bc)) {
+        bi = c0; bslot = -1;
+        for (int j = lane; j < n; j += 64) if ((int)(tail_ld64(mx.q + base + j) >> 32) == c0) bslot = base + j;
+        const unsigned long long m = __ballot(bslot >= 0);
+        bslot = m ? __shfl(bslot, __ffsll((long long)m) - 1, 64) : -1;
+    }
+    Clothoid cl;
+    cl.ok = false; cl.k0 = 0; cl.dk = 0; cl.L = 0;
+    bool have_inc = false;
+    if (bslot >= 0) {
+        const RefEntry* q = mx.q + bslot;
+        cl.k0 = __longlong_as_double((long long)tail_ld64(&q->k0)); cl.dk = __longlong_as_double((long long)tail_ld64(&q->dk));
+        cl.L = __longlong_as_double((long long)tail_ld64(&q->L));
+        const unsigned long long op = tail_ld64(&q->ok);
+        cl.ok = (int)(op & 0xffffffffull) == 1;
+        have_inc = cl.ok && (int)(op >> 32) == 1 && mx.inc != nullptr;
+    }
+    if (lane == 0) {
+        if (a.best_idx) a.best_idx[e] = bi;
+        if (a.best_cost) a.best_cost[e] = bc;
+        if (a.near_idx) a.near_idx[e] = ni;
+    }
+    if (a.mode == LATTICE_EVAL) return;
+    const int den = S - 1 > 1 ? S - 1 : 1;
+    if (have_inc) {
+        const unsigned int sh = (unsigned int)bslot / mx.q_shard_cap, li = (unsigned int)bslot - sh * mx.q_shard_cap;
+        const double* gp = mx.inc + ((size_t)sh * mx.inc_cap + li) * 2 * (size_t)S;
+        for (int i = lane; i < S; i += 64) { tr_x[i] = tail_ld(gp + i); tr_y[i] = tail_ld(gp + S + i); }
+        emit_and_track<F1P_GEN_CLOTHOID, true>(a, cfg, e, lane, ni, den, cl, bc, tr_x, tr_y, inc_x, inc_y, nullptr, &v_near);
+    } else emit_and_track<F1P_GEN_CLOTHOID>(a, cfg, e, lane, ni, den, cl, bc, tr_x, tr_y, inc_x, inc_y, nullptr, &v_near);
+}
+
+template <int GS, bool FOOT, bool TAIL>
+__device__ __forceinline__ void lattice_refine_body(const LatticeArgs& a, const f1p_lattice_cfg& cfg, const MixArgs& mx, unsigned char* lds_raw, const unsigned int nwg) {
     constexpr int GPW = 64 / GS;
     const int tid = threadIdx.x, lane = tid & 63, wave = tid >> 6;
     const int gl = lane & (GS - 1), grp = lane / GS, gbase = lane & ~(GS - 1);
     const int S_arg = cfg.n_stations;
-    if (mx.perm_fill) {
+    if (!TAIL && mx.perm_fill) {
         const int np = F1P_MIX_OREG * mx.perm_rs;
         for (int i = (int)(blockIdx.x * blockDim.x) + tid; i < np; i += (int)(gridDim.x * blockDim.x)) mx.perm_fill[i] = 0;
         if (blockIdx.x == 0 && tid < 2 * F1P_MIX_OREG) mx.ocnt[tid * 32u] = 0u;
@@ -34,7 +102,7 @@
 #endif
     F1P_RPH();
     const bool collide_on = cfg.check_collision && a.has_grid;
-    const unsigned int ngroups_total = gridDim.x * (blockDim.x >> 6) * GPW;
+    const unsigned int ngroups_total = nwg * (blockDim.x >> 6) * GPW;
     const unsigned int g0 = (blockIdx.x * (blockDim.x >> 6) + wave) * GPW + grp;
     const unsigned int sh = (g0 / GPW) % F1P_MIX_QSHARDS, lstride = ngroups_total / F1P_MIX_QSHARDS;
     const unsigned int li_first = (g0 / (GPW * F1P_MIX_QSHARDS)) * GPW + g0 % GPW;
@@ -55,12 +123,14 @@
 #endif
         const int den = S - 1 > 1 ? S - 1 : 1;
         const int sim_m = S - cfg.n_shift - cfg.n_cull;
-        double* ncs = reinterpret_cast<double*>(lds_raw) + (size_t)(wave * GPW + grp) * (64 + 4 * (size_t)S);
+        const size_t gstride = 64 + (TAIL ? 6 : 4) * (size_t)S;
+        double* ncs = reinterpret_cast<double*>(lds_raw) + (size_t)(wave * GPW + grp) * gstride;
         double* nsn = ncs + 32;
         double* inc_x = nsn + 32;
         double* inc_y = inc_x + S;
         double* akv = inc_y + S;
         double* simv = akv + S;
+        double* pos_x = TAIL ? simv + S : akv; double* pos_y = TAIL ? simv + 2 * S : simv;
         const unsigned int i = sh * mx.q_shard_cap + li;
         const bool live = li < n;
         if (!__any(live)) break;
@@ -74,6 +144,8 @@
         const bool work = live && r.ok != 0;
         const int e = r.e;
         const bool check_occ = collide_on && r.ok != -2;
+        int ego_first = 0, ego_cnt = 0, ego_near = 0;
+        if (TAIL) { ego_first = mx.ego_base[e] - (int)(sh * mx.q_shard_cap); ego_cnt = mx.ego_n[e]; }
         EgoXform xf = {};
         if (work && check_occ) xf = mx.xf[e];
         const double* prev = a.prev_theta ? a.prev_theta + (size_t)e * S : nullptr;
@@ -195,14 +267,17 @@
         }
         if (ok) cl = g1_finish(g, c0);
         F1P_RPH();
+        const int wave_li0 = (int)li - grp;
+        const bool inside = TAIL && live && ego_first >= wave_li0 && ego_first + ego_cnt <= wave_li0 + GPW;
+        const bool fin = inside && (int)li == ego_first;
         double cost = __builtin_huge_val();
         const bool run = cl.ok;
         const double k0 = cl.k0, dk = cl.dk, L = run ? cl.L : 1.0;
         const double ds = L / (double)den;
         bool hit = false;
         const bool occ_pass = run && check_occ;
-        const bool store_inc = run && mx.inc != nullptr && li < mx.inc_cap;
-        const bool inc_pass = occ_pass || store_inc;
+        const bool store_inc = run && mx.inc != nullptr && li < mx.inc_cap && !(TAIL && inside);
+        const bool inc_pass = occ_pass || store_inc || (TAIL && run);
         double rix[4] = {0.0, 0.0, 0.0, 0.0}, riy[4] = {0.0, 0.0, 0.0, 0.0};
         if (__any(inc_pass)) {
             if (inc_pass) {
@@ -231,7 +306,6 @@
             __builtin_amdgcn_wave_barrier();
             F1P_RPH();
             double* gp = store_inc ? mx.inc + ((size_t)sh * mx.inc_cap + li) * 2 * (size_t)S : nullptr;
-            double* pos_x = akv; double* pos_y = simv;
             if (inc_pass) {
                 const int per = (S - 1 + GS - 1) / GS;
                 if (gl == 0) { pos_x[0] = 0.0; pos_y[0] = 0.0; }
@@ -293,7 +367,13 @@
                     };
                     if (gp) {
 #pragma unroll
-                        for (int k = 0; k < NSL; ++k) { const int q = qb + k * GS + gl; if (q < S) { __builtin_nontemporal_store(xs[k], gp + q); __builtin_nontemporal_store(ys[k], gp + S + q); } }
+                        for (int k = 0; k < NSL; ++k) {
+                            const int q = qb + k * GS + gl;
+                            if (q < S) {
+                                if (TAIL) { tail_publish(gp + q, xs[k]); tail_publish(gp + S + q, ys[k]); }
+                                else { __builtin_nontemporal_store(xs[k], gp + q); __builtin_nontemporal_store(ys[k], gp + S + q); }
+                            }
+                        }
                     }
                     if (!occ_pass) continue;
                     if (!FOOT || mx.n_disc == 0) {
@@ -330,6 +410,8 @@
             __builtin_amdgcn_wave_barrier();
         }
         F1P_RPH();
+        double v_near = 0.0;
+        if (TAIL && fin) { ego_near = mx.ego_ni[e]; v_near = a.wv[ego_near]; }
         if (run) {
             for (int q = gl; q < S; q += GS) {
                 const double s = (double)q * ds;
@@ -381,10 +463,69 @@
             if (any_hit) cost = __builtin_huge_val();
         }
         __builtin_amdgcn_wave_barrier();
-        if (work && gl == 0) {
+        if (!TAIL && work && gl == 0) {
             RefEntry o = r;
             o.cost = cost; o.k0 = cl.k0; o.dk = cl.dk; o.L = cl.L; o.ok = cl.ok ? 1 : 0; o.pad = store_inc ? 1 : 0;
             mx.q[i] = o;
+        }
+        if constexpr (TAIL) {
+            const double rec_cost = cost, rec_k0 = cl.k0, rec_dk = cl.dk, rec_L = cl.L;
+            const int rec_ok = cl.ok ? 1 : 0;
+            const bool far = live && !inside;
+            if (far && work && gl == 0) {
+                unsigned long long* qw = reinterpret_cast<unsigned long long*>(mx.q + i);
+                tail_publish64(qw + 4, (unsigned long long)__double_as_longlong(cost)); tail_publish64(qw + 5, (unsigned long long)__double_as_longlong(cl.k0));
+                tail_publish64(qw + 6, (unsigned long long)__double_as_longlong(cl.dk)); tail_publish64(qw + 7, (unsigned long long)__double_as_longlong(cl.L));
+                tail_publish64(qw + 8, (unsigned long long)(unsigned int)rec_ok | ((unsigned long long)(store_inc ? 1u : 0u) << 32));
+            }
+            {
+                const unsigned long long live_m = __ballot(live);
+                const int c0 = cfg.cand_begin;
+                double bc = __builtin_huge_val(); int bi = 0x7fffffff, wg = -1, first_g = -1;
+#pragma unroll
+                for (int g = 0; g < GPW; ++g) {
+                    const int og_e = __builtin_amdgcn_readlane(e, g * GS), og_c = __builtin_amdgcn_readlane(r.c, g * GS);
+                    const double og_cost = readlane_d(rec_cost, g * GS);
+                    const bool mine = ((live_m >> (g * GS)) & 1ull) != 0ull && og_e == e;
+                    if (mine && argmin_better(og_cost, og_c, bc, bi)) { bc = og_cost; bi = og_c; wg = g; }
+                    if (mine && og_c == c0) first_g = g;
+                }
+                if (!(bc < __builtin_huge_val()) && !(bc != bc)) { bi = c0; wg = first_g; }
+                Clothoid wcl;
+                wcl.ok = false; wcl.k0 = 0; wcl.dk = 0; wcl.L = 0;
+#pragma unroll
+                for (int g = 0; g < GPW; ++g) {
+                    const double gk0 = readlane_d(rec_k0, g * GS), gdk = readlane_d(rec_dk, g * GS), gL = readlane_d(rec_L, g * GS);
+                    const int gok = __builtin_amdgcn_readlane(rec_ok, g * GS);
+                    if (wg == g) { wcl.k0 = gk0; wcl.dk = gdk; wcl.L = gL; wcl.ok = gok == 1; }
+                }
+                if (fin && gl == 0) {
+                    if (a.best_idx) a.best_idx[e] = bi;
+                    if (a.best_cost) a.best_cost[e] = bc;
+                    if (a.near_idx) a.near_idx[e] = ego_near;
+                }
+                if (a.mode != LATTICE_EVAL) {
+                    const double* wpos = reinterpret_cast<double*>(lds_raw) + (size_t)(wave * GPW + (wg < 0 ? grp : wg)) * gstride + 64 + 4 * (size_t)S;
+                    emit_and_track_group<GS>(a, cfg, fin, e, den, wcl, bc, wpos, wpos + S, v_near);
+                }
+            }
+            if (__any(far)) {
+                asm volatile("s_waitcnt vmcnt(0)" ::: "memory");
+                unsigned int old = 0u;
+                if (far && gl == 0) old = __hip_atomic_fetch_add((f1p_gu32*)(mx.ego_done + e), 1u, __ATOMIC_RELAXED, __HIP_MEMORY_SCOPE_AGENT);
+                unsigned long long lm = __ballot(far && gl == 0 && old + 1u == (unsigned int)mx.ego_n[e]);
+                __builtin_amdgcn_fence(__ATOMIC_ACQUIRE, "wavefront");
+                __builtin_amdgcn_s_waitcnt(0xc07f);
+                __builtin_amdgcn_wave_barrier();
+                while (lm) {
+                    const int src = __ffsll((long long)lm) - 1;
+                    lm &= lm - 1;
+                    const int e2 = __shfl(e, src, 64);
+                    tail_select_wave(a, cfg, mx, e2, lane, reinterpret_cast<double*>(lds_raw) + (size_t)wave * GPW * gstride);
+                    __builtin_amdgcn_s_waitcnt(0xc07f);
+                    __builtin_amdgcn_wave_barrier();
+                }
+            }
         }
 #ifdef F1P_MIX_PHASES
         F1P_RPH();
@@ -517,6 +658,30 @@
     }
 }
 
+template <int GS, bool FOOT = false>
+__global__ __launch_bounds__(256, 2) void k_lattice_refine(LatticeArgs a, f1p_lattice_cfg cfg, MixArgs mx) {
+    extern __shared__ __align__(16) unsigned char lds_raw[];
+    warm_kernargs<sizeof(LatticeArgs) + sizeof(f1p_lattice_cfg) + sizeof(MixArgs)>();
+    lattice_refine_body<GS, FOOT, false>(a, cfg, mx, lds_raw, gridDim.x);
+}
+
+template <int GS, bool FOOT = false>
+__global__ __launch_bounds__(256, 2) void k_lattice_tail(LatticeArgs a, f1p_lattice_cfg cfg, MixArgs mx, unsigned int nwg) {
+    extern __shared__ __align__(16) unsigned char lds_raw[];
+    warm_kernargs<sizeof(LatticeArgs) + sizeof(f1p_lattice_cfg) + sizeof(MixArgs) + 8>();
+    if (blockIdx.x >= nwg) {
+        const int eo = a.e0 + (int)(blockIdx.x - nwg) * (int)blockDim.x + (int)threadIdx.x;
+        if (mx.perm_fill && eo < a.E) {
+            const unsigned r = (unsigned)eo % F1P_MIX_OREG;
+            const int slot = mx.heavy[eo] ? (int)atomicAdd(&mx.ocnt[r * 64u], 1u) : mx.perm_rs - 1 - (int)atomicAdd(&mx.ocnt[r * 64u + 32u], 1u);
+            mx.perm_fill[r * (unsigned)mx.perm_rs + (unsigned)slot] = eo + 1;
+        }
+        return;
+    }
+    lattice_refine_body<GS, FOOT, true>(a, cfg, mx, lds_raw, nwg);
+}
+
+
 bool mixed_refine_fits(f1p_ctx* ctx, int lanes, bool foot, size_t lds) {
     if (lanes == 16) return foot ? lds_fits(ctx, (k_lattice_refine<16, true>), lds) : lds_fits(ctx, k_lattice_refine<16>, lds);
     return foot ? lds_fits(ctx, (k_lattice_refine<64, true>), lds) : lds_fits(ctx, k_lattice_refine<64>, lds);
@@ -524,6 +689,22 @@
 
 bool mixed_refine_cubic_fits(f1p_ctx* ctx, size_t lds) {
     return lds_fits(ctx, k_lattice_refine_cubic<16>, lds) && lds_fits(ctx, (k_lattice_refine_cubic<16, true>), lds);
+}
+
+bool mixed_tail_fits(f1p_ctx* ctx, int lanes, bool foot, size_t lds) {
+    if (lanes == 16) return foot ? lds_fits(ctx, (k_lattice_tail<16, true>), lds) : lds_fits(ctx, k_lattice_tail<16>, lds);
+    return foot ? lds_fits(ctx, (k_lattice_tail<64, true>), lds) : lds_fits(ctx, k_lattice_tail<64>, lds);
+}
+
+void mixed_launch_tail(int lanes, bool foot, unsigned grid, unsigned fill, size_t lds, hipStream_t st, const LatticeArgs& a, const f1p_lattice_cfg& cfg, const MixArgs& mx) {
+    const dim3 g(grid + fill), b(256);
+    if (lanes == 16) {
+        if (foot) hipLaunchKernelGGL((k_lattice_tail<16, true>), g, b, lds, st, a, cfg, mx, grid);
+        else hipLaunchKernelGGL(k_lattice_tail<16>, g, b, lds, st, a, cfg, mx, grid);
+    } else {
+        if (foot) hipLaunchKernelGGL((k_lattice_tail<64, true>), g, b, lds, st, a, cfg, mx, grid);
+        else hipLaunchKernelGGL(k_lattice_tail<64>, g, b, lds, st, a, cfg, mx, grid);
+    }
 }
 
 void mixed_launch_refine(bool cubic, int lanes, bool foot, unsigned grid, size_t lds, hipStream_t st, const LatticeArgs& a, const f1p_lattice_cfg& cfg, const MixArgs& mx) {
diff --git a/f1tenth_planning_amd/csrc/lattice_device.h b/f1tenth_planning_amd/csrc/lattice_device.h
--- a/f1tenth_planning_amd/csrc/lattice_device.h
+++ b/f1tenth_planning_amd/csrc/lattice_device.h
@@ -845,6 +845,78 @@
     }
 }
 
+template <int GS>
+__device__ __forceinline__ void emit_and_track_group(const LatticeArgs& a, const f1p_lattice_cfg& cfg, bool act, int e, int den,
+                                                     const Clothoid& cl, double bc, const double* tr_x, const double* tr_y, double v_near) {
+    const int S = cfg.n_stations;
+    const int lane = threadIdx.x & 63, gl = lane & (GS - 1), gbase = lane & ~(GS - 1);
+    if (act) {
+        double* bt = a.best_traj ? a.best_traj + (size_t)e * S * 4 : nullptr;
+        float4* bt32 = a.best_traj32 ? reinterpret_cast<float4*>(a.best_traj32) + (size_t)e * S : nullptr;
+        double* tho = a.theta_out ? a.theta_out + (size_t)e * S : nullptr;
+        const double ds = cl.ok ? cl.L / (double)den : 0.0;
+        if (bt || bt32 || tho) {
+            for (int i = gl; i < S; i += GS) {
+                double x = 0.0, y = 0.0;
+                if (cl.ok) { x = tr_x[i]; y = tr_y[i]; }
+                const double s = (double)i * ds;
+                const double th = cl.ok ? s * (cl.k0 + 0.5 * s * cl.dk) : 0.0;
+                const double ak = cl.ok ? fabs(cl.k0 + cl.dk * s) : 0.0;
+                if (bt) {
+                    typedef double f1p_d2 __attribute__((ext_vector_type(2)));
+                    if (a.traj_in_hbm) {
+                        __builtin_nontemporal_store((f1p_d2){x, y}, reinterpret_cast<f1p_d2*>(bt) + 2 * i);
+                        __builtin_nontemporal_store((f1p_d2){th, ak}, reinterpret_cast<f1p_d2*>(bt) + 2 * i + 1);
+                    } else {
+                        reinterpret_cast<double2*>(bt)[2 * i] = make_double2(x, y);
+                        reinterpret_cast<double2*>(bt)[2 * i + 1] = make_double2(th, ak);
+                    }
+                }
+                if (bt32) bt32[i] = make_float4((float)x, (float)y, (float)th, (float)ak);
+                if (tho) __builtin_nontemporal_store(th, tho + i);
+            }
+        }
+    }
+    Track o;
+    o.steer = 0.0; o.speed = 0.0; o.la_idx = F1P_LA_NONE; o.status = F1P_ST_ALL_BLOCKED;
+    const bool trk = act && cl.ok && bc < __builtin_huge_val();
+    if (__any(trk)) {
+        const int n = trk ? S : 0;
+        bool plain = true;
+        for (int i = gl; i < n - 1; i += GS) {
+            const double ax = tr_x[i], ay = tr_y[i], dx = tr_x[i + 1] - ax, dy = tr_y[i + 1] - ay;
+            const double l2 = dx * dx + dy * dy;
+            plain &= (l2 > 0.0) & (l2 < __builtin_huge_val()) & (fabs(ax) < __builtin_huge_val()) & (fabs(ay) < __builtin_huge_val());
+        }
+        const unsigned long long gm = GS == 64 ? ~0ull : (1ull << (GS & 63)) - 1ull;
+        plain = group_ballot<GS>(plain, gbase) == gm;
+        if (trk) plain = plain && tr_x[0] == 0.0 && tr_y[0] == 0.0 && S >= 2;
+        double td = 0.0, tt = 0.0; int ti = 0;
+        const bool scan = trk && !plain;
+        if (__any(scan)) {
+            double sd; int si;
+            nearest_scan(0.0, 0.0, tr_x, tr_y, scan ? S : 0, gl, GS, sd, si);
+#pragma unroll
+            for (int m = GS / 2; m >= 1; m >>= 1) {
+                const double od = shfl_xor_d(sd, m);
+                const int oi = __shfl_xor(si, m, F1P_WAVE);
+                if (argmin_better(od, oi, sd, si)) { sd = od; si = oi; }
+            }
+            if (scan) {
+                const SegProj ts = seg_project(0.0, 0.0, tr_x[si], tr_y[si], tr_x[si + 1], tr_y[si + 1]);
+                ti = si; tt = ts.t; td = ts.d;
+            }
+        }
+        const Track t = group_pursuit<GS>(trk, 0.0, 0.0, 0.0, cfg.track_lookahead, cfg.wheelbase, cfg.max_reacquire, tr_x, tr_y, v_near, n, ti, tt, td);
+        if (trk) o = t;
+    }
+    if (act && gl == 0) {
+        a.steer[e] = o.steer;
+        a.speed[e] = o.speed;
+        if (a.status) a.status[e] = o.status;
+    }
+}
+
 template <typename K>
 static bool lds_fits(f1p_ctx* ctx, K kernel, size_t bytes) {
     if (bytes <= (size_t)ctx->prop.sharedMemPerBlock) return true;
diff --git a/f1tenth_planning_amd/csrc/lattice_mixed.h b/f1tenth_planning_amd/csrc/lattice_mixed.h
--- a/f1tenth_planning_amd/csrc/lattice_mixed.h
+++ b/f1tenth_planning_amd/csrc/lattice_mixed.h
@@ -94,6 +94,9 @@
 #endif
 #ifndef F1P_PRO2_MIN_EGOS
 #define F1P_PRO2_MIN_EGOS 3072
+#endif
+#ifndef F1P_MIX_FUSED_TAIL
+#define F1P_MIX_FUSED_TAIL 1
 #endif
 #define F1P_ST_FREE 0
 #define F1P_ST_HIT 1
@@ -122,6 +125,7 @@
     int32_t* ego_base;
     int32_t* ego_n;
     int32_t* ego_ni;
+    unsigned int* ego_done;
     struct EgoXform* xf;
     const uint32_t* clear_bits;
     int clear_r;
@@ -143,6 +147,15 @@
     int32_t* dbg_pass;
 };
 
+__device__ __forceinline__ void mixed_rearm(const MixArgs& mx) {
+    if (blockIdx.x == 0 && threadIdx.x < F1P_MIX_QSHARDS) mx.qcount[threadIdx.x * 32u] = 0u;
+    if (mx.perm_fill) {
+        const int np = F1P_MIX_OREG * mx.perm_rs;
+        for (int i = (int)(blockIdx.x * blockDim.x + threadIdx.x); i < np; i += (int)(gridDim.x * blockDim.x)) mx.perm_fill[i] = 0;
+        if (blockIdx.x == 0 && threadIdx.x < 2 * F1P_MIX_OREG) mx.ocnt[threadIdx.x * 32u] = 0u;
+    }
+}
+
 struct GoalFrame32 { double cx, cy, nx, ny; float gth; int ok; };
 
 __device__ __forceinline__ int cvt_flr_i32_f32(float v) {
@@ -183,6 +196,8 @@
 bool mixed_refine_fits(f1p_ctx* ctx, int lanes, bool foot, size_t lds);
 bool mixed_refine_cubic_fits(f1p_ctx* ctx, size_t lds);
 void mixed_launch_refine(bool cubic, int lanes, bool foot, unsigned grid, size_t lds, hipStream_t st, const LatticeArgs& a, const f1p_lattice_cfg& cfg, const MixArgs& mx);
+bool mixed_tail_fits(f1p_ctx* ctx, int lanes, bool foot, size_t lds);
+void mixed_launch_tail(int lanes, bool foot, unsigned grid, unsigned fill, size_t lds, hipStream_t st, const LatticeArgs& a, const f1p_lattice_cfg& cfg, const MixArgs& mx);
 bool mixed_select_fits(f1p_ctx* ctx, bool cubic, size_t lds, bool tracks = false);
 void mixed_launch_select(bool cubic, bool tracks, unsigned grid, size_t lds, hipStream_t st, const LatticeArgs& a, const f1p_lattice_cfg& cfg, const MixArgs& mx);
 
```

After: 702.3 billion. 6.4% lower.
